# phirling/pyc2ray

Measured on AMD Instinct MI355X. Metric: cell-updates/sec (raytrace+chem), higher is better.
Workload: dtype f64

## Files before the change

include/asora_hip.h:

```cpp
#ifndef ASORA_HIP_H
#define ASORA_HIP_H

#include <stddef.h>
#include <stdint.h>

#ifdef __cplusplus
extern "C" {
#endif


int asora_device_init(int N, int num_src_par);
int asora_device_init_ex(int N, int num_src_par, int device_id);

int asora_device_close(void);

int asora_density_to_device(const double *ndens, int N);

int asora_photo_table_to_device(const double *thin_table, const double *thick_table, int NumTau);

int asora_heat_table_to_device(const double *heat_thin_table, const double *heat_thick_table, int NumTau);

int asora_source_data_to_device(const int32_t *pos, const double *flux, int NumSrc);

#define ASORA_MAX_SPECTRA 16
int asora_spectra_to_device(int NumSpec, int NumTau, const double *photo_thin, const double *photo_thick,
                            const double *heat_thin, const double *heat_thick);
int asora_source_spectra_to_device(const int32_t *spec, int NumSrc);
int asora_num_spectra(void);
int asora_debug_sort_sources(const int32_t *pos, const double *flux, const int32_t *spec, int NumSrc, int32_t *pos_out,
                             double *flux_out, int32_t *spec_out);

int asora_do_all_sources(double R, double *coldensh_out, double sig, double dr, const double *ndens,
                         const double *xh_av, double *phi_ion, int NumSrc, int m1,
                         double minlogtau, double dlogtau, int NumTau);

int c2ray_global_pass(double dt, const double *ndens, const double *temp, const double *xh,
                      double *xh_av, double *xh_intermed, const double *phi_ion,
                      double bh00, double albpow, double colh0, double temph0, double abu_c,
                      int m1, int m2, int m3, int *conv_flag);

int c2ray_do_all_sources(const double *normflux, const int32_t *srcpos, int max_subbox, int subboxsize,
                         double *coldensh_out, double sig, double dr, const double *ndens, const double *xh_av,
                         double *phi_ion, double *phi_heat, float loss_fraction,
                         const double *photo_thin_table, const double *photo_thick_table,
                         const double *heat_thin_table, const double *heat_thick_table,
                         double minlogtau, double dlogtau, double R_max_LLS,
                         int NumTau, int NumSrc, int m1, int m2, int m3,
                         int *sum_nbox, double *photon_loss);

const char *asora_last_error(void);


enum {
    ASORA_GRID_NDENS = 0,
    ASORA_GRID_XH_AV = 1,
    ASORA_GRID_PHI_ION = 2,
    ASORA_GRID_TEMP = 3,
    ASORA_GRID_XH = 4,
    ASORA_GRID_XH_INTERMED = 5,
    ASORA_GRID_PHI_HEAT = 6,
    ASORA_GRID_TEMP_END = 7,
    ASORA_GRID_CLUMP = 8,
    ASORA_GRID_COUNT = 9
};

int asora_grid_to_device(int which, const double *host, int N, char order);
int asora_grid_to_host(int which, double *host, int N, char order);
int asora_grid_copy(int dst, int src);
int asora_grid_scale(int which, double factor);
int asora_grid_sum(int which, double *sum);
int asora_host_alloc(size_t bytes, void **host);
int asora_host_free(void *host);
void *asora_device_ptr(int which);

int asora_raytrace_device(double R, double sig, double dr, int src_begin, int src_count,
                          double minlogtau, double dlogtau, int NumTau);

int asora_raytrace_begin(double R, double sig, double dr, double minlogtau, double dlogtau, int NumTau);
int asora_raytrace_range(int src_begin, int src_count);
int asora_raytrace_begin_planes(double R, double sig, double dr, double minlogtau, double dlogtau, int NumTau,
                                const int *runs, int nruns);
int asora_raytrace_fold(int i_begin, int i_count);
void *asora_stream(void);

int asora_subbox_raytrace_device(int max_subbox, int subboxsize, float loss_fraction, double R_max_LLS, double sig,
                                 double dr, double minlogtau, double dlogtau, int NumTau, int src_begin, int src_count,
                                 int *sum_nbox, double *photon_loss);
int asora_device_init_auto(int N);

int asora_chemistry_device(double dt, double bh00, double albpow, double colh0, double temph0,
                           double abu_c, int *conv_flag, double *sum_xh1, double *sum_xh0);

int asora_chemistry_range(double dt, double bh00, double albpow, double colh0, double temph0, double abu_c,
                          int i_begin, int i_count, int first);
int asora_chemistry_finish(int *conv_flag, double *sum_xh1, double *sum_xh0);
void *asora_reduction_ptr(void);

int asora_evolve_begin(double dt, double bh00, double albpow, double colh0, double temph0, double abu_c,
                       double R, double sig, double dr, double minlogtau, double dlogtau, int NumTau,
                       int src_begin, int src_count, double conv_criterion, double convergence_fraction);
int asora_evolve_enqueue(int iterations);
int asora_evolve_poll(int *niter, int *converged, double *history, int history_rows, int *rows_written);

int asora_evolve_begin_slab(double dt, double bh00, double albpow, double colh0, double temph0, double abu_c,
                            double R, double sig, double dr, double minlogtau, double dlogtau, int NumTau,
                            int src_begin, int src_count, double conv_criterion, double convergence_fraction,
                            int own_begin, int own_count);
int asora_evolve_begin_slab_thermal(double dt, double bh00, double albpow, double colh0, double temph0, double abu_c,
                                    double R, double sig, double dr, double minlogtau, double dlogtau, int NumTau,
                                    int src_begin, int src_count, double conv_criterion, double convergence_fraction,
                                    int own_begin, int own_count);
int asora_evolve_slab_trace(int src_begin, int src_count);
int asora_evolve_slab_fold_out(int i_begin, int i_count);
int asora_evolve_slab_fold_all(void);
void *asora_evolve_slab_outbox(void);
int asora_evolve_slab_outbox_to_host(int i_begin, int i_count, double *host);
int asora_evolve_slab_outbox_from_host(int i_begin, int i_count, const double *host);
int asora_evolve_slab_add(int i_begin, int i_count, const double *dev_planes);
int asora_evolve_slab_add_host(int i_begin, int i_count, const double *host_planes);
void *asora_evolve_slab_heat_outbox(void);
int asora_evolve_slab_heat_outbox_to_host(int i_begin, int i_count, double *host);
int asora_evolve_slab_heat_outbox_from_host(int i_begin, int i_count, const double *host);
int asora_evolve_slab_add_heat(int i_begin, int i_count, const double *dev_planes);
int asora_evolve_slab_add_heat_host(int i_begin, int i_count, const double *host_planes);
int asora_evolve_slab_pass(void);
int asora_evolve_slab_nhi(int i_begin, int i_count);
int asora_evolve_slab_close(const double *host_sums);

int asora_planes_to_host(int which, int i_begin, int i_count, double *host);
int asora_planes_to_device(int which, int i_begin, int i_count, const double *host);

int asora_thermal_params(int enable, double relative_denergy, double t_floor, int max_substeps, unsigned cooling_mask,
                         int compton, double t_cmb);
int asora_thermal_stats(long long *cells_max_substeps, long long *cells_floored, int *max_substeps_used);

int asora_clumping(int mode, double constant);

int asora_lls_opacity(double n_const, double per_density);
int asora_get_lls_opacity(double *n_const, double *per_density);


enum {
    ASORA_OPT_FORTRAN_CONSTANTS = 0,
    ASORA_OPT_GREY_NOTABLES = 1,
    ASORA_OPT_TIMING = 2,
    ASORA_OPT_Z_TRANSPOSED = 3,
    ASORA_OPT_BLOCK_THREADS = 4,
    ASORA_OPT_SECTORS = 5,
    ASORA_OPT_HEATING = 6,
    ASORA_OPT_C2RAY_OWN_FLUX = 7,
    ASORA_OPT_NO_UNIFORM_T = 8,
    ASORA_OPT_SUBBOX_GLOBAL_SHELLS = 9,
    ASORA_OPT_PIPELINED_COPIES = 10,
    ASORA_OPT_SKIP_ZERO_RATES = 11,
    ASORA_OPT_GLOBAL_ATOMICS = 12,
    ASORA_OPT_PAIR_SOURCES = 13,
    ASORA_OPT_SUBBOX_TABLES = 14,
    ASORA_OPT_ALIGNED_ROWS = 15,
    ASORA_OPT_GEOMETRY_ON_HOST = 16,
    ASORA_OPT_PLACEMENT_CANDIDATES = 17,
    ASORA_OPT_OPEN_BOUNDARIES = 18,
    ASORA_OPT_COUNT = 19
};
int asora_set_option(int option, int value);
int asora_get_option(int option);

enum { ASORA_KERNEL_RAYTRACE = 0, ASORA_KERNEL_CHEMISTRY = 1, ASORA_KERNEL_PREP = 2,
       ASORA_KERNEL_FINISH = 3, ASORA_KERNEL_COUNT = 4 };
int asora_kernel_time_ms(int kernel, double *total_ms, long *launches);
int asora_kernel_time_reset(void);
int asora_synchronize(void);

int asora_last_raytrace_counts(long long *gamma_cells, long long *evaluated_cells);
int asora_last_raytrace_counts_ex(long long *gamma_cells, long long *evaluated_cells, long long *zero_rates_left_out);

int asora_debug_coldens(double R, double sig, double dr, int source_index, double *coldens_out, int N);

enum {
    ASORA_VARIANT_PAIRED = 1,
    ASORA_VARIANT_ALIGNED = 2,
    ASORA_VARIANT_BUFFER_ATOMICS = 4,
    ASORA_VARIANT_SPLIT_DESCRIPTORS = 8,
    ASORA_VARIANT_SKIP_ZERO = 16,
    ASORA_VARIANT_GLOBAL_SHELLS = 32,
    ASORA_VARIANT_OPEN_BOUNDARIES = 64
};
int asora_last_raytrace_variant(void);

size_t asora_debug_geometry_bytes(void);
void asora_debug_placement(int *candidates, double *chosen_probe_ms, double *slowest_probe_ms);
void asora_debug_init_cost(double *device_init_ms, double *placement_probe_ms);
int asora_debug_geometry_table(int table, uint32_t *words, size_t capacity_entries, size_t *entries, int *nsteps, int *ntables,
                               int *shells, int *max_cells, int *threads);

const char *asora_build_id(void);
const char *asora_build_flags(void);

#ifdef __cplusplus
}
#endif
#endif
```

pyc2ray_amd/_capi.py:

```python
import ctypes as C
import os

_HERE = os.path.dirname(os.path.abspath(__file__))
LIB_PATH = os.environ.get("PYC2RAY_AMD_LIBASORA") or os.path.join(_HERE, "lib", "libasora_hip.so")

GRID_NDENS, GRID_XH_AV, GRID_PHI_ION, GRID_TEMP, GRID_XH, GRID_XH_INTERMED, GRID_PHI_HEAT = range(7)
GRID_TEMP_END = 7
GRID_CLUMP = 8
(OPT_FORTRAN_CONSTANTS, OPT_GREY_NOTABLES, OPT_TIMING, OPT_Z_TRANSPOSED, OPT_BLOCK_THREADS, OPT_SECTORS,
 OPT_HEATING, OPT_C2RAY_OWN_FLUX, OPT_NO_UNIFORM_T, OPT_SUBBOX_GLOBAL_SHELLS, OPT_PIPELINED_COPIES,
 OPT_SKIP_ZERO_RATES, OPT_GLOBAL_ATOMICS, OPT_PAIR_SOURCES, OPT_SUBBOX_TABLES, OPT_ALIGNED_ROWS, OPT_GEOMETRY_ON_HOST,
 OPT_PLACEMENT_CANDIDATES, OPT_OPEN_BOUNDARIES) = range(19)
MAX_SPECTRA = 16
KERNEL_RAYTRACE, KERNEL_CHEMISTRY, KERNEL_PREP, KERNEL_FINISH = range(4)
VARIANT_PAIRED, VARIANT_ALIGNED, VARIANT_BUFFER_ATOMICS, VARIANT_SPLIT_DESCRIPTORS, VARIANT_SKIP_ZERO, VARIANT_GLOBAL_SHELLS = 1, 2, 4, 8, 16, 32
VARIANT_OPEN_BOUNDARIES = 64

_dp = C.POINTER(C.c_double)
_ip = C.POINTER(C.c_int32)

SIGNATURES = {
    "asora_device_init": (C.c_int, [C.c_int, C.c_int]),
    "asora_device_init_ex": (C.c_int, [C.c_int, C.c_int, C.c_int]),
    "asora_device_close": (C.c_int, []),
    "asora_density_to_device": (C.c_int, [_dp, C.c_int]),
    "asora_photo_table_to_device": (C.c_int, [_dp, _dp, C.c_int]),
    "asora_heat_table_to_device": (C.c_int, [_dp, _dp, C.c_int]),
    "asora_source_data_to_device": (C.c_int, [_ip, _dp, C.c_int]),
    "asora_spectra_to_device": (C.c_int, [C.c_int, C.c_int, _dp, _dp, _dp, _dp]),
    "asora_source_spectra_to_device": (C.c_int, [_ip, C.c_int]),
    "asora_num_spectra": (C.c_int, []),
    "asora_debug_sort_sources": (C.c_int, [_ip, _dp, _ip, C.c_int, _ip, _dp, _ip]),
    "asora_do_all_sources": (C.c_int, [C.c_double, _dp, C.c_double, C.c_double, _dp, _dp, _dp, C.c_int, C.c_int,
                                       C.c_double, C.c_double, C.c_int]),
    "c2ray_global_pass": (C.c_int, [C.c_double, _dp, _dp, _dp, _dp, _dp, _dp, C.c_double, C.c_double, C.c_double,
                                    C.c_double, C.c_double, C.c_int, C.c_int, C.c_int, C.POINTER(C.c_int)]),
    "c2ray_do_all_sources": (C.c_int, [_dp, _ip, C.c_int, C.c_int, _dp, C.c_double, C.c_double, _dp, _dp, _dp, _dp,
                                       C.c_float, _dp, _dp, _dp, _dp, C.c_double, C.c_double, C.c_double,
                                       C.c_int, C.c_int, C.c_int, C.c_int, C.c_int, C.POINTER(C.c_int), _dp]),
    "asora_last_error": (C.c_char_p, []),
    "asora_grid_to_device": (C.c_int, [C.c_int, _dp, C.c_int, C.c_char]),
    "asora_grid_to_host": (C.c_int, [C.c_int, _dp, C.c_int, C.c_char]),
    "asora_grid_copy": (C.c_int, [C.c_int, C.c_int]),
    "asora_grid_scale": (C.c_int, [C.c_int, C.c_double]),
    "asora_device_ptr": (C.c_void_p, [C.c_int]),
    "asora_grid_sum": (C.c_int, [C.c_int, C.POINTER(C.c_double)]),
    "asora_host_alloc": (C.c_int, [C.c_size_t, C.POINTER(C.c_void_p)]),
    "asora_host_free": (C.c_int, [C.c_void_p]),
    "asora_raytrace_device": (C.c_int, [C.c_double, C.c_double, C.c_double, C.c_int, C.c_int, C.c_double,
                                        C.c_double, C.c_int]),
    "asora_raytrace_begin": (C.c_int, [C.c_double, C.c_double, C.c_double, C.c_double, C.c_double, C.c_int]),
    "asora_raytrace_range": (C.c_int, [C.c_int, C.c_int]),
    "asora_raytrace_begin_planes": (C.c_int, [C.c_double, C.c_double, C.c_double, C.c_double, C.c_double, C.c_int, _ip,
                                              C.c_int]),
    "asora_raytrace_fold": (C.c_int, [C.c_int, C.c_int]),
    "asora_stream": (C.c_void_p, []),
    "asora_subbox_raytrace_device": (C.c_int, [C.c_int, C.c_int, C.c_float, C.c_double, C.c_double, C.c_double, C.c_double,
                                               C.c_double, C.c_int, C.c_int, C.c_int, C.POINTER(C.c_int), _dp]),
    "asora_device_init_auto": (C.c_int, [C.c_int]),
    "asora_chemistry_device": (C.c_int, [C.c_double, C.c_double, C.c_double, C.c_double, C.c_double, C.c_double,
                                         C.POINTER(C.c_int), _dp, _dp]),
    "asora_chemistry_range": (C.c_int, [C.c_double, C.c_double, C.c_double, C.c_double, C.c_double, C.c_double,
                                        C.c_int, C.c_int, C.c_int]),
    "asora_chemistry_finish": (C.c_int, [C.POINTER(C.c_int), _dp, _dp]),
    "asora_reduction_ptr": (C.c_void_p, []),
    "asora_evolve_begin": (C.c_int, [C.c_double] * 11 + [C.c_int, C.c_int, C.c_int, C.c_double, C.c_double]),
    "asora_evolve_enqueue": (C.c_int, [C.c_int]),
    "asora_evolve_poll": (C.c_int, [C.POINTER(C.c_int), C.POINTER(C.c_int), _dp, C.c_int, C.POINTER(C.c_int)]),
    "asora_evolve_begin_slab": (C.c_int, [C.c_double] * 11 + [C.c_int, C.c_int, C.c_int, C.c_double, C.c_double, C.c_int, C.c_int]),
    "asora_evolve_begin_slab_thermal": (C.c_int, [C.c_double] * 11 + [C.c_int, C.c_int, C.c_int, C.c_double, C.c_double, C.c_int, C.c_int]),
    "asora_evolve_slab_trace": (C.c_int, [C.c_int, C.c_int]),
    "asora_evolve_slab_fold_out": (C.c_int, [C.c_int, C.c_int]),
    "asora_evolve_slab_outbox": (C.c_void_p, []),
    "asora_evolve_slab_outbox_to_host": (C.c_int, [C.c_int, C.c_int, _dp]),
    "asora_evolve_slab_outbox_from_host": (C.c_int, [C.c_int, C.c_int, _dp]),
    "asora_evolve_slab_fold_all": (C.c_int, []),
    "asora_debug_placement": (None, [C.POINTER(C.c_int), _dp, _dp]),
    "asora_debug_init_cost": (None, [_dp, _dp]),
    "asora_evolve_slab_add": (C.c_int, [C.c_int, C.c_int, C.c_void_p]),
    "asora_evolve_slab_add_host": (C.c_int, [C.c_int, C.c_int, _dp]),
    "asora_evolve_slab_heat_outbox": (C.c_void_p, []),
    "asora_evolve_slab_heat_outbox_to_host": (C.c_int, [C.c_int, C.c_int, _dp]),
    "asora_evolve_slab_heat_outbox_from_host": (C.c_int, [C.c_int, C.c_int, _dp]),
    "asora_evolve_slab_add_heat": (C.c_int, [C.c_int, C.c_int, C.c_void_p]),
    "asora_evolve_slab_add_heat_host": (C.c_int, [C.c_int, C.c_int, _dp]),
    "asora_evolve_slab_pass": (C.c_int, []),
    "asora_evolve_slab_nhi": (C.c_int, [C.c_int, C.c_int]),
    "asora_evolve_slab_close": (C.c_int, [_dp]),
    "asora_planes_to_host": (C.c_int, [C.c_int, C.c_int, C.c_int, _dp]),
    "asora_planes_to_device": (C.c_int, [C.c_int, C.c_int, C.c_int, _dp]),
    "asora_thermal_params": (C.c_int, [C.c_int, C.c_double, C.c_double, C.c_int, C.c_uint, C.c_int, C.c_double]),
    "asora_thermal_stats": (C.c_int, [C.POINTER(C.c_longlong), C.POINTER(C.c_longlong), C.POINTER(C.c_int)]),
    "asora_clumping": (C.c_int, [C.c_int, C.c_double]),
    "asora_lls_opacity": (C.c_int, [C.c_double, C.c_double]),
    "asora_get_lls_opacity": (C.c_int, [_dp, _dp]),
    "asora_set_option": (C.c_int, [C.c_int, C.c_int]),
    "asora_get_option": (C.c_int, [C.c_int]),
    "asora_kernel_time_ms": (C.c_int, [C.c_int, _dp, C.POINTER(C.c_long)]),
    "asora_kernel_time_reset": (C.c_int, []),
    "asora_synchronize": (C.c_int, []),
    "asora_last_raytrace_counts": (C.c_int, [C.POINTER(C.c_longlong), C.POINTER(C.c_longlong)]),
    "asora_last_raytrace_counts_ex": (C.c_int, [C.POINTER(C.c_longlong), C.POINTER(C.c_longlong), C.POINTER(C.c_longlong)]),
    "asora_debug_coldens": (C.c_int, [C.c_double, C.c_double, C.c_double, C.c_int, _dp, C.c_int]),
    "asora_last_raytrace_variant": (C.c_int, []),
    "asora_debug_geometry_bytes": (C.c_size_t, []),
    "asora_debug_geometry_table": (C.c_int, [C.c_int, C.POINTER(C.c_uint32), C.c_size_t, C.POINTER(C.c_size_t), C.POINTER(C.c_int),
                                             C.POINTER(C.c_int), C.POINTER(C.c_int), C.POINTER(C.c_int), C.POINTER(C.c_int)]),
    "asora_build_id": (C.c_char_p, []),
    "asora_build_flags": (C.c_char_p, []),
}

_lib = None


def load():
    global _lib
    if _lib is not None:
        return _lib
    if not os.path.exists(LIB_PATH):
        raise RuntimeError(
            f"pyc2ray_amd: HIP library not found at {LIB_PATH}. Build it with "
            "`make -C pyc2ray_amd/csrc` (or `python -c 'import __graft_entry__ as g; g.build()'`). "
            "There is no CPU fallback.")
    if os.environ.get("PYC2RAY_AMD_NO_TORCH", "0") != "1":
        try:
            import torch
        except ImportError:
            pass
    lib = C.CDLL(LIB_PATH)
    for name, (res, args) in SIGNATURES.items():
        fn = getattr(lib, name)
        fn.restype = res
        fn.argtypes = args
    _lib = lib
    return lib


def check(rc, what):
    if rc != 0:
        msg = load().asora_last_error()
        raise RuntimeError(f"{what} failed (code {rc}): {msg.decode() if msg else 'unknown error'}")


def dptr(a):
    return a.ctypes.data_as(_dp)


def iptr(a):
    return a.ctypes.data_as(_ip)
```

pyc2ray_amd/csrc/api.hip:

```cpp
#include "asora_internal.hpp"

#include <chrono>

namespace asora {

static State g_state;
static std::string g_error;

State &state() { return g_state; }
int fail(int code, const std::string &msg) { g_error = msg; return code; }
void clear_error() { g_error.clear(); }

static int flush_timers()
{
    State &st = g_state;
    if (st.pending_timers.empty()) return 0;
    ASORA_HIP_TRY(hipStreamSynchronize(st.stream));
    for (hipStream_t s : st.side) if (s) ASORA_HIP_TRY(hipStreamSynchronize(s));
    for (auto &pt : st.pending_timers) {
        float ms = 0.f;
        if (hipEventElapsedTime(&ms, pt.e0, pt.e1) == hipSuccess) {
            st.k_ms[pt.which] += (double)ms;
            st.k_n[pt.which] += 1;
        }
        st.free_events.push_back(pt.e0);
        st.free_events.push_back(pt.e1);
    }
    st.pending_timers.clear();
    return 0;
}

static hipEvent_t take_event()
{
    State &st = g_state;
    if (!st.free_events.empty()) { hipEvent_t e = st.free_events.back(); st.free_events.pop_back(); return e; }
    hipEvent_t e = nullptr;
    (void)hipEventCreate(&e);
    return e;
}

KernelTimer::KernelTimer(int w, hipStream_t s)
    : which(w), on(g_state.opt[ASORA_OPT_TIMING] != 0 && g_state.stream != nullptr), stream(s ? s : g_state.stream)
{
    if (!on) return;
    if (g_state.pending_timers.size() >= 4096) (void)flush_timers();
    e0 = take_event();
    e1 = take_event();
    (void)hipEventRecord(e0, stream);
}
KernelTimer::~KernelTimer()
{
    if (!on) return;
    (void)hipEventRecord(e1, stream);
    g_state.pending_timers.push_back({which, e0, e1});
}

int ensure_runtime()
{
    State &st = g_state;
    if (st.stream) return 0;
    ASORA_HIP_TRY(hipSetDevice(st.device));
    hipDeviceProp_t prop;
    ASORA_HIP_TRY(hipGetDeviceProperties(&prop, st.device));
    st.cu_count = prop.multiProcessorCount > 0 ? prop.multiProcessorCount : 256;
    ASORA_HIP_TRY(hipStreamCreateWithFlags(&st.stream, hipStreamNonBlocking));
    for (int q = 0; q < 2; ++q) {
        ASORA_HIP_TRY(hipStreamCreateWithFlags(&st.side[q], hipStreamNonBlocking));
        ASORA_HIP_TRY(hipEventCreateWithFlags(&st.side_done[q], hipEventDisableTiming));
    }
    ASORA_HIP_TRY(hipEventCreateWithFlags(&st.main_ready, hipEventDisableTiming));
    st.red_blocks = chemistry_reduction_blocks(st);
    st.red_cap = 3 * (size_t)st.red_blocks;
    ASORA_HIP_TRY(hipMalloc(&st.red_partial, sizeof(double) * st.red_cap));
    ASORA_HIP_TRY(hipMalloc(&st.red_final, sizeof(double) * 3));
    ASORA_HIP_TRY(hipHostMalloc(&st.red_host, sizeof(double) * 3, hipHostMallocDefault));
    ASORA_HIP_TRY(hipMalloc(&st.counters, sizeof(unsigned long long) * COUNTER_FIELDS * COUNTER_SLOTS));
    ASORA_HIP_TRY(hipMemset(st.counters, 0, sizeof(unsigned long long) * COUNTER_FIELDS * COUNTER_SLOTS));
    return 0;
}

static int release_all()
{
    State &st = g_state;
    auto drop = [](auto *&ptr) { if (ptr) { (void)hipFree(ptr); ptr = nullptr; } };
    drop(st.grid[ASORA_GRID_PHI_HEAT]);
    drop(st.grid[ASORA_GRID_TEMP_END]); drop(st.heat_acc); drop(st.heat_outbox); drop(st.th_stats_dev);
    st.heat_clean[0] = st.heat_clean[1] = false;
    st.th_on = false; st.th = ThermalConsts();
    drop(st.grid[ASORA_GRID_CLUMP]);
    st.clump_mode = 0; st.clump_c = 1.0;
    st.lls_a = st.lls_b = 0.0;
    for (int g = 0; g < ASORA_GRID_COUNT; ++g) { st.grid[g] = nullptr; st.grid_valid[g] = false; }
    st.nhi = st.staging = st.acc = nullptr;
    drop(st.arena); st.arena_bytes = 0;
    st.ev_clean[0] = st.ev_clean[1] = false; st.ev_sets_known = false;
    drop(st.reach.mask); drop(st.reach.count_dev); st.reach = State::ReachMask();
    st.ev_open = false;
    st.temp_probe_valid = false;
    st.nhi_t = st.phi_t = st.heat_t = nullptr;
    st.have_heat_tables = false;
    drop(st.tables); st.table_len = 0; st.num_spec = 1; st.spec_stride = 0;
    drop(st.src_spec); drop(st.src_spec_sorted); st.src_spec_max = 0;
    drop(st.src_pos); drop(st.src_flux); drop(st.src_pos_sorted); drop(st.src_flux_sorted); st.src_i0_sorted.clear(); st.num_src = 0;
    st.src_pos_host.clear(); st.src_pos_sorted_host.clear();
    release_pair_lists(st);
    drop(st.shell_scratch); st.shell_scratch_bytes = 0;
    drop(st.sb_trail); st.sb_trail_bytes = 0;
    if (st.geom_patch_dev) { (void)hipFree(st.geom_patch_dev); st.geom_patch_dev = nullptr; st.geom_patch_cap = 0; }
    drop(st.sb_active); drop(st.sb_nbox); drop(st.sb_loss); drop(st.sb_loss_final); st.subbox_cap = 0;
    release_geometry(st);
    st.init = false; st.N = 0; st.ncell = 0;
    st.rt_radius[0] = State::RadiusHistory(); st.rt_radius[1] = State::RadiusHistory();
    if (st.zero_probe_dev) { (void)hipFree(st.zero_probe_dev); st.zero_probe_dev = nullptr; }
    if (st.zero_probe_host) { (void)hipHostFree(st.zero_probe_host); st.zero_probe_host = nullptr; }
    if (st.zero_probe_done) { (void)hipEventDestroy(st.zero_probe_done); st.zero_probe_done = nullptr; }
    st.zero_probe_pending = false; st.zero_known = false; st.zero_dark = false; st.zero_since_probe = 0;
    st.rt_open = false;
    return 0;
}

int require_init(const char *who)
{
    if (!g_state.init) return fail(2, std::string(who) + ": device not initialised (call asora_device_init first)");
    return 0;
}

int check_N(const char *who, int N)
{
    if (N != g_state.N)
        return fail(3, std::string(who) + ": mesh size " + std::to_string(N) + " does not match device_init(" +
                           std::to_string(g_state.N) + ")");
    return 0;
}

int check_planes(const char *who, int code, const char *tail, int i_begin, int i_count)
{
    if (i_begin < 0 || i_count < 0 || i_begin + i_count > g_state.N) return fail(code, std::string(who) + ": " + tail);
    return 0;
}

int check_sources(const char *who, int code, const std::string &tail, int src_begin, int src_count)
{
    if (src_begin < 0 || src_count < 0 || src_begin + src_count > g_state.num_src) return fail(code, std::string(who) + ": " + tail);
    return 0;
}

int require_grids(const char *who, std::initializer_list<int> grids)
{
    for (int g : grids)
        if (!g_state.grid_valid[g]) return fail(4, std::string(who) + ": grid " + std::to_string(g) + " holds no data");
    return 0;
}

}

using namespace asora;

extern "C" {

constexpr int ARENA_CANDIDATES = 8;
constexpr int ARENA_SLOTS = 14;
__global__ void __launch_bounds__(256) placement_probe_kernel(char *arena, size_t slot, size_t n)
{
    const double *in[5]; double *out[7];
    for (int q = 0; q < 5; ++q) in[q] = reinterpret_cast<const double *>(arena + q * slot);
    for (int q = 0; q < 7; ++q) out[q] = reinterpret_cast<double *>(arena + (5 + q) * slot);
    for (size_t i = (size_t)blockIdx.x * 256 + threadIdx.x; i < n; i += (size_t)gridDim.x * 256) {
        double s = 0.0;
#pragma unroll
        for (int q = 0; q < 5; ++q) s += __builtin_nontemporal_load(in[q] + i);
#pragma unroll
        for (int q = 0; q < 7; ++q) out[q][i] = s;
    }
}

static int choose_arena(State &st, size_t slot, int slots)
{
    const auto wall0 = std::chrono::steady_clock::now();
    const size_t total = slot * (size_t)slots;
    int want = st.opt[ASORA_OPT_PLACEMENT_CANDIDATES] > 0 ? st.opt[ASORA_OPT_PLACEMENT_CANDIDATES] : ARENA_CANDIDATES;
    if (const char *e = getenv("ASORA_PLACEMENT_CANDIDATES")) want = std::max(1, atoi(e));
    want = std::min(want, 32);
    if (st.N < 128) want = 1;
    size_t free_b = 0, all_b = 0;
    if (want > 1 && hipMemGetInfo(&free_b, &all_b) == hipSuccess && total > 0)
        want = (int)std::max<size_t>(1, std::min<size_t>((size_t)want, (size_t)(0.125 * (double)free_b) / total));
    st.arena_candidates = 0; st.arena_probe_ms = st.arena_probe_worst_ms = st.arena_probe_wall_ms = 0.0;
    if (want == 1) {
        ASORA_HIP_TRY(hipMalloc(&st.arena, total));
        st.arena_bytes = total; st.arena_candidates = 1;
        return 0;
    }
    hipEvent_t t0, t1;
    ASORA_HIP_TRY(hipEventCreate(&t0)); ASORA_HIP_TRY(hipEventCreate(&t1));
    std::vector<char *> cand;
    std::vector<float> ms;
    int best = -1;
    float worst = 0.0f;
    const size_t n = st.ncell;
    for (int c = 0; c < want; ++c) {
        char *a = nullptr;
        if (hipMalloc(&a, total) != hipSuccess) { (void)hipGetLastError(); break; }
        cand.push_back(a);
        float t = 1e30f;
        for (int rep = 0; rep < 3; ++rep) {
            (void)hipEventRecord(t0, st.stream);
            hipLaunchKernelGGL(placement_probe_kernel, dim3(1024), dim3(256), 0, st.stream, a, slot, n);
            (void)hipEventRecord(t1, st.stream);
            if (hipEventSynchronize(t1) != hipSuccess) { t = 1e30f; break; }
            float e = 0.0f;
            (void)hipEventElapsedTime(&e, t0, t1);
            if (rep >= 1) t = std::min(t, e);
        }
        ms.push_back(t);
        if (best < 0 || t < ms[(size_t)best]) best = c;
        worst = std::max(worst, t);
        if (c >= 1 && ms[(size_t)best] <= 0.93f * worst) break;
    }
    (void)hipEventDestroy(t0); (void)hipEventDestroy(t1);
    if (best < 0) return fail(2, "device_init: out of device memory for the grids");
    for (size_t c = 0; c < cand.size(); ++c) if ((int)c != best) (void)hipFree(cand[c]);
    st.arena = cand[(size_t)best];
    st.arena_bytes = total;
    st.arena_candidates = (int)cand.size();
    st.arena_probe_ms = ms[(size_t)best]; st.arena_probe_worst_ms = worst;
    st.arena_probe_wall_ms = std::chrono::duration<double, std::milli>(std::chrono::steady_clock::now() - wall0).count();
    return 0;
}

void asora_debug_placement(int *candidates, double *chosen_probe_ms, double *slowest_probe_ms)
{
    if (candidates) *candidates = g_state.arena_candidates;
    if (chosen_probe_ms) *chosen_probe_ms = g_state.arena_probe_ms;
    if (slowest_probe_ms) *slowest_probe_ms = g_state.arena_probe_worst_ms;
}

void asora_debug_init_cost(double *device_init_ms, double *placement_probe_ms)
{
    if (device_init_ms) *device_init_ms = g_state.device_init_wall_ms;
    if (placement_probe_ms) *placement_probe_ms = g_state.arena_probe_wall_ms;
}

const char *asora_last_error(void) { return g_error.c_str(); }

int asora_device_init_ex(int N, int num_src_par, int device_id)
{
    clear_error();
    State &st = g_state;
    const auto init_wall0 = std::chrono::steady_clock::now();
    if (N < 2 || N > 1280) return fail(1, "device_init: N must be in [2, 1280] (32-bit cell indices over 2 N^3)");
    if (st.stream && device_id != st.device) return fail(1, "device_init: the device cannot change within a process");
    if (st.init) release_all();
    st.device = device_id;
    if (int rc = ensure_runtime()) return rc;
    st.N = N;
    st.ncell = (size_t)N * N * N;
    st.num_src_par = num_src_par;
    st.auto_init = false;
    const size_t bytes = st.ncell * sizeof(double);
    const size_t slot = (bytes + 4095) / 4096 * 4096;
    if (int rc = choose_arena(st, slot, ARENA_SLOTS)) return rc;
    {
        size_t at = 0;
        auto take = [&](size_t grids) { double *q = reinterpret_cast<double *>(st.arena + at); at += grids * slot; return q; };
        st.grid[ASORA_GRID_NDENS] = take(1); st.grid[ASORA_GRID_XH] = take(1); st.grid[ASORA_GRID_XH_AV] = take(1);
        st.grid[ASORA_GRID_TEMP] = take(1); st.grid[ASORA_GRID_XH_INTERMED] = take(1);
        st.acc = take(4);
        st.nhi = take(2);
        st.grid[ASORA_GRID_PHI_ION] = take(2);
        st.staging = take(1);
    }
    for (int g = 0; g < ASORA_GRID_COUNT; ++g)
        if (g != ASORA_GRID_PHI_HEAT && g != ASORA_GRID_TEMP_END && g != ASORA_GRID_CLUMP && !st.grid[g]) return fail(11, "device_init: a grid without a place in the arena (internal error)");
    st.nhi_t = st.nhi + st.ncell;
    st.phi_t = st.grid[ASORA_GRID_PHI_ION] + st.ncell;
    st.heat_t = nullptr;
    st.ev_sets_known = false;
    {
        size_t worst = 0;
        for (int planes = 1; planes <= N; ++planes) worst = std::max(worst, chemistry_tile_blocks(st, N, planes));
        if (int rc = ensure_red_capacity(3 * worst)) return rc;
    }
    st.init = true;
    st.device_init_wall_ms = std::chrono::duration<double, std::milli>(std::chrono::steady_clock::now() - init_wall0).count();
    return 0;
}

int asora_device_init(int N, int num_src_par)
{
    int dev = g_state.stream ? g_state.device : 0;
    if (!g_state.stream) {
        if (hipGetDevice(&dev) != hipSuccess) dev = 0;
    }
    return asora_device_init_ex(N, num_src_par, dev);
}

int asora_device_close(void)
{
    clear_error();
    if (int rc = require_init("device_close")) return rc;
    ASORA_HIP_TRY(hipStreamSynchronize(g_state.stream));
    return release_all();
}

void *asora_stream(void) { return (void *)g_state.stream; }

int asora_set_option(int option, int value)
{
    clear_error();
    if (option < 0 || option >= ASORA_OPT_COUNT) return fail(3, "set_option: unknown option");
    g_state.opt[option] = value;
    return 0;
}

int asora_get_option(int option)
{
    if (option < 0 || option >= ASORA_OPT_COUNT) return -1;
    return g_state.opt[option];
}

int asora_kernel_time_ms(int kernel, double *total_ms, long *launches)
{
    clear_error();
    if (kernel < 0 || kernel >= ASORA_KERNEL_COUNT) return fail(3, "kernel_time_ms: unknown kernel");
    if (int rc = flush_timers()) return rc;
    if (total_ms) *total_ms = g_state.k_ms[kernel];
    if (launches) *launches = g_state.k_n[kernel];
    return 0;
}

int asora_kernel_time_reset(void)
{
    (void)flush_timers();
    for (int k = 0; k < ASORA_KERNEL_COUNT; ++k) { g_state.k_ms[k] = 0.0; g_state.k_n[k] = 0; }
    return 0;
}

int asora_synchronize(void)
{
    clear_error();
    if (!g_state.stream) return 0;
    ASORA_HIP_TRY(hipStreamSynchronize(g_state.stream));
    ASORA_HIP_TRY(hipDeviceSynchronize());
    return 0;
}

}
```

pyc2ray_amd/csrc/asora_internal.hpp:

```cpp
#pragma once
#include <hip/hip_runtime.h>
#include <algorithm>
#include <cmath>
#include <cstdint>
#include <cstdio>
#include <cstdlib>
#include <cstring>
#include <initializer_list>
#include <string>
#include <vector>

#include "../../include/asora_hip.h"

namespace asora {

struct OctGeomDev {
    const uint4 *cellA;
    const uint4 *cellB;
    int nsteps;
    int info;
    int inner;
    int reserved_;
};

constexpr int MAX_UNITS = 96;

constexpr int COUNTER_SLOTS = 4096;
constexpr int ZERO_PROBE_SLOTS = 256;
constexpr int COUNTER_FIELDS = 3;

inline double lut_index_limit(int NumTau, int table_len)
{
    const double by_reference = (double)(float)NumTau, by_table = (double)(table_len > 0 ? table_len - 1 : 0);
    return by_reference < by_table ? by_reference : by_table;
}

struct RtParams {
    int N;
    int S;
    int max_cells;
    double R;
    double sig, dr;
    double minlogtau, dlogtau, numtau_f;
    double lut_k1, lut_k0;
    double tau_zero;
    int NumTau, table_len;
    int fortran_consts, grey, z_transposed;
    int src_begin, src_count;
    int shape_src_count;
    int split_desc;
    int radius_stays;
    OctGeomDev geom[MAX_UNITS];
    int units;
    int spread;
    const double2 *logtab;
    unsigned ncell;
    const double *nhi;
    double *phi;
    const double2 *tables;
    double *heat;
    const int32_t *src_pos;
    const double *src_flux;
    double *dump;
    double *shell_scratch;
    unsigned long long *counters;
    const int *done_flag;
    unsigned long long *zero_probe;
    int aligned;
    const int2 *pairs[2];
    int npairs[2];
    int sb_k0[12], sb_k1[12];
    int sb_first;
    int sb_edge_r, sb_edge_l;
    int flux_src;
    const int *sb_active;
    double *sb_loss;
    double *sb_trail;
    const int32_t *src_spec;
    unsigned spec_stride;
    int open_bc;
};

struct ThermalConsts {
    double relative_denergy = 0.1;
    double t_floor = 1.0;
    double t_cmb = 0.0;
    int max_substeps = 10000;
    unsigned cooling_mask = 31u;
    int compton = 0;
};
constexpr unsigned THERMAL_COOL_RECOMB = 1u, THERMAL_COOL_COLION = 2u, THERMAL_COOL_COLEXC = 4u, THERMAL_COOL_BREMS = 8u,
                   THERMAL_COOL_COMPTON = 16u;

constexpr int EVOLVE_HIST = 64;
struct EvolveStatus {
    int niter;
    int done;
    double prev1, prev0;
    double conv_criterion, conv_fraction;
    double hist[EVOLVE_HIST][5];
};

struct State {
    bool init = false;
    bool auto_init = false;
    int device = 0;
    int N = 0;
    size_t ncell = 0;
    int num_src_par = 0;
    int cu_count = 256;

    double *grid[ASORA_GRID_COUNT] = {nullptr, nullptr, nullptr, nullptr, nullptr, nullptr, nullptr, nullptr, nullptr};
    bool grid_valid[ASORA_GRID_COUNT] = {false, false, false, false, false, false, false, false, false};

    double *nhi = nullptr;
    double *nhi_t = nullptr;
    double *phi_t = nullptr;
    double *heat_t = nullptr;
    bool have_heat_tables = false;
    double *staging = nullptr;

    double2 *tables = nullptr;
    int table_len = 0;
    int num_spec = 1;
    size_t spec_stride = 0;

    int32_t *src_pos = nullptr;
    double *src_flux = nullptr;
    int num_src = 0;
    int32_t *src_pos_sorted = nullptr;
    double *src_flux_sorted = nullptr;
    std::vector<int> src_i0_sorted;
    int32_t *src_spec = nullptr, *src_spec_sorted = nullptr;
    int src_spec_max = 0;
    std::vector<hipEvent_t> pipe_events;

    std::vector<void *> geom_owned;
    size_t geom_bytes = 0;
    OctGeomDev geom_host[MAX_UNITS];
    bool geom_aligned = false;
    unsigned long long *zero_probe_dev = nullptr;
    unsigned long long *zero_probe_host = nullptr;
    hipEvent_t zero_probe_done = nullptr;
    bool zero_probe_pending = false, zero_known = false, zero_dark = false;
    int zero_since_probe = 0;
    int last_variant = 0;
    struct RadiusHistory { double last_R = -1.0; long same_R_calls = 0; bool has_changed = false; };
    RadiusHistory rt_radius[2];
    std::vector<int32_t> src_pos_host, src_pos_sorted_host;
    struct PairList { const void *list; int begin, count; int2 *dev[2]; int n[2]; };
    std::vector<PairList> pair_lists;
    int geom_units = 0;
    double2 *logtab_dev = nullptr;
    bool geom_valid = false;
    bool geom_on_host = false;
    struct SphereCell { uint32_t *dev_word; uint32_t word_without_rate; int a, b, c; };
    std::vector<SphereCell> geom_sphere;
    void *geom_patch_dev = nullptr;
    size_t geom_patch_cap = 0;
    int geom_N = 0, geom_S = 0, geom_max_cells = 0, geom_threads = 0;
    int geom_subbox = 0, geom_ext_r = 0, geom_ext_l = 0, geom_boxsize = 0;
    std::vector<int> geom_step_after_shell[12];
    double geom_R = 0.0, geom_dr = 0.0;

    RtParams rt_params;
    bool rt_open = false, rt_heat = false;
    bool rt_pipelined = false;
    bool rt_by_planes = false;
    hipStream_t side[2] = {nullptr, nullptr};
    hipEvent_t side_done[2] = {nullptr, nullptr}, main_ready = nullptr;
    bool side_pending[2] = {false, false};
    int side_next = 0;

    int *sb_active = nullptr, *sb_nbox = nullptr, *sb_nactive = nullptr;
    double *sb_loss = nullptr, *sb_loss_final = nullptr;
    size_t subbox_cap = 0;

    double *sb_trail = nullptr;
    size_t sb_trail_bytes = 0;

    double *shell_scratch = nullptr;
    size_t shell_scratch_bytes = 0;

    double *red_partial = nullptr;
    size_t red_cap = 0;
    double *red_final = nullptr;
    double *red_host = nullptr;
    int red_blocks = 0;

    unsigned long long *counters = nullptr;
    long long last_gamma_cells = 0, last_eval_cells = 0;

    double *acc = nullptr;
    char *arena = nullptr;
    size_t arena_bytes = 0;
    int arena_candidates = 0;
    double arena_probe_ms = 0.0, arena_probe_worst_ms = 0.0;
    double arena_probe_wall_ms = 0.0, device_init_wall_ms = 0.0;
    int ev_base = 0;
    bool ev_clean[2] = {false, false};
    bool ev_sets_known = false;
    int ev_folded_iter = -1;
    EvolveStatus *ev_status = nullptr;
    EvolveStatus *ev_host = nullptr;
    bool ev_open = false, ev_first = true;
    double *temp_probe_dev = nullptr;
    double temp_probe[5] = {0, 0, 0, 0, 0};
    bool temp_probe_valid = false;
    double temp_consts[4] = {0, 0, 0, 0};
    int ev_reported = 0;
    int ev_enqueued = 0;
    double ev_chem[6] = {0, 0, 0, 0, 0, 0};
    int ev_src_begin = 0, ev_src_count = 0;
    RtParams ev_rt;
    bool ev_slab = false;
    int ev_own_begin = 0, ev_own_count = 0;
    bool ev_slab_passed = false;
    bool ev_folded_all = false;
    bool ev_rates_in_outbox = false;
    bool ev_slab_thermal = false;
    struct ReachMask {
        unsigned char *mask = nullptr;
        size_t bytes = 0;
        unsigned long long *count_dev = nullptr;
        bool in_use = false;
        bool pays = false;
        struct Key {
            bool valid = false;
            long src_generation = -1;
            int src_begin = 0, src_count = 0;
            double R = -1.0;
            bool operator==(const Key &o) const { return valid == o.valid && src_generation == o.src_generation && src_begin == o.src_begin && src_count == o.src_count && R == o.R; }
        } key;
    } reach;
    long src_generation = 0;

    bool th_on = false;
    ThermalConsts th;
    double *heat_acc = nullptr;
    bool heat_clean[2] = {false, false};
    double *heat_outbox = nullptr;
    unsigned long long *th_stats_dev = nullptr;

    int clump_mode = 0;
    double clump_c = 1.0;
    double temp_probe_clump = 1.0;

    double lls_a = 0.0, lls_b = 0.0;
    bool coldens_only = false;

    hipStream_t stream = nullptr;
    struct PendingTimer { int which; hipEvent_t e0, e1; };
    std::vector<PendingTimer> pending_timers;
    std::vector<hipEvent_t> free_events;
    int opt[ASORA_OPT_COUNT] = {0, 0, 0, 1, 0, 0, 0, 0, 0, 0, 1, 0, 0, 0, 0, 0, 0, 0, 0};
    double k_ms[ASORA_KERNEL_COUNT] = {0, 0, 0, 0};
    long k_n[ASORA_KERNEL_COUNT] = {0, 0, 0, 0};
};

State &state();
int fail(int code, const std::string &msg);
void clear_error();

#define ASORA_HIP_TRY(expr)                                                                     \
    do {                                                                                        \
        hipError_t e__ = (expr);                                                                \
        if (e__ != hipSuccess)                                                                  \
            return ::asora::fail(10, std::string(#expr) + ": " + hipGetErrorName(e__) + " - " + \
                                         hipGetErrorString(e__));                               \
    } while (0)

struct KernelTimer {
    int which;
    bool on;
    hipStream_t stream;
    hipEvent_t e0 = nullptr, e1 = nullptr;
    explicit KernelTimer(int w, hipStream_t s = nullptr);
    ~KernelTimer();
};


constexpr unsigned CELL_VALID = 1u << 30, CELL_LAST = 1u << 31, CELL_RATE = 1u << 29,
                   CELL_SPHERE = 1u << 28,
                   CELL_ZERO_SHIFT = 25,
                   CELL_NEG_SHIFT = 22,
                   CELL_SLOT_MASK = (1u << 22) - 1;

struct GeomTableSpec {
    int face = -1;
    int merge_mask = 0;
    int ext[3] = {0, 0, 0};
    int ext_neg = 0;
    int wedge = -1;
    int align_class = -1;
};
int build_geometry_on_device(State &st, const std::vector<GeomTableSpec> &specs, double R, double dr, int q_max, int threads,
                             int boxsize, std::vector<OctGeomDev> &out, std::vector<std::vector<int>> &step_after, int &S_all,
                             uint32_t &max_cells_all);
struct SubboxGeometry { int ext_r, ext_l, boxsize; };
int ensure_geometry(State &st, RtParams &p, int threads, int units, const SubboxGeometry *sbg = nullptr, bool aligned = false);
void release_geometry(State &st);
bool note_call_radius(State &st, double R, int path);
void release_pair_lists(State &st);
int launch_fold_range(State &st, const double *src_t, double *dst, int i_begin, int i_count);
int ensure_logtab(State &st);
int launch_prepare_nhi(State &st, bool need_transposed);
int launch_finish_phi(State &st);
int check_open_boundaries(const State &st, const char *who, bool open, bool dump);
int launch_raytrace(State &st, RtParams &p, bool dump, bool heat, hipStream_t side = nullptr);
struct SubboxTables { int units = 0, threads = 0, S = 0, max_batch = 0, nsrc = 1; bool ok = false, aligned = false; const int32_t *host_pos = nullptr; };
int subbox_tables_prepare(State &st, RtParams &p, int ext_r, int ext_l, int subboxsize, int src_count, bool heat, SubboxTables &out,
                          const int32_t *host_pos);
int subbox_tables_sweep(State &st, const RtParams &p, const SubboxTables &tab, int s_begin, int s_end, bool heat);
int launch_fold_transposed(State &st, const double *src_t, double *dst);
int launch_fold_sum(State &st, const double *a, const double *b_t, double *dst);
int launch_transpose(State &st, const double *src, double *dst, int N);

struct SubboxParams {
    int N, W;
    int ext_r, ext_l;
    int s_begin, s_end;
    int edge_r, edge_l;
    double sig, dr, R;
    double numtau_f, lut_k1, lut_k0;
    int table_len;
    int grey, heat, add_zero;
    int src_begin, src_count;
    int flux_src;
    int dump_src;
    unsigned ncell;
    const double *nhi;
    double *phi, *heat_grid;
    double *dump;
    const double2 *tables, *logtab;
    const int32_t *src_pos;
    const double *src_flux;
    double *scratch;
    size_t unit_stride;
    const int *active;
    double *loss;
};
int launch_subbox_sweep(State &st, const SubboxParams &p, hipStream_t side = nullptr);
int launch_subbox_decide(State &st, int mode, int count, const double *src_flux, int src_begin, double loss_fraction,
                         int more_range, int *active, double *loss, double *loss_final, int *nbox, int *n_active);

struct ChemParams {
    size_t ncell;
    double dt, bh00, albpow, colh0, temph0, abu_c;
    const double *ndens, *temp, *xh, *phi;
    double *xh_av, *xh_intermed;
    double *red_partial, *red_final;
    int red_blocks;
    int accumulate = 0;
    bool thermal = false;
    const double *phi_heat = nullptr;
    double *temp_end = nullptr;
    unsigned long long *th_stats = nullptr;
    ThermalConsts th;
    const double *clump = nullptr;
    double clump_c = 1.0;
};
int launch_chemistry(State &st, ChemParams &p, hipStream_t stream, bool clumped = true);
int chemistry_reduction_blocks(const State &st);

struct ChemTileParams {
    int N = 0, i_begin = 0, i_end = 0;
    double dt = 0, bh00 = 0, albpow = 0, colh0 = 0, temph0 = 0, abu_c = 0;
    const double *ndens = nullptr, *temp = nullptr, *xh = nullptr, *xh_av_in = nullptr;
    double *gamma = nullptr, *gamma_t = nullptr;
    double *phi_out = nullptr;
    double *zero_a = nullptr, *zero_t = nullptr;
    double *xh_av = nullptr, *xh_intermed = nullptr;
    double *nhi = nullptr, *nhi_t = nullptr;
    double *red_partial = nullptr, *red_final = nullptr;
    int red_stride = 0;
    int accumulate = 0;
    EvolveStatus *status = nullptr;
    bool local_sums = false;
    const unsigned char *reach_a = nullptr, *reach_t = nullptr;
    bool fold = false, emit = false;
    int uniform = 0, uniform_t_ok = 0;
    double uniform_T = 0, uniform_brech0 = 0, uniform_acolh0 = 0;
    bool thermal = false;
    double *heat = nullptr, *heat_t = nullptr;
    double *zero_ha = nullptr, *zero_ht = nullptr;
    double *temp_end = nullptr;
    unsigned long long *th_stats = nullptr;
    ThermalConsts th;
    const double *clump = nullptr;
    double clump_c = 1.0;
    double *heat_out = nullptr;
    double lls_a = 0.0, lls_b = 0.0;
};
int launch_grid_sum(State &st, const double *a, size_t n, double *out_dev);
int launch_scale(State &st, double *a, size_t n, double factor);
int launch_temp_probe(State &st, const double *temp, size_t n, double bh00, double albpow, double colh0, double temph0,
                      double *out_dev);
int launch_chemistry_tiles(State &st, ChemTileParams &p, hipStream_t stream);
size_t chemistry_tile_blocks(const State &st, int N, int planes);
int launch_prepare_nhi_from(State &st, const double *xh_av, bool need_transposed);
int launch_prepare_range(State &st, int i_begin, int i_count, bool zero_acc, double *acc, const int *done = nullptr);
int launch_fold_out(State &st, const double *a, const double *a_t, double *out, double *z_a, double *z_t, int i_begin, int i_count,
                    const int *done);
int launch_fold_out_pair(State &st, const double *a, const double *a_t, double *out, double *z_a, double *z_t, const double *h,
                         const double *h_t, double *hout, double *zh_a, double *zh_t, int i_begin, int i_count, const int *done);
int launch_add_planes(State &st, double *dst, const double *src, size_t n, const int *done);
int launch_convergence_test(State &st, const double *sums, EvolveStatus *status);
int launch_reach_mask(State &st, const int32_t *src_pos, int src_begin, int src_count, double R, unsigned char *mask, size_t bytes_one_layout);
int launch_reach_count(State &st, const unsigned char *mask, size_t bytes_both_layouts, unsigned long long *out_dev);

int ensure_runtime();
int require_init(const char *who);
int check_N(const char *who, int N);
int check_planes(const char *who, int code, const char *tail, int i_begin, int i_count);
int check_sources(const char *who, int code, const std::string &tail, int src_begin, int src_count);
int require_grids(const char *who, std::initializer_list<int> grids);
int ensure_optional_grid(int which);
int reset_counters();
int require_raytrace_inputs(const char *who, double R, int NumTau, bool density, bool xh_av);
void fill_rt_params(RtParams &p, double R, double sig, double dr, double minlogtau, double dlogtau, int NumTau, int radius_path = 0);
inline void use_source_list(RtParams &p, const State &st, bool sorted)
{
    p.src_pos = sorted ? st.src_pos_sorted : st.src_pos;
    p.src_flux = sorted ? st.src_flux_sorted : st.src_flux;
    p.src_spec = sorted ? st.src_spec_sorted : st.src_spec;
}
int check_source_spectra(const char *who);
void sort_sources_by_position(const int32_t *pos, int NumSrc, std::vector<int> &order);
int ensure_red_capacity(size_t entries);
int ensure_temp_probe(double bh00, double albpow, double colh0, double temph0);
ChemTileParams chem_tile_common(int i_begin, int i_count, const double chem[6]);

}
```

pyc2ray_amd/csrc/chemistry.hip:

```cpp
#include "rates_device.hpp"

#include <algorithm>

namespace asora {

constexpr int CH_THREADS = 256;

struct TempFactors {
    double T = -1.0;
    double brech0 = 0.0, acolh0 = 0.0;
    bool t_ok = false;
};
__device__ __forceinline__ void temperature_factors(const ChemParams &p, double T, TempFactors &f)
{
    if (T == f.T) return;
    f.T = T;
    f.brech0 = 1.0 * p.bh00 * pow(T / 1e4, p.albpow);
    f.acolh0 = p.colh0 * sqrt(T) * exp(-p.temph0 / T);
    f.t_ok = fabs((T - T) / T) < (double)1.0e-3f;
}

template <bool CLUMP = false>
__device__ __forceinline__ void chemistry_cell(const ChemParams &p, double n, double x0, double gamma,
                                               double &xav, double &xint, unsigned int &nconv, const TempFactors &tf,
                                               double clump = 1.0)
{
    const double min_frac_change = (double)1.0e-3f;
    const double min_frac_atoms = (double)1.0e-8f;
    const double eps = 1e-14;

    const double xav_start = xav;
    const double yh_av = 1.0 - xav;

    const double brech0 = CLUMP ? clump * tf.brech0 : tf.brech0, acolh0 = tf.acolh0;
    const bool t_ok = tf.t_ok;

    int nit = 0;
    for (;;) {
        nit += 1;
        const double xav_old = xav;
        const double de = n * (xav + p.abu_c);
        const double aih0 = gamma + de * acolh0;
        const double delth = aih0 + de * brech0;
        const double eqxh = aih0 / delth;
        const double deltht = delth * p.dt;
        const double ee = exp(-deltht);
        xint = (x0 - eqxh) * ee + eqxh;
        if (xint < eps) xint = eps;
        const double avg = (deltht < (double)1.0e-8f) ? 1.0 : (1.0 - ee) / deltht;
        xav = eqxh + (x0 - eqxh) * avg;
        if (xav < eps) xav = eps;
        if ((fabs((xav - xav_old) / (1.0 - xav)) < min_frac_change || (1.0 - xav < min_frac_atoms)) && t_ok)
            break;
        if (nit > 400) break;
    }
    if (fabs(xav - xav_start) > min_frac_change && fabs((xav - xav_start) / yh_av) > min_frac_change &&
        yh_av > min_frac_atoms)
        nconv += 1;
}

constexpr double THERMAL_KB = 1.381e-16;
constexpr double CODATA_SIGMA_T = 6.6524587321e-25, CODATA_SIGMA_SB = 5.670374419e-5, CODATA_C = 2.99792458e10,
                 CODATA_KB = 1.380649e-16, CODATA_ME = 9.1093837015e-28;
constexpr double COMPTON_A_RAD = 4.0 * CODATA_SIGMA_SB / CODATA_C;
constexpr double COMPTON_C = 4.0 * CODATA_SIGMA_T * COMPTON_A_RAD * CODATA_KB / (CODATA_ME * CODATA_C);

template <bool CLUMP = false>
__device__ __forceinline__ double thermal_cooling(const ThermalConsts &c, double T, double n_e, double n_HII, double n_HI,
                                                  double colh0, double temph0, double clump = 1.0)
{
#pragma clang fp contract(off)
    double L = 0.0;
    if (c.cooling_mask & THERMAL_COOL_RECOMB) {
        const double lam = 2.0 * 157807.0 / T;
        double rec = 3.435e-30 * T * pow(lam, 1.970) / pow(1.0 + pow(lam / 2.25, 0.376), 3.720) * n_e * n_HII;
        if (CLUMP) rec = rec * clump;
        L += rec;
    }
    if (c.cooling_mask & THERMAL_COOL_COLION)
        L += THERMAL_KB * temph0 * colh0 * sqrt(T) * exp(-temph0 / T) * n_e * n_HI;
    if (c.cooling_mask & THERMAL_COOL_COLEXC)
        L += 7.5e-19 * exp(-118348.0 / T) / (1.0 + sqrt(T / 1e5)) * n_e * n_HI;
    if (c.cooling_mask & THERMAL_COOL_BREMS) {
        const double u = 5.5 - log10(T);
        const double gff = 1.1 + 0.34 * exp(-(u * u) / 3.0);
        L += 1.42e-27 * gff * sqrt(T) * n_e * n_HII;
    }
    if ((c.cooling_mask & THERMAL_COOL_COMPTON) && c.compton) {
        const double tg = c.t_cmb;
        L += COMPTON_C * ((tg * tg) * (tg * tg)) * (T - tg) * n_e;
    }
    return L;
}

struct ThermalTally {
    unsigned capped = 0, floored = 0;
    int max_sub = 0;
};

template <bool CLUMP = false>
__device__ __forceinline__ void thermal_integrate(const ThermalConsts &c, double dt, double abu_c, double colh0, double temph0,
                                                  double n, double x, double phi_heat, double T_start, double &T_end,
                                                  double &T_av, bool &capped, bool &floored, int &max_sub, double clump = 1.0)
{
#pragma clang fp contract(off)
    const double n_e = n * (x + abu_c), n_HII = n * x, n_HI = n * (1.0 - x);
    const double n_p = n * (1.0 + x + abu_c);
    const double cv = 1.5 * THERMAL_KB * n_p;
    const double H = n_HI * phi_heat;
    double T = T_start, e = cv * T_start, t = 0.0, intT = 0.0;
    int k = 0;
    for (;;) {
        k += 1;
        const double r = H - thermal_cooling<CLUMP>(c, T, n_e, n_HII, n_HI, colh0, temph0, clump);
        double h = dt - t;
        bool last = true;
        if (k < c.max_substeps && r != 0.0) {
            const double hl = c.relative_denergy * e / fabs(r);
            if (hl < h) { h = hl; last = false; }
        }
        double Tn = (e + h * r) / cv;
        if (Tn < c.t_floor) { Tn = c.t_floor; floored = true; }
        e = cv * Tn;
        intT += h * (T + Tn) * 0.5;
        T = Tn;
        if (last) break;
        t += h;
    }
    if (k >= c.max_substeps) capped = true;
    if (k > max_sub) max_sub = k;
    T_end = T;
    T_av = intT / dt;
}

template <bool CLUMP = false>
__device__ __forceinline__ void chemistry_cell_thermal(const ChemParams &p, double n, double x0, double gamma, double phi_heat,
                                                       double T_start, double &xav_io, double &xint_out, double &T_end_out,
                                                       unsigned int &nconv, ThermalTally &tally, double clump = 1.0)
{
#pragma clang fp contract(off)
    const double min_frac_change = (double)1.0e-3f;
    const double min_frac_atoms = (double)1.0e-8f;
    const double eps = 1e-14;

    double xav = xav_io, xint = 0.0;
    const double xav_start = xav;
    const double yh_av = 1.0 - xav;
    double T_av = T_start, T_end = T_start;
    bool capped = false, floored = false;
    int max_sub = tally.max_sub;

    int nit = 0;
    for (;;) {
        nit += 1;
        const double xav_old = xav, T_prev = T_end;
        const double de = n * (xav + p.abu_c);
        double brech0 = 1.0 * p.bh00 * pow(T_av / 1e4, p.albpow);
        if (CLUMP) brech0 = clump * brech0;
        const double acolh0 = p.colh0 * sqrt(T_av) * exp(-p.temph0 / T_av);
        const double aih0 = gamma + de * acolh0;
        const double delth = aih0 + de * brech0;
        const double eqxh = aih0 / delth;
        const double deltht = delth * p.dt;
        const double ee = exp(-deltht);
        xint = (x0 - eqxh) * ee + eqxh;
        if (xint < eps) xint = eps;
        const double avg = (deltht < (double)1.0e-8f) ? 1.0 : (1.0 - ee) / deltht;
        xav = eqxh + (x0 - eqxh) * avg;
        if (xav < eps) xav = eps;
        thermal_integrate<CLUMP>(p.th, p.dt, p.abu_c, p.colh0, p.temph0, n, xav, phi_heat, T_start, T_end, T_av, capped, floored,
                                 max_sub, clump);
        const bool t_ok = fabs((T_end - T_prev) / T_end) < min_frac_change;
        if ((fabs((xav - xav_old) / (1.0 - xav)) < min_frac_change || (1.0 - xav < min_frac_atoms)) && t_ok)
            break;
        if (nit > 400) break;
    }
    if (fabs(xav - xav_start) > min_frac_change && fabs((xav - xav_start) / yh_av) > min_frac_change &&
        yh_av > min_frac_atoms)
        nconv += 1;
    tally.capped += capped ? 1u : 0u;
    tally.floored += floored ? 1u : 0u;
    tally.max_sub = max_sub;
    xav_io = xav; xint_out = xint; T_end_out = T_end;
}

__device__ __forceinline__ void thermal_tally_flush(unsigned long long *stats, ThermalTally t)
{
    unsigned c = t.capped, f = t.floored;
    int m = t.max_sub;
    for (int o = 32; o > 0; o >>= 1) {
        c += __shfl_xor(c, o);
        f += __shfl_xor(f, o);
        m = max(m, __shfl_xor(m, o));
    }
    if ((threadIdx.x & 63) == 0) {
        if (c) atomicAdd(&stats[0], (unsigned long long)c);
        if (f) atomicAdd(&stats[1], (unsigned long long)f);
        atomicMax(&stats[2], (unsigned long long)m);
    }
}

template <bool THERMAL, bool CLUMP = false>
__global__ void __launch_bounds__(CH_THREADS) chemistry_kernel(const ChemParams p)
{
    double sum1 = 0.0, sum0 = 0.0;
    unsigned int nconv = 0;
    TempFactors tf;

    const size_t npair = p.ncell / 2;
    const size_t stride = (size_t)gridDim.x * CH_THREADS;
    const double2 *nd2 = reinterpret_cast<const double2 *>(p.ndens);
    const double2 *tp2 = reinterpret_cast<const double2 *>(p.temp);
    const double2 *x02 = reinterpret_cast<const double2 *>(p.xh);
    const double2 *ph2 = reinterpret_cast<const double2 *>(p.phi);
    double2 *xa2 = reinterpret_cast<double2 *>(p.xh_av);
    double2 *xi2 = reinterpret_cast<double2 *>(p.xh_intermed);
    const double2 *cl2 = reinterpret_cast<const double2 *>(p.clump);
    ThermalTally tally;
    if (THERMAL) {
#pragma unroll 1
        for (size_t i = (size_t)blockIdx.x * CH_THREADS + threadIdx.x; i < p.ncell; i += stride) {
            double xav = p.xh_av[i], xint, te;
            const double c = !CLUMP ? 1.0 : p.clump ? p.clump[i] : p.clump_c;
            chemistry_cell_thermal<CLUMP>(p, p.ndens[i], p.xh[i], p.phi[i], p.phi_heat[i], p.temp[i], xav, xint, te, nconv, tally, c);
            p.xh_intermed[i] = xint;
            p.xh_av[i] = xav;
            p.temp_end[i] = te;
            sum1 += xint; sum0 += 1.0 - xint;
        }
    }
    for (size_t q = (size_t)blockIdx.x * CH_THREADS + threadIdx.x; !THERMAL && q < npair; q += stride) {
        const double2 n = nd2[q], T = tp2[q], x0 = x02[q], g = ph2[q];
        double2 xav = xa2[q], xint;
        const double2 c = CLUMP ? cl2[q] : make_double2(1.0, 1.0);
        temperature_factors(p, T.x, tf);
        chemistry_cell<CLUMP>(p, n.x, x0.x, g.x, xav.x, xint.x, nconv, tf, c.x);
        temperature_factors(p, T.y, tf);
        chemistry_cell<CLUMP>(p, n.y, x0.y, g.y, xav.y, xint.y, nconv, tf, c.y);
        xi2[q] = xint;
        xa2[q] = xav;
        sum1 += xint.x; sum0 += 1.0 - xint.x;
        sum1 += xint.y; sum0 += 1.0 - xint.y;
    }
    if (!THERMAL && (p.ncell & 1) && blockIdx.x == 0 && threadIdx.x == 0) {
        const size_t idx = p.ncell - 1;
        double xav = p.xh_av[idx], xint;
        temperature_factors(p, p.temp[idx], tf);
        chemistry_cell<CLUMP>(p, p.ndens[idx], p.xh[idx], p.phi[idx], xav, xint, nconv, tf, CLUMP ? p.clump[idx] : 1.0);
        p.xh_intermed[idx] = xint;
        p.xh_av[idx] = xav;
        sum1 += xint; sum0 += 1.0 - xint;
    }
    if (THERMAL) thermal_tally_flush(p.th_stats, tally);

    __shared__ double r1[CH_THREADS], r0[CH_THREADS];
    __shared__ unsigned int rc[CH_THREADS];
    r1[threadIdx.x] = sum1; r0[threadIdx.x] = sum0; rc[threadIdx.x] = nconv;
    __syncthreads();
    for (int off = CH_THREADS / 2; off > 0; off >>= 1) {
        if ((int)threadIdx.x < off) {
            r1[threadIdx.x] += r1[threadIdx.x + off];
            r0[threadIdx.x] += r0[threadIdx.x + off];
            rc[threadIdx.x] += rc[threadIdx.x + off];
        }
        __syncthreads();
    }
    if (threadIdx.x == 0) {
        p.red_partial[blockIdx.x] = r1[0];
        p.red_partial[p.red_blocks + blockIdx.x] = r0[0];
        p.red_partial[2 * p.red_blocks + blockIdx.x] = (double)rc[0];
    }
}

constexpr int RED_THREADS = 1024;
__global__ void __launch_bounds__(RED_THREADS) chemistry_reduce_kernel(const double *partial, int nblocks, double *out,
                                                                       int accumulate, EvolveStatus *status,
                                                                       const EvolveStatus *gate = nullptr)
{
    if (status && status->done) return;
    if (gate && gate->done) return;
    double v[3];
    for (int q = 0; q < 3; ++q) {
        double s = 0.0;
        for (int b = threadIdx.x; b < nblocks; b += RED_THREADS) s += partial[(size_t)q * nblocks + b];
        for (int o = 32; o > 0; o >>= 1) s += __shfl_down(s, o);
        v[q] = s;
    }
    __shared__ double r[3][RED_THREADS / 64];
    if ((threadIdx.x & 63) == 0)
        for (int q = 0; q < 3; ++q) r[q][threadIdx.x >> 6] = v[q];
    __syncthreads();
    if (threadIdx.x == 0) {
        double tot[3];
        for (int q = 0; q < 3; ++q) {
            double s = 0.0;
            for (int w = 0; w < RED_THREADS / 64; ++w) s += r[q][w];
            tot[q] = s;
            out[q] = (accumulate ? out[q] : 0.0) + s;
        }
        if (status) {
            const double sum1 = tot[0], sum0 = tot[1], nconv = tot[2];
            const double rel1 = sum1 > 0.0 ? fabs((sum1 - status->prev1) / sum1) : 1.0;
            const double rel0 = sum0 > 0.0 ? fabs((sum0 - status->prev0) / sum0) : 1.0;
            const bool converged = (nconv < status->conv_criterion) ||
                                   (rel1 < status->conv_fraction && rel0 < status->conv_fraction);
            double *h = status->hist[status->niter % EVOLVE_HIST];
            h[0] = nconv; h[1] = sum1; h[2] = sum0; h[3] = rel1; h[4] = rel0;
            status->prev1 = sum1; status->prev0 = sum0;
            status->niter += 1;
            if (converged) status->done = 1;
        }
    }
}

__device__ __forceinline__ double stream_load(const double *q) { return __builtin_nontemporal_load(q); }

template <bool FOLD, bool EMIT, bool UNIFORM_T, bool THERMAL = false, bool CLUMP = false>
__global__ void __launch_bounds__(CH_THREADS, 1) chemistry_tile_kernel(const ChemTileParams p)
{
    static_assert(!THERMAL || (EMIT && !UNIFORM_T), "thermal pass: the device loop's emit forms only (with or without fold), never UNIFORM_T");
    if (p.status && p.status->done) return;
    __shared__ double tile_g[32][33], tile_n[32][33];
    __shared__ double tile_h[(THERMAL && FOLD) ? 32 : 1][33];
    __shared__ double r1[CH_THREADS], r0[CH_THREADS];
    __shared__ unsigned int rc[CH_THREADS];

    const int N = p.N;
    const int NL = (N + 7) >> 3;
    const int tx = threadIdx.x & 31, ty = threadIdx.x >> 5;
    const int kb = blockIdx.x * 32, ib = p.i_begin + blockIdx.z * 32;
    ChemParams cp;
    cp.dt = p.dt; cp.bh00 = p.bh00; cp.albpow = p.albpow; cp.colh0 = p.colh0; cp.temph0 = p.temph0; cp.abu_c = p.abu_c;
    if (THERMAL) cp.th = p.th;

    double sum1 = 0.0, sum0 = 0.0;
    unsigned int nconv = 0;
    ThermalTally tally;
    TempFactors tf;
    if (UNIFORM_T) { tf.T = p.uniform_T; tf.brech0 = p.uniform_brech0; tf.acolh0 = p.uniform_acolh0; tf.t_ok = p.uniform_t_ok != 0; }
    for (int j = blockIdx.y; j < N; j += gridDim.y) {
        if ((FOLD || EMIT) && j != (int)blockIdx.y) __syncthreads();
        if (FOLD) {
            for (int r = ty; r < 32; r += 8) {
                const int k = kb + r, i = ib + tx;
                if (k < N && i < p.i_end) {
                    const size_t o = ((size_t)k * N + j) * N + i;
                    const bool reached = !p.reach_t || p.reach_t[((size_t)k * N + j) * NL + (i >> 3)] != 0;
                    tile_g[r][tx] = reached ? stream_load(p.gamma_t + o) : 0.0;
                    if (EMIT && reached) p.zero_t[o] = 0.0;
                    if (THERMAL) {
                        tile_h[r][tx] = reached ? stream_load(p.heat_t + o) : 0.0;
                        if (reached) p.zero_ht[o] = 0.0;
                    }
                }
            }
            __syncthreads();
        }
        for (int r = ty; r < 32; r += 8) {
            const int i = ib + r, k = kb + tx;
            if (i < p.i_end && k < N) {
                const size_t idx = ((size_t)i * N + j) * N + k;
                const bool reached = !FOLD || !p.reach_a || p.reach_a[((size_t)i * N + j) * NL + (k >> 3)] != 0;
                double g = reached ? stream_load(p.gamma + idx) : 0.0;
                if (FOLD) g += tile_g[tx][r];
                if (p.phi_out) p.phi_out[idx] = g;
                if (EMIT && reached) p.zero_a[idx] = 0.0;
                const double n = stream_load(p.ndens + idx);
                double xav = stream_load(p.xh_av_in + idx), xint;
                double c = 1.0;
                if (CLUMP) c = (THERMAL && !p.clump) ? p.clump_c : stream_load(p.clump + idx);
                if (THERMAL) {
                    double hr = reached ? stream_load(p.heat + idx) : 0.0;
                    if (FOLD) hr += tile_h[tx][r];
                    else p.heat_out[idx] = hr;
                    if (reached) p.zero_ha[idx] = 0.0;
                    double te;
                    chemistry_cell_thermal<CLUMP>(cp, n, stream_load(p.xh + idx), g, hr, stream_load(p.temp + idx), xav, xint, te, nconv,
                                                  tally, c);
                    p.temp_end[idx] = te;
                } else {
                    if (!UNIFORM_T) temperature_factors(cp, stream_load(p.temp + idx), tf);
                    chemistry_cell<CLUMP>(cp, n, stream_load(p.xh + idx), g, xav, xint, nconv, tf, c);
                }
                p.xh_intermed[idx] = xint;
                p.xh_av[idx] = xav;
                sum1 += xint; sum0 += 1.0 - xint;
                if (EMIT) {
                    const double v = absorber_density(n, xav, p.lls_a, p.lls_b);
                    p.nhi[idx] = v;
                    tile_n[r][tx] = v;
                }
            }
        }
        if (EMIT) {
            __syncthreads();
            for (int r = ty; r < 32; r += 8) {
                const int k = kb + r, i = ib + tx;
                if (k < N && i < p.i_end) p.nhi_t[((size_t)k * N + j) * N + i] = tile_n[tx][r];
            }
        }
    }

    if (THERMAL) thermal_tally_flush(p.th_stats, tally);
    r1[threadIdx.x] = sum1; r0[threadIdx.x] = sum0; rc[threadIdx.x] = nconv;
    __syncthreads();
    for (int off = CH_THREADS / 2; off > 0; off >>= 1) {
        if ((int)threadIdx.x < off) {
            r1[threadIdx.x] += r1[threadIdx.x + off];
            r0[threadIdx.x] += r0[threadIdx.x + off];
            rc[threadIdx.x] += rc[threadIdx.x + off];
        }
        __syncthreads();
    }
    if (threadIdx.x == 0) {
        const size_t b = ((size_t)blockIdx.z * gridDim.y + blockIdx.y) * gridDim.x + blockIdx.x;
        p.red_partial[b] = r1[0];
        p.red_partial[(size_t)p.red_stride + b] = r0[0];
        p.red_partial[2 * (size_t)p.red_stride + b] = (double)rc[0];
    }
}

__global__ void __launch_bounds__(CH_THREADS) temp_minmax_kernel(const double *__restrict__ temp, size_t n, double *partial)
{
    double lo = INFINITY, hi = -INFINITY;
    bool nan = false;
    for (size_t q = (size_t)blockIdx.x * CH_THREADS + threadIdx.x; q < n; q += (size_t)gridDim.x * CH_THREADS) {
        const double t = temp[q];
        nan = nan || (t != t);
        lo = fmin(lo, t); hi = fmax(hi, t);
    }
    __shared__ double slo[CH_THREADS], shi[CH_THREADS];
    __shared__ int snan[CH_THREADS];
    slo[threadIdx.x] = lo; shi[threadIdx.x] = hi; snan[threadIdx.x] = nan ? 1 : 0;
    __syncthreads();
    for (int off = CH_THREADS / 2; off > 0; off >>= 1) {
        if ((int)threadIdx.x < off) {
            slo[threadIdx.x] = fmin(slo[threadIdx.x], slo[threadIdx.x + off]);
            shi[threadIdx.x] = fmax(shi[threadIdx.x], shi[threadIdx.x + off]);
            snan[threadIdx.x] |= snan[threadIdx.x + off];
        }
        __syncthreads();
    }
    if (threadIdx.x == 0) {
        partial[blockIdx.x] = slo[0];
        partial[gridDim.x + blockIdx.x] = shi[0];
        partial[2 * gridDim.x + blockIdx.x] = (double)snan[0];
    }
}

__global__ void __launch_bounds__(CH_THREADS) temp_probe_final_kernel(const double *partial, int nblocks, double bh00, double albpow,
                                                                      double colh0, double temph0, double *out)
{
    double lo = INFINITY, hi = -INFINITY, nan = 0.0;
    for (int b = threadIdx.x; b < nblocks; b += CH_THREADS) {
        lo = fmin(lo, partial[b]); hi = fmax(hi, partial[nblocks + b]); nan += partial[2 * nblocks + b];
    }
    __shared__ double slo[CH_THREADS], shi[CH_THREADS], snan[CH_THREADS];
    slo[threadIdx.x] = lo; shi[threadIdx.x] = hi; snan[threadIdx.x] = nan;
    __syncthreads();
    for (int off = CH_THREADS / 2; off > 0; off >>= 1) {
        if ((int)threadIdx.x < off) {
            slo[threadIdx.x] = fmin(slo[threadIdx.x], slo[threadIdx.x + off]);
            shi[threadIdx.x] = fmax(shi[threadIdx.x], shi[threadIdx.x + off]);
            snan[threadIdx.x] += snan[threadIdx.x + off];
        }
        __syncthreads();
    }
    if (threadIdx.x != 0) return;
    lo = slo[0]; hi = shi[0]; nan = snan[0];
    ChemParams p;
    p.bh00 = bh00; p.albpow = albpow; p.colh0 = colh0; p.temph0 = temph0;
    TempFactors tf;
    temperature_factors(p, lo, tf);
    out[0] = (lo == hi && nan == 0.0) ? 1.0 : 0.0;
    out[1] = lo; out[2] = tf.brech0; out[3] = tf.acolh0; out[4] = tf.t_ok ? 1.0 : 0.0;
}

int launch_temp_probe(State &st, const double *temp, size_t n, double bh00, double albpow, double colh0, double temph0,
                      double *out_dev)
{
    const int blocks = (int)std::min<size_t>(std::max<size_t>(1, (n + CH_THREADS - 1) / CH_THREADS), (size_t)st.red_blocks);
    hipLaunchKernelGGL(temp_minmax_kernel, dim3(blocks), dim3(CH_THREADS), 0, st.stream, temp, n, st.red_partial);
    ASORA_HIP_TRY(hipGetLastError());
    hipLaunchKernelGGL(temp_probe_final_kernel, dim3(1), dim3(CH_THREADS), 0, st.stream, (const double *)st.red_partial, blocks, bh00,
                       albpow, colh0, temph0, out_dev);
    ASORA_HIP_TRY(hipGetLastError());
    return 0;
}

__global__ void __launch_bounds__(CH_THREADS) grid_sum_kernel(const double *__restrict__ a, size_t n, double *partial)
{
    double s = 0.0;
    for (size_t q = (size_t)blockIdx.x * CH_THREADS + threadIdx.x; q < n; q += (size_t)gridDim.x * CH_THREADS) s += a[q];
    __shared__ double sh[CH_THREADS];
    sh[threadIdx.x] = s;
    __syncthreads();
    for (int off = CH_THREADS / 2; off > 0; off >>= 1) {
        if ((int)threadIdx.x < off) sh[threadIdx.x] += sh[threadIdx.x + off];
        __syncthreads();
    }
    if (threadIdx.x == 0) partial[blockIdx.x] = sh[0];
}

__global__ void __launch_bounds__(CH_THREADS) grid_sum_final_kernel(const double *partial, int nblocks, double *out)
{
    double s = 0.0;
    for (int b = threadIdx.x; b < nblocks; b += CH_THREADS) s += partial[b];
    __shared__ double sh[CH_THREADS];
    sh[threadIdx.x] = s;
    __syncthreads();
    for (int off = CH_THREADS / 2; off > 0; off >>= 1) {
        if ((int)threadIdx.x < off) sh[threadIdx.x] += sh[threadIdx.x + off];
        __syncthreads();
    }
    if (threadIdx.x == 0) out[0] = sh[0];
}

int launch_grid_sum(State &st, const double *a, size_t n, double *out_dev)
{
    const int blocks = (int)std::min<size_t>(std::max<size_t>(1, (n + CH_THREADS - 1) / CH_THREADS), (size_t)st.red_blocks);
    hipLaunchKernelGGL(grid_sum_kernel, dim3(blocks), dim3(CH_THREADS), 0, st.stream, a, n, st.red_partial);
    ASORA_HIP_TRY(hipGetLastError());
    hipLaunchKernelGGL(grid_sum_final_kernel, dim3(1), dim3(CH_THREADS), 0, st.stream, (const double *)st.red_partial, blocks, out_dev);
    ASORA_HIP_TRY(hipGetLastError());
    return 0;
}

int chemistry_reduction_blocks(const State &st) { return st.cu_count * 8; }

static int clumping_of(const State &st, bool thermal, size_t ncell, const double *&clump, double &clump_c, double &bh00_factor)
{
    clump = nullptr; clump_c = 1.0; bh00_factor = 1.0;
    if (st.clump_mode == 0) return 0;
    if (st.clump_mode == 2) {
        if (!st.grid[ASORA_GRID_CLUMP] || !st.grid_valid[ASORA_GRID_CLUMP] || ncell != st.ncell)
            return fail(4, "chemistry: clumping mode 2 needs ASORA_GRID_CLUMP on the device");
        clump = st.grid[ASORA_GRID_CLUMP];
        return 1;
    }
    if (!thermal) { bh00_factor = st.clump_c; return 0; }
    clump_c = st.clump_c;
    return 1;
}

int launch_chemistry(State &st, ChemParams &p, hipStream_t stream, bool clumped)
{
    const size_t want = std::max<size_t>(1, (p.ncell / 2 + CH_THREADS - 1) / CH_THREADS);
    const int blocks = (int)std::min<size_t>(want, (size_t)p.red_blocks);
    ChemParams q = p;
    q.red_blocks = blocks;
    int ck = 0;
    if (clumped) {
        double f;
        ck = clumping_of(st, p.thermal, p.ncell, q.clump, q.clump_c, f);
        if (ck > 1) return ck;
        q.bh00 = f * p.bh00;
    }
    {
        KernelTimer kt(ASORA_KERNEL_CHEMISTRY);
        if (p.thermal && ck) hipLaunchKernelGGL((chemistry_kernel<true, true>), dim3(blocks), dim3(CH_THREADS), 0, stream, q);
        else if (p.thermal)  hipLaunchKernelGGL(chemistry_kernel<true>, dim3(blocks), dim3(CH_THREADS), 0, stream, q);
        else if (ck)         hipLaunchKernelGGL((chemistry_kernel<false, true>), dim3(blocks), dim3(CH_THREADS), 0, stream, q);
        else                 hipLaunchKernelGGL(chemistry_kernel<false>, dim3(blocks), dim3(CH_THREADS), 0, stream, q);
        ASORA_HIP_TRY(hipGetLastError());
    }
    hipLaunchKernelGGL(chemistry_reduce_kernel, dim3(1), dim3(RED_THREADS), 0, stream,
                       (const double *)p.red_partial, blocks, p.red_final, p.accumulate, (EvolveStatus *)nullptr,
                       (const EvolveStatus *)nullptr);
    ASORA_HIP_TRY(hipGetLastError());
    return 0;
}

static dim3 tile_pass_grid(const State &st, int N, int planes)
{
    const unsigned kt = (N + 31) / 32, it = (planes + 31) / 32;
    const unsigned want = (unsigned)st.cu_count * 16u;
    unsigned jc = std::max(1u, std::min((unsigned)N, (want + kt * it - 1) / (kt * it)));
    return dim3(kt, jc, it);
}

size_t chemistry_tile_blocks(const State &st, int N, int planes)
{
    const dim3 g = tile_pass_grid(st, N, planes);
    return (size_t)g.x * g.y * g.z;
}

template <bool CLUMP>
static int launch_tile_form(const ChemTileParams &q, dim3 grid, hipStream_t stream)
{
    const bool u = q.uniform != 0;
    if (q.thermal) {
        if (!q.emit) return fail(11, "chemistry: the thermal pass exists in the emit forms only (internal error)");
        if (!q.fold && !q.heat_out) return fail(11, "chemistry: the thermal pass without fold keeps the summed heating (internal error)");
        if (q.fold) hipLaunchKernelGGL((chemistry_tile_kernel<true, true, false, true, CLUMP>), grid, dim3(CH_THREADS), 0, stream, q);
        else        hipLaunchKernelGGL((chemistry_tile_kernel<false, true, false, true, CLUMP>), grid, dim3(CH_THREADS), 0, stream, q);
    } else if (q.fold && q.emit) {
        if (u) hipLaunchKernelGGL((chemistry_tile_kernel<true, true, true, false, CLUMP>), grid, dim3(CH_THREADS), 0, stream, q);
        else   hipLaunchKernelGGL((chemistry_tile_kernel<true, true, false, false, CLUMP>), grid, dim3(CH_THREADS), 0, stream, q);
    } else if (!q.fold && !q.emit) {
        if (u) hipLaunchKernelGGL((chemistry_tile_kernel<false, false, true, false, CLUMP>), grid, dim3(CH_THREADS), 0, stream, q);
        else   hipLaunchKernelGGL((chemistry_tile_kernel<false, false, false, false, CLUMP>), grid, dim3(CH_THREADS), 0, stream, q);
    } else if (!q.fold && q.emit) {
        if (u) hipLaunchKernelGGL((chemistry_tile_kernel<false, true, true, false, CLUMP>), grid, dim3(CH_THREADS), 0, stream, q);
        else   hipLaunchKernelGGL((chemistry_tile_kernel<false, true, false, false, CLUMP>), grid, dim3(CH_THREADS), 0, stream, q);
    } else return fail(11, "chemistry: unsupported fold/emit combination (internal error)");
    return 0;
}

int launch_chemistry_tiles(State &st, ChemTileParams &p, hipStream_t stream)
{
    const int planes = p.i_end - p.i_begin;
    if (planes <= 0) return 0;
    const dim3 grid = tile_pass_grid(st, p.N, planes);
    const size_t blocks = (size_t)grid.x * grid.y * grid.z;
    if (3 * blocks > st.red_cap) return fail(11, "chemistry: reduction buffer too small (internal error)");
    ChemTileParams q = p;
    q.red_stride = (int)blocks;
    double f;
    const int ck = clumping_of(st, p.thermal, st.ncell, q.clump, q.clump_c, f);
    if (ck > 1) return ck;
    q.bh00 = f * p.bh00;
    if (p.uniform && !p.thermal && st.temp_probe_clump != f)
        return fail(4, "chemistry: the temperature probe was made for another clumping mode (set asora_clumping before asora_evolve_begin)");
    {
        KernelTimer kt(ASORA_KERNEL_CHEMISTRY, stream);
        if (int rc = ck ? launch_tile_form<true>(q, grid, stream) : launch_tile_form<false>(q, grid, stream)) return rc;
        ASORA_HIP_TRY(hipGetLastError());
    }
    hipLaunchKernelGGL(chemistry_reduce_kernel, dim3(1), dim3(RED_THREADS), 0, stream,
                       (const double *)p.red_partial, (int)blocks, p.red_final, p.accumulate,
                       p.local_sums ? (EvolveStatus *)nullptr : p.status, (const EvolveStatus *)(p.local_sums ? p.status : nullptr));
    ASORA_HIP_TRY(hipGetLastError());
    return 0;
}

__global__ void convergence_test_kernel(const double *sums, EvolveStatus *status)
{
    if (status->done) return;
    const double sum1 = sums[0], sum0 = sums[1], nconv = sums[2];
    const double rel1 = sum1 > 0.0 ? fabs((sum1 - status->prev1) / sum1) : 1.0;
    const double rel0 = sum0 > 0.0 ? fabs((sum0 - status->prev0) / sum0) : 1.0;
    const bool converged = (nconv < status->conv_criterion) ||
                           (rel1 < status->conv_fraction && rel0 < status->conv_fraction);
    double *h = status->hist[status->niter % EVOLVE_HIST];
    h[0] = nconv; h[1] = sum1; h[2] = sum0; h[3] = rel1; h[4] = rel0;
    status->prev1 = sum1; status->prev0 = sum0;
    status->niter += 1;
    if (converged) status->done = 1;
}

int launch_convergence_test(State &st, const double *sums, EvolveStatus *status)
{
    hipLaunchKernelGGL(convergence_test_kernel, dim3(1), dim3(1), 0, st.stream, sums, status);
    ASORA_HIP_TRY(hipGetLastError());
    return 0;
}

}
```

pyc2ray_amd/csrc/chemistry_api.hip:

```cpp
#include "asora_internal.hpp"

namespace asora {

int ensure_temp_probe(double bh00, double albpow, double colh0, double temph0)
{
    State &st = state();
    const double clump = st.clump_mode == 1 ? st.clump_c : 1.0;
    const double b = clump * bh00;
    const double c[4] = {b, albpow, colh0, temph0};
    if (st.temp_probe_valid && std::memcmp(c, st.temp_consts, sizeof c) == 0 && st.temp_probe_clump == clump) return 0;
    if (!st.temp_probe_dev) ASORA_HIP_TRY(hipMalloc(&st.temp_probe_dev, sizeof(double) * 8));
    if (int rc = launch_temp_probe(st, st.grid[ASORA_GRID_TEMP], st.ncell, b, albpow, colh0, temph0, st.temp_probe_dev)) return rc;
    ASORA_HIP_TRY(hipMemcpyAsync(st.temp_probe, st.temp_probe_dev, sizeof(double) * 5, hipMemcpyDeviceToHost, st.stream));
    ASORA_HIP_TRY(hipStreamSynchronize(st.stream));
    std::memcpy(st.temp_consts, c, sizeof c);
    st.temp_probe_clump = clump;
    st.temp_probe_valid = true;
    return 0;
}

ChemTileParams chem_tile_common(int i_begin, int i_count, const double chem[6])
{
    State &st = state();
    ChemTileParams p;
    p.N = st.N; p.i_begin = i_begin; p.i_end = i_begin + i_count;
    p.dt = chem[0]; p.bh00 = chem[1]; p.albpow = chem[2]; p.colh0 = chem[3]; p.temph0 = chem[4]; p.abu_c = chem[5];
    p.ndens = st.grid[ASORA_GRID_NDENS]; p.temp = st.grid[ASORA_GRID_TEMP]; p.xh = st.grid[ASORA_GRID_XH];
    p.xh_av = st.grid[ASORA_GRID_XH_AV]; p.xh_intermed = st.grid[ASORA_GRID_XH_INTERMED];
    p.red_partial = st.red_partial; p.red_final = st.red_final;
    p.uniform = (st.temp_probe_valid && st.temp_probe[0] != 0.0 && !st.opt[ASORA_OPT_NO_UNIFORM_T]) ? 1 : 0;
    p.uniform_T = st.temp_probe[1]; p.uniform_brech0 = st.temp_probe[2]; p.uniform_acolh0 = st.temp_probe[3];
    p.uniform_t_ok = st.temp_probe[4] != 0.0 ? 1 : 0;
    p.lls_a = st.lls_a; p.lls_b = st.lls_b;
    return p;
}

static int read_reductions(int *conv_flag, double *sum_xh1, double *sum_xh0)
{
    State &st = state();
    ASORA_HIP_TRY(hipMemcpyAsync(st.red_host, st.red_final, sizeof(double) * 3, hipMemcpyDeviceToHost, st.stream));
    ASORA_HIP_TRY(hipStreamSynchronize(st.stream));
    if (sum_xh1) *sum_xh1 = st.red_host[0];
    if (sum_xh0) *sum_xh0 = st.red_host[1];
    if (conv_flag) *conv_flag = (int)st.red_host[2];
    return 0;
}

int ensure_red_capacity(size_t entries)
{
    State &st = state();
    if (entries <= st.red_cap) return 0;
    if (st.stream) ASORA_HIP_TRY(hipStreamSynchronize(st.stream));
    if (st.red_partial) { (void)hipFree(st.red_partial); st.red_partial = nullptr; st.red_cap = 0; }
    ASORA_HIP_TRY(hipMalloc(&st.red_partial, sizeof(double) * entries));
    st.red_cap = entries;
    return 0;
}

}

using namespace asora;

extern "C" {

int asora_chemistry_device(double dt, double bh00, double albpow, double colh0, double temph0, double abu_c,
                           int *conv_flag, double *sum_xh1, double *sum_xh0)
{
    clear_error();
    if (int rc = require_init("chemistry_device")) return rc;
    State &st = state();
    if (int rc = require_grids("chemistry_device", {ASORA_GRID_NDENS, ASORA_GRID_TEMP, ASORA_GRID_XH, ASORA_GRID_XH_AV, ASORA_GRID_PHI_ION})) return rc;
    if (st.th_on) {
        if (!st.grid[ASORA_GRID_PHI_HEAT] || !st.grid_valid[ASORA_GRID_PHI_HEAT])
            return fail(4, "chemistry_device: thermal mode needs the heating rates (ASORA_GRID_PHI_HEAT) on the device");
        if (int rc = ensure_optional_grid(ASORA_GRID_TEMP_END)) return rc;
    }
    st.grid_valid[ASORA_GRID_XH_INTERMED] = true;
    ChemParams p;
    p.ncell = st.ncell;
    p.dt = dt; p.bh00 = bh00; p.albpow = albpow; p.colh0 = colh0; p.temph0 = temph0; p.abu_c = abu_c;
    p.ndens = st.grid[ASORA_GRID_NDENS]; p.temp = st.grid[ASORA_GRID_TEMP]; p.xh = st.grid[ASORA_GRID_XH];
    p.phi = st.grid[ASORA_GRID_PHI_ION];
    p.xh_av = st.grid[ASORA_GRID_XH_AV]; p.xh_intermed = st.grid[ASORA_GRID_XH_INTERMED];
    p.red_partial = st.red_partial; p.red_final = st.red_final; p.red_blocks = st.red_blocks;
    if (st.th_on) {
        p.thermal = true; p.th = st.th;
        p.phi_heat = st.grid[ASORA_GRID_PHI_HEAT]; p.temp_end = st.grid[ASORA_GRID_TEMP_END]; p.th_stats = st.th_stats_dev;
        ASORA_HIP_TRY(hipMemsetAsync(st.th_stats_dev, 0, 3 * sizeof(unsigned long long), st.stream));
        st.grid_valid[ASORA_GRID_TEMP_END] = true;
    }
    if (int rc = launch_chemistry(st, p, st.stream)) return rc;
    return read_reductions(conv_flag, sum_xh1, sum_xh0);
}

int asora_chemistry_range(double dt, double bh00, double albpow, double colh0, double temph0, double abu_c,
                          int i_begin, int i_count, int first)
{
    clear_error();
    if (int rc = require_init("chemistry_range")) return rc;
    State &st = state();
    if (st.th_on) return fail(4, "chemistry_range: not available in thermal mode (single GPU: asora_chemistry_device or asora_evolve_*)");
    if (int rc = require_grids("chemistry_range", {ASORA_GRID_NDENS, ASORA_GRID_TEMP, ASORA_GRID_XH, ASORA_GRID_XH_AV, ASORA_GRID_PHI_ION})) return rc;
    st.grid_valid[ASORA_GRID_XH_INTERMED] = true;
    if (int rc = check_planes("chemistry_range", 4, "bad plane range", i_begin, i_count)) return rc;
    if (i_count == 0 && !first) return 0;
    if (i_count == 0) {
        ASORA_HIP_TRY(hipMemsetAsync(st.red_final, 0, sizeof(double) * 3, st.stream));
        return 0;
    }
    if (int rc = ensure_red_capacity(3 * chemistry_tile_blocks(st, st.N, i_count))) return rc;
    if (int rc = ensure_temp_probe(bh00, albpow, colh0, temph0)) return rc;
    const double chem[6] = {dt, bh00, albpow, colh0, temph0, abu_c};
    ChemTileParams p = chem_tile_common(i_begin, i_count, chem);
    p.xh_av_in = st.grid[ASORA_GRID_XH_AV];
    p.gamma = st.grid[ASORA_GRID_PHI_ION];
    p.accumulate = first ? 0 : 1;
    return launch_chemistry_tiles(st, p, st.stream);
}

int asora_chemistry_finish(int *conv_flag, double *sum_xh1, double *sum_xh0)
{
    clear_error();
    if (int rc = require_init("chemistry_finish")) return rc;
    return read_reductions(conv_flag, sum_xh1, sum_xh0);
}

void *asora_reduction_ptr(void) { return state().init ? (void *)state().red_final : nullptr; }

int c2ray_global_pass(double dt, const double *ndens, const double *temp, const double *xh, double *xh_av,
                      double *xh_intermed, const double *phi_ion, double bh00, double albpow, double colh0,
                      double temph0, double abu_c, int m1, int m2, int m3, int *conv_flag)
{
    clear_error();
    if (m1 < 1 || m2 < 1 || m3 < 1) return fail(3, "global_pass: bad mesh size");
    if (!ndens || !temp || !xh || !xh_av || !xh_intermed || !phi_ion) return fail(3, "global_pass: null grid");
    if (int rc = ensure_runtime()) return rc;
    State &st = state();
    const size_t ncell = (size_t)m1 * m2 * m3, bytes = ncell * sizeof(double);
    double *d[6] = {nullptr, nullptr, nullptr, nullptr, nullptr, nullptr};
    const double *h[6] = {ndens, temp, xh, xh_av, xh_intermed, phi_ion};
    int rc = 0;
    auto cleanup = [&]() { for (auto *q : d) if (q) (void)hipFree(q); };
    for (int g = 0; g < 6 && !rc; ++g) {
        hipError_t e = hipMalloc(&d[g], bytes);
        if (e == hipSuccess) e = hipMemcpyAsync(d[g], h[g], bytes, hipMemcpyHostToDevice, st.stream);
        if (e != hipSuccess) rc = fail(10, std::string("global_pass: ") + hipGetErrorString(e));
    }
    if (rc) { cleanup(); return rc; }
    ChemParams p;
    p.ncell = ncell;
    p.dt = dt; p.bh00 = bh00; p.albpow = albpow; p.colh0 = colh0; p.temph0 = temph0; p.abu_c = abu_c;
    p.ndens = d[0]; p.temp = d[1]; p.xh = d[2]; p.xh_av = d[3]; p.xh_intermed = d[4]; p.phi = d[5];
    p.red_partial = st.red_partial; p.red_final = st.red_final; p.red_blocks = st.red_blocks;
    rc = launch_chemistry(st, p, st.stream, false);
    if (!rc) {
        hipError_t e = hipMemcpyAsync(xh_av, d[3], bytes, hipMemcpyDeviceToHost, st.stream);
        if (e == hipSuccess) e = hipMemcpyAsync(xh_intermed, d[4], bytes, hipMemcpyDeviceToHost, st.stream);
        if (e == hipSuccess) e = hipMemcpyAsync(st.red_host, st.red_final, sizeof(double) * 3, hipMemcpyDeviceToHost, st.stream);
        if (e == hipSuccess) e = hipStreamSynchronize(st.stream);
        if (e != hipSuccess) rc = fail(10, std::string("global_pass: ") + hipGetErrorString(e));
    }
    if (!rc && conv_flag) *conv_flag = (int)st.red_host[2];
    cleanup();
    return rc;
}

int asora_thermal_params(int enable, double relative_denergy, double t_floor, int max_substeps, unsigned cooling_mask,
                         int compton, double t_cmb)
{
    clear_error();
    if (int rc = require_init("thermal_params")) return rc;
    State &st = state();
    if (!enable) { st.th_on = false; return 0; }
    if (!st.have_heat_tables || st.opt[ASORA_OPT_GREY_NOTABLES])
        return fail(4, "thermal_params: thermal mode needs heating tables on the device (heat_table_to_device) and table rates");
    if (!(relative_denergy > 0.0) || !(t_floor >= 0.0) || max_substeps < 1 || !(t_cmb >= 0.0) || cooling_mask > 31u)
        return fail(3, "thermal_params: need relative_denergy > 0, t_floor >= 0, max_substeps >= 1, t_cmb >= 0, cooling_mask < 32");
    if (!st.th_stats_dev) {
        ASORA_HIP_TRY(hipMalloc(&st.th_stats_dev, 3 * sizeof(unsigned long long)));
        ASORA_HIP_TRY(hipMemsetAsync(st.th_stats_dev, 0, 3 * sizeof(unsigned long long), st.stream));
    }
    st.th.relative_denergy = relative_denergy; st.th.t_floor = t_floor; st.th.max_substeps = max_substeps;
    st.th.cooling_mask = cooling_mask; st.th.compton = compton ? 1 : 0; st.th.t_cmb = t_cmb;
    st.th_on = true;
    return 0;
}

int asora_clumping(int mode, double constant)
{
    clear_error();
    State &st = state();
    if (mode == 0) { st.clump_mode = 0; st.clump_c = 1.0; return 0; }
    if (int rc = require_init("clumping")) return rc;
    if (mode == 1) {
        if (!(std::isfinite(constant) && constant > 0.0)) return fail(3, "clumping: the constant must be finite and > 0");
        st.clump_mode = 1; st.clump_c = constant;
        return 0;
    }
    if (mode == 2) {
        if (!st.grid[ASORA_GRID_CLUMP] || !st.grid_valid[ASORA_GRID_CLUMP])
            return fail(4, "clumping: mode 2 needs the factors on the device (asora_grid_to_device(ASORA_GRID_CLUMP, ...))");
        st.clump_mode = 2; st.clump_c = 1.0;
        return 0;
    }
    return fail(3, "clumping: mode must be 0 (off), 1 (constant) or 2 (per cell)");
}

int asora_lls_opacity(double n_const, double per_density)
{
    clear_error();
    State &st = state();
    if (!(std::isfinite(n_const) && n_const >= 0.0 && std::isfinite(per_density) && per_density >= 0.0))
        return fail(3, "lls_opacity: n_const and per_density must be finite and >= 0");
    if (n_const == 0.0 && per_density == 0.0) { st.lls_a = st.lls_b = 0.0; return 0; }
    if (int rc = require_init("lls_opacity")) return rc;
    if (st.opt[ASORA_OPT_GREY_NOTABLES])
        return fail(4, "lls_opacity: needs table rates (grey opacity, ASORA_OPT_GREY_NOTABLES, is on)");
    st.lls_a = n_const; st.lls_b = per_density;
    return 0;
}

int asora_get_lls_opacity(double *n_const, double *per_density)
{
    clear_error();
    if (n_const) *n_const = state().lls_a;
    if (per_density) *per_density = state().lls_b;
    return 0;
}

int asora_thermal_stats(long long *cells_max_substeps, long long *cells_floored, int *max_substeps_used)
{
    clear_error();
    if (int rc = require_init("thermal_stats")) return rc;
    State &st = state();
    unsigned long long h[3] = {0, 0, 0};
    if (st.th_stats_dev) {
        ASORA_HIP_TRY(hipMemcpyAsync(h, st.th_stats_dev, sizeof h, hipMemcpyDeviceToHost, st.stream));
        ASORA_HIP_TRY(hipStreamSynchronize(st.stream));
    }
    if (cells_max_substeps) *cells_max_substeps = (long long)h[0];
    if (cells_floored) *cells_floored = (long long)h[1];
    if (max_substeps_used) *max_substeps_used = (int)h[2];
    return 0;
}

}
```

pyc2ray_amd/csrc/evolve_api.hip:

```cpp
#include "asora_internal.hpp"

namespace asora {

static double *acc_pair(int set) { return state().acc + (size_t)set * 2 * state().ncell; }
static double *heat_pair(int set) { return state().heat_acc + (size_t)set * 2 * state().ncell; }

static int ensure_heat_acc()
{
    State &st = state();
    if (st.heat_acc) return 0;
    ASORA_HIP_TRY(hipMalloc(&st.heat_acc, 4 * st.ncell * sizeof(double)));
    ASORA_HIP_TRY(hipMemsetAsync(st.heat_acc, 0, 4 * st.ncell * sizeof(double), st.stream));
    st.heat_clean[0] = st.heat_clean[1] = true;
    return 0;
}

static int ensure_heat_outbox()
{
    State &st = state();
    if (st.heat_outbox) return 0;
    ASORA_HIP_TRY(hipMalloc(&st.heat_outbox, st.ncell * sizeof(double)));
    return 0;
}

static int zero_pairs_unless_clean(bool heating = false)
{
    State &st = state();
    const size_t pair_bytes = 2 * st.ncell * sizeof(double);
    if (heating) {
        for (int q = 0; q < 2; ++q)
            if (!st.heat_clean[q]) {
                ASORA_HIP_TRY(hipMemsetAsync(heat_pair(q), 0, pair_bytes, st.stream));
                st.heat_clean[q] = true;
            }
        return 0;
    }
    if (!st.ev_sets_known) { st.ev_clean[0] = st.ev_clean[1] = false; st.ev_sets_known = true; }
    if (st.ev_clean[0] && st.ev_clean[1]) return 0;
    ASORA_HIP_TRY(hipMemsetAsync(acc_pair(0), 0, 2 * pair_bytes, st.stream));
    st.ev_clean[0] = st.ev_clean[1] = true;
    return 0;
}

static int decide_reach_mask(int src_begin, int src_count, double R)
{
    State &st = state();
    State::ReachMask &rm = st.reach;
    static const int mode = []() { const char *v = getenv("ASORA_REACH_MASK"); return v ? atoi(v) : 1; }();
    const bool possible = mode != 0 && std::isfinite(R) && 2.0 * R + 2.0 < (double)st.N && st.opt[ASORA_OPT_Z_TRANSPOSED] != 0;
    const State::ReachMask::Key now{true, st.src_generation, src_begin, src_count, R};
    const bool same = rm.key == now;
    const bool covers = possible && mode != 2 && (double)src_count * (4.0 / 3.0) * 3.14159265358979 * R * R * R >= (double)st.ncell;
    if (possible && !same) {
        if (covers) rm.pays = false;
        else {
            const size_t one = (size_t)st.N * st.N * ((st.N + 7) / 8);
            if (!rm.mask) { ASORA_HIP_TRY(hipMalloc(&rm.mask, 2 * one)); rm.bytes = one; }
            if (!rm.count_dev) ASORA_HIP_TRY(hipMalloc(&rm.count_dev, sizeof(unsigned long long)));
            if (int rc = launch_reach_mask(st, st.src_pos, src_begin, src_count, R, rm.mask, one)) return rc;
            if (int rc = launch_reach_count(st, rm.mask, 2 * one, rm.count_dev)) return rc;
            unsigned long long marked = 0;
            ASORA_HIP_TRY(hipMemcpyAsync(&marked, rm.count_dev, sizeof marked, hipMemcpyDeviceToHost, st.stream));
            ASORA_HIP_TRY(hipStreamSynchronize(st.stream));
            rm.pays = (double)marked <= 0.55 * (double)(2 * one);
        }
        rm.key = now;
    }
    const bool wanted = possible && (rm.pays || mode == 2);
    if ((wanted && !same) || (wanted != rm.in_use))
        if (int rc = zero_pairs_unless_clean()) return rc;
    rm.in_use = wanted;
    return 0;
}

static ChemTileParams evolve_pass_params(int i_begin, int i_count, int set)
{
    State &st = state();
    ChemTileParams c = chem_tile_common(i_begin, i_count, st.ev_chem);
    c.xh_av_in = st.ev_first ? st.grid[ASORA_GRID_XH] : st.grid[ASORA_GRID_XH_AV];
    c.gamma = acc_pair(set); c.gamma_t = c.gamma + st.ncell;
    c.zero_a = acc_pair(set ^ 1); c.zero_t = c.zero_a + st.ncell;
    c.nhi = st.nhi; c.nhi_t = st.nhi_t;
    c.status = st.ev_status;
    c.fold = true; c.emit = true;
    return c;
}

static void evolve_pass_thermal(ChemTileParams &c, int set)
{
    State &st = state();
    c.thermal = true; c.uniform = 0; c.th = st.th;
    c.heat = heat_pair(set); c.heat_t = c.heat + st.ncell;
    c.zero_ha = heat_pair(set ^ 1); c.zero_ht = c.zero_ha + st.ncell;
    c.temp_end = st.grid[ASORA_GRID_TEMP_END]; c.th_stats = st.th_stats_dev;
}

}

using namespace asora;

extern "C" {

static int evolve_begin_impl(double dt, double bh00, double albpow, double colh0, double temph0, double abu_c,
                             double R, double sig, double dr, double minlogtau, double dlogtau, int NumTau,
                             int src_begin, int src_count, double conv_criterion, double convergence_fraction,
                             bool slab, int own_begin, int own_count, bool slab_thermal = false)
{
    clear_error();
    if (int rc = require_init("evolve_begin")) return rc;
    State &st = state();
    st.ev_open = false;
    if (slab && st.th_on && !slab_thermal)
        return fail(4, "evolve_begin_slab: thermal mode is on, and this entry begins an isothermal step (single-GPU thermal loop: "
                       "asora_evolve_begin; across ranks, with the heating rates exchanged as well: asora_evolve_begin_slab_thermal)");
    if (slab_thermal && (!st.have_heat_tables || st.opt[ASORA_OPT_GREY_NOTABLES]))
        return fail(4, "evolve_begin_slab_thermal: needs heating tables on the device (heat_table_to_device)");
    if (slab_thermal && !st.th_on)
        return fail(4, "evolve_begin_slab_thermal: needs the thermal mode (asora_thermal_params(1, ...) first)");
    if (slab) {
        if (int rc = check_planes("evolve_begin_slab", 4, "bad range of own planes", own_begin, own_count)) return rc;
        if (!st.opt[ASORA_OPT_Z_TRANSPOSED]) return fail(4, "evolve_begin_slab: needs the [k][j][i] twins (ASORA_OPT_Z_TRANSPOSED = 1)");
    }
    if (int rc = require_grids("evolve_begin", {ASORA_GRID_NDENS, ASORA_GRID_TEMP, ASORA_GRID_XH})) return rc;
    if (int rc = require_raytrace_inputs("evolve_begin", R, NumTau, false, false)) return rc;
    if (int rc = check_sources("evolve_begin", 4, "source range outside the " + std::to_string(st.num_src) + " uploaded sources", src_begin, src_count)) return rc;
    if (st.opt[ASORA_OPT_HEATING]) return fail(4, "evolve_begin: the fused loop carries no heating rates (use raytrace_device)");
    if (st.th_on) {
        if (!st.have_heat_tables || st.opt[ASORA_OPT_GREY_NOTABLES])
            return fail(4, "evolve_begin: thermal mode needs heating tables on the device (heat_table_to_device)");
        if (!st.opt[ASORA_OPT_Z_TRANSPOSED]) return fail(4, "evolve_begin: thermal mode needs the [k][j][i] twins (ASORA_OPT_Z_TRANSPOSED = 1)");
        if (int rc = ensure_optional_grid(ASORA_GRID_PHI_HEAT)) return rc;
        if (int rc = ensure_optional_grid(ASORA_GRID_TEMP_END)) return rc;
        if (int rc = ensure_heat_acc()) return rc;
        if (slab) { if (int rc = ensure_heat_outbox()) return rc; }
    }
    if (int rc = ensure_temp_probe(bh00, albpow, colh0, temph0)) return rc;

    if (!st.ev_sets_known || slab)
        if (int rc = zero_pairs_unless_clean()) return rc;
    if (slab) st.reach.in_use = false;
    else if (int rc = decide_reach_mask(src_begin, src_count, R)) return rc;

    if (!st.ev_clean[0] && !st.ev_clean[1]) return fail(11, "evolve_begin: no clean accumulator pair (internal error)");
    st.ev_base = st.ev_clean[0] ? 0 : 1;
    if (st.th_on) {
        if (int rc = zero_pairs_unless_clean(true)) return rc;
        ASORA_HIP_TRY(hipMemsetAsync(st.th_stats_dev, 0, 3 * sizeof(unsigned long long), st.stream));
    }
    st.ev_folded_iter = 0;
    if (!st.ev_status) {
        ASORA_HIP_TRY(hipMalloc(&st.ev_status, sizeof(EvolveStatus)));
        ASORA_HIP_TRY(hipHostMalloc(&st.ev_host, sizeof(EvolveStatus), hipHostMallocDefault));
    }
    ASORA_HIP_TRY(hipStreamSynchronize(st.stream));
    std::memset(st.ev_host, 0, sizeof(EvolveStatus));
    st.ev_host->prev1 = 2.0 * (double)st.ncell;
    st.ev_host->prev0 = 2.0 * (double)st.ncell;
    st.ev_host->conv_criterion = conv_criterion;
    st.ev_host->conv_fraction = convergence_fraction;
    ASORA_HIP_TRY(hipMemcpyAsync(st.ev_status, st.ev_host, sizeof(EvolveStatus), hipMemcpyHostToDevice, st.stream));
    if (int rc = reset_counters()) return rc;
    if (int rc = launch_prepare_nhi_from(st, st.grid[ASORA_GRID_XH], st.opt[ASORA_OPT_Z_TRANSPOSED] != 0)) return rc;

    fill_rt_params(st.ev_rt, R, sig, dr, minlogtau, dlogtau, NumTau);
    st.ev_rt.phi = acc_pair(st.ev_base);
    st.ev_rt.done_flag = &st.ev_status->done;
    st.ev_rt.src_begin = src_begin; st.ev_rt.src_count = src_count; st.ev_rt.shape_src_count = src_count;
    if (src_begin == 0 && src_count == st.num_src && st.src_pos_sorted) use_source_list(st.ev_rt, st, true);
    st.ev_src_begin = src_begin; st.ev_src_count = src_count;
    st.ev_chem[0] = dt; st.ev_chem[1] = bh00; st.ev_chem[2] = albpow; st.ev_chem[3] = colh0; st.ev_chem[4] = temph0;
    st.ev_chem[5] = abu_c;
    st.ev_first = true;
    st.ev_reported = 0;
    st.ev_enqueued = 0;
    st.ev_slab = slab; st.ev_own_begin = own_begin; st.ev_own_count = own_count; st.ev_slab_passed = false;
    st.ev_slab_thermal = slab && st.th_on;
    st.ev_rates_in_outbox = false; st.ev_folded_all = false;
    st.ev_open = true;
    return 0;
}

int asora_evolve_begin(double dt, double bh00, double albpow, double colh0, double temph0, double abu_c,
                       double R, double sig, double dr, double minlogtau, double dlogtau, int NumTau,
                       int src_begin, int src_count, double conv_criterion, double convergence_fraction)
{
    return evolve_begin_impl(dt, bh00, albpow, colh0, temph0, abu_c, R, sig, dr, minlogtau, dlogtau, NumTau, src_begin, src_count,
                             conv_criterion, convergence_fraction, false, 0, 0);
}

int asora_evolve_begin_slab(double dt, double bh00, double albpow, double colh0, double temph0, double abu_c,
                            double R, double sig, double dr, double minlogtau, double dlogtau, int NumTau,
                            int src_begin, int src_count, double conv_criterion, double convergence_fraction,
                            int own_begin, int own_count)
{
    return evolve_begin_impl(dt, bh00, albpow, colh0, temph0, abu_c, R, sig, dr, minlogtau, dlogtau, NumTau, src_begin, src_count,
                             conv_criterion, convergence_fraction, true, own_begin, own_count);
}

int asora_evolve_begin_slab_thermal(double dt, double bh00, double albpow, double colh0, double temph0, double abu_c,
                                    double R, double sig, double dr, double minlogtau, double dlogtau, int NumTau,
                                    int src_begin, int src_count, double conv_criterion, double convergence_fraction,
                                    int own_begin, int own_count)
{
    return evolve_begin_impl(dt, bh00, albpow, colh0, temph0, abu_c, R, sig, dr, minlogtau, dlogtau, NumTau, src_begin, src_count,
                             conv_criterion, convergence_fraction, true, own_begin, own_count, true);
}

static int require_slab(const char *who)
{
    if (int rc = require_init(who)) return rc;
    if (!state().ev_open || !state().ev_slab)
        return fail(4, std::string(who) + ": no multi-GPU evolve step in progress (call asora_evolve_begin_slab)");
    if (state().ev_enqueued - state().ev_reported + 1 > EVOLVE_HIST)
        return fail(4, std::string(who) + ": " + std::to_string(EVOLVE_HIST) + " iterations enqueued since the last asora_evolve_poll (poll first)");
    return 0;
}
static int slab_set() { return (state().ev_base + state().ev_enqueued) & 1; }
static double *slab_pair(int which) { return acc_pair(slab_set() ^ which); }
static double *slab_heat_pair(int which) { return heat_pair(slab_set() ^ which); }
static int require_slab_thermal(const char *who)
{
    if (int rc = require_slab(who)) return rc;
    if (!state().ev_slab_thermal)
        return fail(4, std::string(who) + ": the step carries no heating rates (begin it with asora_evolve_begin_slab_thermal)");
    return 0;
}

int asora_evolve_slab_trace(int src_begin, int src_count)
{
    clear_error();
    if (int rc = require_slab("evolve_slab_trace")) return rc;
    State &st = state();
    if (st.ev_slab_passed) return fail(4, "evolve_slab_trace: the iteration's pass has been enqueued already (close it first)");
    if (src_begin < st.ev_src_begin || src_count < 0 || src_begin + src_count > st.ev_src_begin + st.ev_src_count)
        return fail(4, "evolve_slab_trace: source range outside the step's sources");
    if (src_count == 0) return 0;
    st.ev_sets_known = false;
    RtParams p = st.ev_rt;
    p.phi = slab_pair(0);
    p.src_begin = src_begin; p.src_count = src_count;
    if (!(src_begin == 0 && src_count == st.num_src)) use_source_list(p, st, false);
    if (st.ev_slab_thermal) {
        p.heat = slab_heat_pair(0);
        st.heat_clean[0] = st.heat_clean[1] = false;
    }
    return launch_raytrace(st, p, false, st.ev_slab_thermal);
}

int asora_evolve_slab_fold_out(int i_begin, int i_count)
{
    clear_error();
    if (int rc = require_slab("evolve_slab_fold_out")) return rc;
    State &st = state();
    if (int rc = check_planes("evolve_slab_fold_out", 4, "bad plane range", i_begin, i_count)) return rc;
    if (i_count > 0 && i_begin < st.ev_own_begin + st.ev_own_count && st.ev_own_begin < i_begin + i_count)
        return fail(4, "evolve_slab_fold_out: the range holds planes this rank owns (their rates stay: the pass folds them)");
    st.ev_sets_known = false;
    double *cur = slab_pair(0), *nxt = slab_pair(1);
    if (st.ev_slab_thermal) {
        double *hcur = slab_heat_pair(0), *hnxt = slab_heat_pair(1);
        return launch_fold_out_pair(st, cur, cur + st.ncell, st.staging, nxt, nxt + st.ncell, hcur, hcur + st.ncell, st.heat_outbox,
                                    hnxt, hnxt + st.ncell, i_begin, i_count, &st.ev_status->done);
    }
    return launch_fold_out(st, cur, cur + st.ncell, st.staging, nxt, nxt + st.ncell, i_begin, i_count, &st.ev_status->done);
}

int asora_evolve_slab_fold_all(void)
{
    clear_error();
    if (int rc = require_slab("evolve_slab_fold_all")) return rc;
    State &st = state();
    if (st.ev_slab_passed) return fail(4, "evolve_slab_fold_all: the iteration's pass has been enqueued already");
    if (st.ev_own_begin != 0 || st.ev_own_count != st.N)
        return fail(4, "evolve_slab_fold_all: the step must own every plane (asora_evolve_begin_slab(..., 0, N)): the chemistry is replicated");
    st.ev_sets_known = false;
    st.ev_rates_in_outbox = true; st.ev_folded_all = true;
    double *cur = slab_pair(0), *nxt = slab_pair(1);
    if (st.ev_slab_thermal) {
        double *hcur = slab_heat_pair(0), *hnxt = slab_heat_pair(1);
        return launch_fold_out_pair(st, cur, cur + st.ncell, st.staging, nullptr, nxt + st.ncell, hcur, hcur + st.ncell, st.heat_outbox,
                                    nullptr, hnxt + st.ncell, 0, st.N, &st.ev_status->done);
    }
    return launch_fold_out(st, cur, cur + st.ncell, st.staging, nullptr, nxt + st.ncell, 0, st.N, &st.ev_status->done);
}

void *asora_evolve_slab_outbox(void) { return state().init ? (void *)state().staging : nullptr; }
void *asora_evolve_slab_heat_outbox(void) { return state().init ? (void *)state().heat_outbox : nullptr; }

static int outbox_copy(const char *who, double *box, int i_begin, int i_count, double *host, bool to_host)
{
    clear_error();
    if (int rc = require_init(who)) return rc;
    State &st = state();
    if (i_begin < 0 || i_count < 0 || i_begin + i_count > st.N || (i_count > 0 && !host)) return fail(3, std::string(who) + ": bad arguments");
    if (i_count == 0) return 0;
    if (!box) return fail(4, std::string(who) + ": no heating out-box (begin a step with asora_evolve_begin_slab_thermal)");
    const size_t plane = (size_t)st.N * st.N;
    double *dev = box + (size_t)i_begin * plane;
    if (to_host) ASORA_HIP_TRY(hipMemcpyAsync(host, dev, (size_t)i_count * plane * sizeof(double), hipMemcpyDeviceToHost, st.stream));
    else         ASORA_HIP_TRY(hipMemcpyAsync(dev, host, (size_t)i_count * plane * sizeof(double), hipMemcpyHostToDevice, st.stream));
    ASORA_HIP_TRY(hipStreamSynchronize(st.stream));
    return 0;
}

int asora_evolve_slab_outbox_from_host(int i_begin, int i_count, const double *host)
{
    return outbox_copy("evolve_slab_outbox_from_host", state().staging, i_begin, i_count, const_cast<double *>(host), false);
}

int asora_evolve_slab_outbox_to_host(int i_begin, int i_count, double *host)
{
    return outbox_copy("evolve_slab_outbox_to_host", state().staging, i_begin, i_count, host, true);
}

int asora_evolve_slab_heat_outbox_from_host(int i_begin, int i_count, const double *host)
{
    return outbox_copy("evolve_slab_heat_outbox_from_host", state().heat_outbox, i_begin, i_count, const_cast<double *>(host), false);
}

int asora_evolve_slab_heat_outbox_to_host(int i_begin, int i_count, double *host)
{
    return outbox_copy("evolve_slab_heat_outbox_to_host", state().heat_outbox, i_begin, i_count, host, true);
}

static int slab_add(const char *who, bool heating, int i_begin, int i_count, const double *dev_planes)
{
    clear_error();
    if (int rc = heating ? require_slab_thermal(who) : require_slab(who)) return rc;
    State &st = state();
    if (i_begin < 0 || i_count < 0 || i_begin + i_count > st.N || (i_count > 0 && !dev_planes)) return fail(4, std::string(who) + ": bad arguments");
    if (st.ev_slab_passed) return fail(4, std::string(who) + ": the iteration's pass has been enqueued already");
    if (i_count > 0 && (i_begin < st.ev_own_begin || i_begin + i_count > st.ev_own_begin + st.ev_own_count))
        return fail(4, std::string(who) + ": rates received for planes this rank does not own");
    st.ev_sets_known = false;
    const size_t plane = (size_t)st.N * st.N;
    double *pair = heating ? slab_heat_pair(0) : slab_pair(0);
    return launch_add_planes(st, pair + (size_t)i_begin * plane, dev_planes, (size_t)i_count * plane, &st.ev_status->done);
}

static int slab_add_host(const char *who, bool heating, int i_begin, int i_count, const double *host_planes)
{
    clear_error();
    if (int rc = heating ? require_slab_thermal(who) : require_slab(who)) return rc;
    State &st = state();
    if (i_begin < 0 || i_count < 0 || i_begin + i_count > st.N || (i_count > 0 && !host_planes)) return fail(4, std::string(who) + ": bad arguments");
    if (i_count == 0) return 0;
    const size_t plane = (size_t)st.N * st.N;
    double *tmp = (heating ? st.heat_outbox : st.staging) + (size_t)i_begin * plane;
    ASORA_HIP_TRY(hipMemcpyAsync(tmp, host_planes, (size_t)i_count * plane * sizeof(double), hipMemcpyHostToDevice, st.stream));
    ASORA_HIP_TRY(hipStreamSynchronize(st.stream));
    return slab_add(who, heating, i_begin, i_count, tmp);
}

int asora_evolve_slab_add(int i_begin, int i_count, const double *dev_planes)
{
    return slab_add("evolve_slab_add", false, i_begin, i_count, dev_planes);
}

int asora_evolve_slab_add_host(int i_begin, int i_count, const double *host_planes)
{
    return slab_add_host("evolve_slab_add_host", false, i_begin, i_count, host_planes);
}

int asora_evolve_slab_add_heat(int i_begin, int i_count, const double *dev_planes)
{
    return slab_add("evolve_slab_add_heat", true, i_begin, i_count, dev_planes);
}

int asora_evolve_slab_add_heat_host(int i_begin, int i_count, const double *host_planes)
{
    return slab_add_host("evolve_slab_add_heat_host", true, i_begin, i_count, host_planes);
}

int asora_evolve_slab_pass(void)
{
    clear_error();
    if (int rc = require_slab("evolve_slab_pass")) return rc;
    State &st = state();
    if (st.ev_slab_passed) return fail(4, "evolve_slab_pass: already enqueued for this iteration");
    if (st.ev_rates_in_outbox && !st.ev_folded_all)
        return fail(4, "evolve_slab_pass: this step exchanges whole grids (asora_evolve_slab_fold_all), and this iteration's fold has not been enqueued");
    st.ev_sets_known = false;
    st.ev_slab_passed = true;
    st.grid_valid[ASORA_GRID_XH_AV] = st.grid_valid[ASORA_GRID_XH_INTERMED] = true;
    st.grid_valid[ASORA_GRID_PHI_ION] = false;
    if (st.ev_slab_thermal) {
        st.heat_clean[0] = st.heat_clean[1] = false;
        st.grid_valid[ASORA_GRID_TEMP_END] = true;
        st.grid_valid[ASORA_GRID_PHI_HEAT] = false;
    }
    if (st.ev_own_count == 0) {
        ASORA_HIP_TRY(hipMemsetAsync(st.red_final, 0, sizeof(double) * 3, st.stream));
        return 0;
    }
    if (int rc = ensure_red_capacity(3 * chemistry_tile_blocks(st, st.N, st.ev_own_count))) return rc;
    ChemTileParams c = evolve_pass_params(st.ev_own_begin, st.ev_own_count, slab_set());
    c.local_sums = true;
    if (st.ev_slab_thermal) evolve_pass_thermal(c, slab_set());
    if (st.ev_rates_in_outbox) {
        c.gamma = st.staging; c.gamma_t = nullptr; c.phi_out = st.grid[ASORA_GRID_PHI_ION]; c.fold = false;
        if (st.ev_slab_thermal) { c.heat = st.heat_outbox; c.heat_t = nullptr; c.heat_out = st.grid[ASORA_GRID_PHI_HEAT]; }
    }
    return launch_chemistry_tiles(st, c, st.stream);
}

int asora_evolve_slab_nhi(int i_begin, int i_count)
{
    clear_error();
    if (int rc = require_slab("evolve_slab_nhi")) return rc;
    State &st = state();
    if (int rc = check_planes("evolve_slab_nhi", 4, "bad plane range", i_begin, i_count)) return rc;
    return launch_prepare_range(st, i_begin, i_count, false, nullptr, &st.ev_status->done);
}

int asora_evolve_slab_close(const double *host_sums)
{
    clear_error();
    if (int rc = require_slab("evolve_slab_close")) return rc;
    State &st = state();
    if (!st.ev_slab_passed) return fail(4, "evolve_slab_close: the iteration's pass has not been enqueued");
    if (host_sums) {
        ASORA_HIP_TRY(hipStreamSynchronize(st.stream));
        std::memcpy(st.red_host, host_sums, sizeof(double) * 3);
        ASORA_HIP_TRY(hipMemcpyAsync(st.red_final, st.red_host, sizeof(double) * 3, hipMemcpyHostToDevice, st.stream));
    }
    if (int rc = launch_convergence_test(st, st.red_final, st.ev_status)) return rc;
    st.ev_first = false;
    st.ev_slab_passed = false; st.ev_folded_all = false;
    st.ev_enqueued += 1;
    return 0;
}

int asora_evolve_enqueue(int iterations)
{
    clear_error();
    if (int rc = require_init("evolve_enqueue")) return rc;
    State &st = state();
    if (!st.ev_open) return fail(4, "evolve_enqueue: no evolve step in progress (call asora_evolve_begin)");
    if (st.ev_slab) return fail(4, "evolve_enqueue: the step was begun with asora_evolve_begin_slab (use the asora_evolve_slab_* calls)");
    if (iterations < 1 || iterations > EVOLVE_HIST / 2) return fail(3, "evolve_enqueue: between 1 and 32 iterations per call");
    if (st.ev_enqueued - st.ev_reported + iterations > EVOLVE_HIST)
        return fail(4, "evolve_enqueue: " + std::to_string(st.ev_enqueued - st.ev_reported) + " iterations enqueued since the last "
                           "asora_evolve_poll; the history ring holds " + std::to_string(EVOLVE_HIST) + " (poll first)");
    st.ev_sets_known = false;
    for (int it = 0; it < iterations; ++it) {
        const int set = (st.ev_base + st.ev_enqueued + it) & 1;
        if (st.ev_src_count > 0) {
            RtParams p = st.ev_rt;
            p.phi = acc_pair(set);
            if (st.th_on) p.heat = heat_pair(set);
            if (int rc = launch_raytrace(st, p, false, st.th_on)) return rc;
        }
        ChemTileParams c = evolve_pass_params(0, st.N, set);
        if (st.reach.in_use) { c.reach_a = st.reach.mask; c.reach_t = st.reach.mask + st.reach.bytes; }
        if (st.th_on) evolve_pass_thermal(c, set);
        if (int rc = launch_chemistry_tiles(st, c, st.stream)) return rc;
        st.ev_first = false;
    }
    if (st.th_on) {
        st.heat_clean[0] = st.heat_clean[1] = false;
        st.grid_valid[ASORA_GRID_TEMP_END] = true;
        st.grid_valid[ASORA_GRID_PHI_HEAT] = false;
    }
    st.ev_enqueued += iterations;
    st.grid_valid[ASORA_GRID_XH_AV] = st.grid_valid[ASORA_GRID_XH_INTERMED] = true;
    st.grid_valid[ASORA_GRID_PHI_ION] = false;
    return 0;
}

int asora_evolve_poll(int *niter, int *converged, double *history, int history_rows, int *rows_written)
{
    clear_error();
    if (int rc = require_init("evolve_poll")) return rc;
    State &st = state();
    if (!st.ev_open) return fail(4, "evolve_poll: no evolve step in progress (call asora_evolve_begin)");
    ASORA_HIP_TRY(hipMemcpyAsync(st.ev_host, st.ev_status, sizeof(EvolveStatus), hipMemcpyDeviceToHost, st.stream));
    ASORA_HIP_TRY(hipStreamSynchronize(st.stream));
    const EvolveStatus &h = *st.ev_host;
    const bool thermal = st.ev_slab ? st.ev_slab_thermal : st.th_on;
    if (h.niter > 0) {
        const int set = (st.ev_base + h.niter - 1) & 1;
        if (st.ev_slab && st.ev_rates_in_outbox) st.ev_folded_iter = h.niter;
        if (st.ev_folded_iter != h.niter) {
            const double *a = acc_pair(set);
            if (int rc = launch_fold_sum(st, a, a + st.ncell, st.grid[ASORA_GRID_PHI_ION])) return rc;
            if (thermal) {
                const double *hsum = heat_pair(set);
                if (int rc = launch_fold_sum(st, hsum, hsum + st.ncell, st.grid[ASORA_GRID_PHI_HEAT])) return rc;
            }
            st.ev_folded_iter = h.niter;
        }
        st.grid_valid[ASORA_GRID_PHI_ION] = true;
        st.ev_clean[set] = false; st.ev_clean[set ^ 1] = true;
        if (thermal) {
            st.grid_valid[ASORA_GRID_PHI_HEAT] = true;
            st.heat_clean[set] = false; st.heat_clean[set ^ 1] = true;
        }
    }
    st.ev_sets_known = true;
    int rows = 0;
    for (int it = st.ev_reported; it < h.niter && history && rows < history_rows; ++it, ++rows)
        for (int q = 0; q < 5; ++q) history[5 * rows + q] = h.hist[it % EVOLVE_HIST][q];
    st.ev_enqueued = h.niter;
    if (history) st.ev_reported += rows;
    else st.ev_reported = h.niter;
    if (rows_written) *rows_written = rows;
    if (niter) *niter = h.niter;
    if (converged) *converged = h.done;
    return 0;
}

}
```

pyc2ray_amd/csrc/grids_api.hip:

```cpp
#include "asora_internal.hpp"
#include "rates_device.hpp"


namespace asora {

int ensure_optional_grid(int which)
{
    State &st = state();
    if ((which != ASORA_GRID_PHI_HEAT && which != ASORA_GRID_TEMP_END && which != ASORA_GRID_CLUMP) || st.grid[which]) return 0;
    const bool twin = which == ASORA_GRID_PHI_HEAT;
    ASORA_HIP_TRY(hipMalloc(&st.grid[which], (twin ? 2 : 1) * st.ncell * sizeof(double)));
    if (twin) st.heat_t = st.grid[which] + st.ncell;
    st.grid_valid[which] = false;
    return 0;
}

}

using namespace asora;

extern "C" {

int asora_grid_to_device(int which, const double *host, int N, char order)
{
    clear_error();
    if (int rc = require_init("grid_to_device")) return rc;
    if (int rc = check_N("grid_to_device", N)) return rc;
    if (which < 0 || which >= ASORA_GRID_COUNT) return fail(3, "grid_to_device: bad grid selector");
    if (!host) return fail(3, "grid_to_device: null host pointer");
    State &st = state();
    if (int rc = ensure_optional_grid(which)) return rc;
    st.zero_since_probe = std::max(st.zero_since_probe, 48);
    const size_t bytes = st.ncell * sizeof(double);
    if (order == 'C' || order == 'c') {
        ASORA_HIP_TRY(hipMemcpyAsync(st.grid[which], host, bytes, hipMemcpyHostToDevice, st.stream));
    } else if (order == 'F' || order == 'f') {
        ASORA_HIP_TRY(hipMemcpyAsync(st.staging, host, bytes, hipMemcpyHostToDevice, st.stream));
        if (int rc = launch_transpose(st, st.staging, st.grid[which], N)) return rc;
    } else
        return fail(3, "grid_to_device: order must be 'C' or 'F'");
    ASORA_HIP_TRY(hipStreamSynchronize(st.stream));
    st.grid_valid[which] = true;
    if (which == ASORA_GRID_TEMP) st.temp_probe_valid = false;
    return 0;
}

int asora_grid_to_host(int which, double *host, int N, char order)
{
    clear_error();
    if (int rc = require_init("grid_to_host")) return rc;
    if (int rc = check_N("grid_to_host", N)) return rc;
    if (which < 0 || which >= ASORA_GRID_COUNT) return fail(3, "grid_to_host: bad grid selector");
    if (!host) return fail(3, "grid_to_host: null host pointer");
    State &st = state();
    if (!st.grid[which] || !st.grid_valid[which]) return fail(3, "grid_to_host: grid " + std::to_string(which) + " holds no data");
    const size_t bytes = st.ncell * sizeof(double);
    if (order == 'C' || order == 'c') {
        ASORA_HIP_TRY(hipMemcpyAsync(host, st.grid[which], bytes, hipMemcpyDeviceToHost, st.stream));
    } else if (order == 'F' || order == 'f') {
        if (int rc = launch_transpose(st, st.grid[which], st.staging, N)) return rc;
        ASORA_HIP_TRY(hipMemcpyAsync(host, st.staging, bytes, hipMemcpyDeviceToHost, st.stream));
    } else
        return fail(3, "grid_to_host: order must be 'C' or 'F'");
    ASORA_HIP_TRY(hipStreamSynchronize(st.stream));
    return 0;
}

int asora_grid_copy(int dst, int src)
{
    clear_error();
    if (int rc = require_init("grid_copy")) return rc;
    if (dst < 0 || dst >= ASORA_GRID_COUNT || src < 0 || src >= ASORA_GRID_COUNT || dst == src)
        return fail(3, "grid_copy: bad grid selectors");
    State &st = state();
    if (!st.grid_valid[src]) return fail(3, "grid_copy: source grid holds no data");
    if (int rc = ensure_optional_grid(dst)) return rc;
    ASORA_HIP_TRY(hipMemcpyAsync(st.grid[dst], st.grid[src], st.ncell * sizeof(double), hipMemcpyDeviceToDevice,
                                 st.stream));
    st.grid_valid[dst] = true;
    if (dst == ASORA_GRID_TEMP) st.temp_probe_valid = false;
    return 0;
}

int asora_grid_scale(int which, double factor)
{
    clear_error();
    if (int rc = require_init("grid_scale")) return rc;
    if (which < 0 || which >= ASORA_GRID_COUNT) return fail(3, "grid_scale: bad grid selector");
    State &st = state();
    if (!st.grid_valid[which]) return fail(3, "grid_scale: grid " + std::to_string(which) + " holds no data");
    if (int rc = launch_scale(st, st.grid[which], st.ncell, factor)) return rc;
    if (which == ASORA_GRID_TEMP) st.temp_probe_valid = false;
    return 0;
}

int asora_grid_sum(int which, double *sum)
{
    clear_error();
    if (int rc = require_init("grid_sum")) return rc;
    if (which < 0 || which >= ASORA_GRID_COUNT) return fail(3, "grid_sum: bad grid selector");
    if (!sum) return fail(3, "grid_sum: null output pointer");
    State &st = state();
    if (!st.grid_valid[which]) return fail(3, "grid_sum: grid " + std::to_string(which) + " holds no data");
    if (!st.temp_probe_dev) ASORA_HIP_TRY(hipMalloc(&st.temp_probe_dev, sizeof(double) * 8));
    if (int rc = launch_grid_sum(st, st.grid[which], st.ncell, st.temp_probe_dev + 5)) return rc;
    ASORA_HIP_TRY(hipMemcpyAsync(sum, st.temp_probe_dev + 5, sizeof(double), hipMemcpyDeviceToHost, st.stream));
    ASORA_HIP_TRY(hipStreamSynchronize(st.stream));
    return 0;
}

int asora_host_alloc(size_t bytes, void **host)
{
    clear_error();
    if (!host || bytes == 0) return fail(3, "host_alloc: null pointer or zero size");
    *host = nullptr;
    ASORA_HIP_TRY(hipHostMalloc(host, bytes, hipHostMallocDefault));
    return 0;
}

int asora_host_free(void *host)
{
    clear_error();
    if (!host) return 0;
    ASORA_HIP_TRY(hipHostFree(host));
    return 0;
}

void *asora_device_ptr(int which)
{
    if (!state().init || which < 0 || which >= ASORA_GRID_COUNT) return nullptr;
    return state().grid[which];
}

int asora_density_to_device(const double *ndens, int N)
{
    return asora_grid_to_device(ASORA_GRID_NDENS, ndens, N, 'C');
}

static size_t rate_block_entries(int NumTau) { return std::max<size_t>(4 * (size_t)NumTau, 16); }

static int upload_rate_tables(const char *who, int NumSpec, int NumTau, const double *thin, const double *thick, const double *heat_thin,
                              const double *heat_thick)
{
    State &st = state();
    const bool heat = heat_thin && heat_thick;
    if (heat) { if (int rc = ensure_optional_grid(ASORA_GRID_PHI_HEAT)) return rc; }
    st.zero_since_probe = std::max(st.zero_since_probe, 48);
    if (st.tables) { (void)hipFree(st.tables); st.tables = nullptr; }
    st.table_len = 0; st.num_spec = 1; st.spec_stride = 0; st.have_heat_tables = false;
    const size_t block = rate_block_entries(NumTau);
    std::vector<double2> pairs(block * (size_t)NumSpec, double2{0.0, 0.0});
    for (int k = 0; k < NumSpec; ++k) {
        double2 *b = pairs.data() + block * (size_t)k;
        pack_rate_table(b, 0, thick + (size_t)k * NumTau, NumTau);
        pack_rate_table(b, 1, thin + (size_t)k * NumTau, NumTau);
        if (heat) {
            pack_rate_table(b, 2, heat_thick + (size_t)k * NumTau, NumTau);
            pack_rate_table(b, 3, heat_thin + (size_t)k * NumTau, NumTau);
        }
    }
    (void)who;
    ASORA_HIP_TRY(hipMalloc(&st.tables, pairs.size() * sizeof(double2)));
    ASORA_HIP_TRY(hipMemcpy(st.tables, pairs.data(), pairs.size() * sizeof(double2), hipMemcpyHostToDevice));
    st.table_len = NumTau;
    st.num_spec = NumSpec;
    st.spec_stride = block;
    st.have_heat_tables = heat;
    return 0;
}

int asora_photo_table_to_device(const double *thin_table, const double *thick_table, int NumTau)
{
    clear_error();
    if (int rc = require_init("photo_table_to_device")) return rc;
    if (NumTau < 1 || !thin_table || !thick_table) return fail(3, "photo_table_to_device: empty table");
    return upload_rate_tables("photo_table_to_device", 1, NumTau, thin_table, thick_table, nullptr, nullptr);
}

int asora_heat_table_to_device(const double *heat_thin_table, const double *heat_thick_table, int NumTau)
{
    clear_error();
    if (int rc = require_init("heat_table_to_device")) return rc;
    State &st = state();
    if (!st.tables) return fail(4, "heat_table_to_device: upload the photo tables first (photo_table_to_device)");
    if (st.num_spec != 1)
        return fail(4, "heat_table_to_device: " + std::to_string(st.num_spec) + " table sets are on the device; their heating tables go "
                       "up with them (spectra_to_device)");
    if (NumTau != st.table_len || !heat_thin_table || !heat_thick_table)
        return fail(3, "heat_table_to_device: the heating tables must have the length of the photo tables (" +
                           std::to_string(st.table_len) + ")");
    if (int rc = ensure_optional_grid(ASORA_GRID_PHI_HEAT)) return rc;
    std::vector<double2> pairs(4 * (size_t)NumTau, double2{0.0, 0.0});
    pack_rate_table(pairs.data(), 2, heat_thick_table, NumTau);
    pack_rate_table(pairs.data(), 3, heat_thin_table, NumTau);
    const size_t lo = rate_table_byte_offset(2, NumTau), hi = rate_table_byte_offset(4, NumTau);
    ASORA_HIP_TRY(hipMemcpy(reinterpret_cast<char *>(st.tables) + lo, reinterpret_cast<const char *>(pairs.data()) + lo, hi - lo,
                            hipMemcpyHostToDevice));
    st.have_heat_tables = true;
    return 0;
}

int asora_spectra_to_device(int NumSpec, int NumTau, const double *photo_thin, const double *photo_thick, const double *heat_thin,
                            const double *heat_thick)
{
    clear_error();
    if (int rc = require_init("spectra_to_device")) return rc;
    if (NumSpec < 1 || NumSpec > ASORA_MAX_SPECTRA)
        return fail(3, "spectra_to_device: NumSpec=" + std::to_string(NumSpec) + " outside [1, " + std::to_string(ASORA_MAX_SPECTRA) + "]");
    if (NumTau < 1 || !photo_thin || !photo_thick) return fail(3, "spectra_to_device: empty table");
    if ((heat_thin == nullptr) != (heat_thick == nullptr)) return fail(3, "spectra_to_device: one heating table without the other");
    return upload_rate_tables("spectra_to_device", NumSpec, NumTau, photo_thin, photo_thick, heat_thin, heat_thick);
}

int asora_num_spectra(void) { return state().tables ? state().num_spec : 0; }

}

namespace asora {

void sort_sources_by_position(const int32_t *pos, int NumSrc, std::vector<int> &order)
{
    order.resize((size_t)std::max(NumSrc, 0));
    for (int s = 0; s < NumSrc; ++s) order[s] = s;
    std::stable_sort(order.begin(), order.end(), [pos](int a, int b) {
        if (pos[3 * a] != pos[3 * b]) return pos[3 * a] < pos[3 * b];
        if (pos[3 * a + 1] != pos[3 * b + 1]) return pos[3 * a + 1] < pos[3 * b + 1];
        return pos[3 * a + 2] < pos[3 * b + 2];
    });
}

static void drop_source_spectra(State &st)
{
    if (st.src_spec) { (void)hipFree(st.src_spec); st.src_spec = nullptr; }
    if (st.src_spec_sorted) { (void)hipFree(st.src_spec_sorted); st.src_spec_sorted = nullptr; }
    st.src_spec_max = 0;
}

int check_source_spectra(const char *who)
{
    State &st = state();
    if (!st.src_spec) return 0;
    if (st.opt[ASORA_OPT_GREY_NOTABLES])
        return fail(4, std::string(who) + ": grey opacity uses no tables, so sources cannot have table sets of their own "
                                          "(source_spectra_to_device with zeros, or ASORA_OPT_GREY_NOTABLES = 0)");
    if (st.src_spec_max >= st.num_spec)
        return fail(4, std::string(who) + ": a source has table set " + std::to_string(st.src_spec_max) + " but the device holds " +
                           std::to_string(st.num_spec) + " (spectra_to_device)");
    return 0;
}

}

extern "C" {

int asora_source_data_to_device(const int32_t *pos, const double *flux, int NumSrc)
{
    clear_error();
    if (int rc = require_init("source_data_to_device")) return rc;
    if (NumSrc < 0 || (NumSrc > 0 && (!pos || !flux))) return fail(3, "source_data_to_device: bad arguments");
    State &st = state();
    st.zero_since_probe = std::max(st.zero_since_probe, 48);
    for (int s = 0; s < NumSrc; ++s)
        for (int ax = 0; ax < 3; ++ax)
            if (pos[3 * s + ax] < 0 || pos[3 * s + ax] >= st.N)
                return fail(3, "source_data_to_device: source " + std::to_string(s) + " lies outside the mesh (0-based " +
                                   std::to_string(pos[3 * s + ax]) + " on axis " + std::to_string(ax) + ")");
    if (st.src_pos) { (void)hipFree(st.src_pos); st.src_pos = nullptr; }
    if (st.src_flux) { (void)hipFree(st.src_flux); st.src_flux = nullptr; }
    if (st.src_pos_sorted) { (void)hipFree(st.src_pos_sorted); st.src_pos_sorted = nullptr; }
    if (st.src_flux_sorted) { (void)hipFree(st.src_flux_sorted); st.src_flux_sorted = nullptr; }
    drop_source_spectra(st);
    st.src_i0_sorted.clear();
    st.src_pos_host.clear(); st.src_pos_sorted_host.clear();
    release_pair_lists(st);
    st.num_src = 0;
    if (NumSrc == 0) return 0;
    ASORA_HIP_TRY(hipMalloc(&st.src_pos, sizeof(int32_t) * 3 * (size_t)NumSrc));
    ASORA_HIP_TRY(hipMalloc(&st.src_flux, sizeof(double) * (size_t)NumSrc));
    ASORA_HIP_TRY(hipMemcpy(st.src_pos, pos, sizeof(int32_t) * 3 * (size_t)NumSrc, hipMemcpyHostToDevice));
    ASORA_HIP_TRY(hipMemcpy(st.src_flux, flux, sizeof(double) * (size_t)NumSrc, hipMemcpyHostToDevice));
    {
        std::vector<int> order;
        sort_sources_by_position(pos, NumSrc, order);
        std::vector<int32_t> ps(3 * (size_t)NumSrc);
        std::vector<double> fs((size_t)NumSrc);
        st.src_i0_sorted.resize((size_t)NumSrc);
        for (int s = 0; s < NumSrc; ++s) {
            const int o = order[s];
            ps[3 * s] = pos[3 * o]; ps[3 * s + 1] = pos[3 * o + 1]; ps[3 * s + 2] = pos[3 * o + 2];
            fs[s] = flux[o];
            st.src_i0_sorted[s] = pos[3 * o];
        }
        ASORA_HIP_TRY(hipMalloc(&st.src_pos_sorted, sizeof(int32_t) * 3 * (size_t)NumSrc));
        ASORA_HIP_TRY(hipMalloc(&st.src_flux_sorted, sizeof(double) * (size_t)NumSrc));
        ASORA_HIP_TRY(hipMemcpy(st.src_pos_sorted, ps.data(), sizeof(int32_t) * 3 * (size_t)NumSrc, hipMemcpyHostToDevice));
        ASORA_HIP_TRY(hipMemcpy(st.src_flux_sorted, fs.data(), sizeof(double) * (size_t)NumSrc, hipMemcpyHostToDevice));
        st.src_pos_sorted_host.swap(ps);
    }
    st.src_pos_host.assign(pos, pos + 3 * (size_t)NumSrc);
    st.num_src = NumSrc;
    st.src_generation += 1;
    return 0;
}

int asora_source_spectra_to_device(const int32_t *spec, int NumSrc)
{
    clear_error();
    if (int rc = require_init("source_spectra_to_device")) return rc;
    State &st = state();
    if (NumSrc != st.num_src)
        return fail(3, "source_spectra_to_device: " + std::to_string(NumSrc) + " table sets for the " + std::to_string(st.num_src) +
                           " sources on the device (source_data_to_device first)");
    drop_source_spectra(st);
    if (!spec || NumSrc == 0) return 0;
    const int limit = st.tables ? st.num_spec : ASORA_MAX_SPECTRA;
    int top = 0;
    for (int s = 0; s < NumSrc; ++s) {
        if (spec[s] < 0 || spec[s] >= limit)
            return fail(3, "source_spectra_to_device: source " + std::to_string(s) + " has table set " + std::to_string(spec[s]) +
                               ", outside [0, " + std::to_string(limit) + ")");
        top = std::max(top, (int)spec[s]);
    }
    if (top == 0) return 0;
    std::vector<int> order;
    sort_sources_by_position(st.src_pos_host.data(), NumSrc, order);
    std::vector<int32_t> sorted((size_t)NumSrc);
    for (int s = 0; s < NumSrc; ++s) sorted[s] = spec[order[s]];
    ASORA_HIP_TRY(hipMalloc(&st.src_spec, sizeof(int32_t) * (size_t)NumSrc));
    ASORA_HIP_TRY(hipMalloc(&st.src_spec_sorted, sizeof(int32_t) * (size_t)NumSrc));
    ASORA_HIP_TRY(hipMemcpy(st.src_spec, spec, sizeof(int32_t) * (size_t)NumSrc, hipMemcpyHostToDevice));
    ASORA_HIP_TRY(hipMemcpy(st.src_spec_sorted, sorted.data(), sizeof(int32_t) * (size_t)NumSrc, hipMemcpyHostToDevice));
    st.src_spec_max = top;
    return 0;
}

int asora_debug_sort_sources(const int32_t *pos, const double *flux, const int32_t *spec, int NumSrc, int32_t *pos_out,
                             double *flux_out, int32_t *spec_out)
{
    clear_error();
    if (NumSrc < 0 || (NumSrc > 0 && (!pos || !flux || !pos_out || !flux_out))) return fail(3, "debug_sort_sources: bad arguments");
    std::vector<int> order;
    sort_sources_by_position(pos, NumSrc, order);
    for (int s = 0; s < NumSrc; ++s) {
        const int o = order[s];
        for (int ax = 0; ax < 3; ++ax) pos_out[3 * s + ax] = pos[3 * o + ax];
        flux_out[s] = flux[o];
        if (spec && spec_out) spec_out[s] = spec[o];
    }
    return 0;
}

int asora_planes_to_host(int which, int i_begin, int i_count, double *host)
{
    clear_error();
    if (int rc = require_init("planes_to_host")) return rc;
    State &st = state();
    if (which < 0 || which >= ASORA_GRID_COUNT) return fail(3, "planes_to_host: bad grid selector");
    if (int rc = check_planes("planes_to_host", 3, "bad plane range", i_begin, i_count)) return rc;
    if (i_count == 0) return 0;
    if (!host) return fail(3, "planes_to_host: null host pointer");
    if (!st.grid_valid[which]) return fail(3, "planes_to_host: grid " + std::to_string(which) + " holds no data");
    const size_t plane = (size_t)st.N * st.N;
    ASORA_HIP_TRY(hipMemcpyAsync(host, st.grid[which] + (size_t)i_begin * plane, (size_t)i_count * plane * sizeof(double),
                                 hipMemcpyDeviceToHost, st.stream));
    ASORA_HIP_TRY(hipStreamSynchronize(st.stream));
    return 0;
}

int asora_planes_to_device(int which, int i_begin, int i_count, const double *host)
{
    clear_error();
    if (int rc = require_init("planes_to_device")) return rc;
    State &st = state();
    if (which < 0 || which >= ASORA_GRID_COUNT) return fail(3, "planes_to_device: bad grid selector");
    if (int rc = check_planes("planes_to_device", 3, "bad plane range", i_begin, i_count)) return rc;
    if (i_count == 0) return 0;
    if (!host) return fail(3, "planes_to_device: null host pointer");
    if (int rc = ensure_optional_grid(which)) return rc;
    const size_t plane = (size_t)st.N * st.N;
    ASORA_HIP_TRY(hipMemcpyAsync(st.grid[which] + (size_t)i_begin * plane, host, (size_t)i_count * plane * sizeof(double),
                                 hipMemcpyHostToDevice, st.stream));
    ASORA_HIP_TRY(hipStreamSynchronize(st.stream));
    st.grid_valid[which] = true;
    if (which == ASORA_GRID_TEMP) st.temp_probe_valid = false;
    return 0;
}

}
```

pyc2ray_amd/csrc/raytrace_api.hip:

```cpp
#include "asora_internal.hpp"

namespace asora {

int reset_counters()
{
    State &st = state();
    ASORA_HIP_TRY(hipMemsetAsync(st.counters, 0, sizeof(unsigned long long) * COUNTER_FIELDS * COUNTER_SLOTS, st.stream));
    return 0;
}

int require_raytrace_inputs(const char *who, double R, int NumTau, bool density, bool xh_av)
{
    State &st = state();
    const std::string w = std::string(who) + ": ";
    if (int rc = check_open_boundaries(st, who, st.opt[ASORA_OPT_OPEN_BOUNDARIES] != 0, false)) return rc;
    if (density && !st.grid_valid[ASORA_GRID_NDENS]) return fail(4, w + "density not on device (density_to_device)");
    if (xh_av && !st.grid_valid[ASORA_GRID_XH_AV]) return fail(4, w + "xh_av not on device");
    if (!st.opt[ASORA_OPT_GREY_NOTABLES] && !st.tables) return fail(4, w + "radiation tables not on device (photo_table_to_device)");
    if (!(R >= 0.0)) return fail(4, w + "R must be >= 0");
    if (NumTau < 1 && !st.opt[ASORA_OPT_GREY_NOTABLES]) return fail(4, w + "NumTau must be >= 1");
    return check_source_spectra(who);
}

static int check_rt_sources(int src_begin, int src_count)
{
    return check_sources("raytrace", 4, "source range [" + std::to_string(src_begin) + "," + std::to_string(src_begin + src_count) +
                         ") outside the " + std::to_string(state().num_src) + " uploaded sources (source_data_to_device)", src_begin, src_count);
}

void fill_rt_params(RtParams &p, double R, double sig, double dr, double minlogtau, double dlogtau, int NumTau, int radius_path)
{
    State &st = state();
    std::memset(&p, 0, sizeof p);
    p.N = st.N;
    p.R = R; p.sig = sig; p.dr = dr;
    p.minlogtau = minlogtau; p.dlogtau = dlogtau;
    p.table_len = st.table_len > 0 ? st.table_len : 1;
    p.NumTau = NumTau; p.numtau_f = lut_index_limit(NumTau, p.table_len);
    p.fortran_consts = st.opt[ASORA_OPT_FORTRAN_CONSTANTS];
    p.grey = st.opt[ASORA_OPT_GREY_NOTABLES];
    p.z_transposed = st.opt[ASORA_OPT_Z_TRANSPOSED] != 0 ? 1 : 0;
    p.ncell = (unsigned)st.ncell;
    p.nhi = st.nhi;
    p.phi = st.grid[ASORA_GRID_PHI_ION];
    p.tables = st.tables;
    p.heat = st.grid[ASORA_GRID_PHI_HEAT];
    p.spec_stride = (unsigned)st.spec_stride;
    use_source_list(p, st, false);
    p.counters = st.counters;
    p.radius_stays = note_call_radius(st, R, radius_path) ? 1 : 0;
    p.open_bc = st.opt[ASORA_OPT_OPEN_BOUNDARIES] != 0 ? 1 : 0;
}

static int rt_begin(double R, double sig, double dr, double minlogtau, double dlogtau, int NumTau, double *dump,
                    bool pipelined = false)
{
    State &st = state();
    st.rt_open = false;
    if (int rc = require_raytrace_inputs("raytrace", R, NumTau, true, true)) return rc;

    const bool zt = st.opt[ASORA_OPT_Z_TRANSPOSED] != 0;
    const bool heat = st.opt[ASORA_OPT_HEATING] != 0 && dump == nullptr;
    if (heat && (!st.have_heat_tables || st.opt[ASORA_OPT_GREY_NOTABLES]))
        return fail(4, "raytrace: heating requested but no heating tables on device (heat_table_to_device)");
    const size_t bytes = st.ncell * sizeof(double);
    ASORA_HIP_TRY(hipMemsetAsync(st.grid[ASORA_GRID_PHI_ION], 0, bytes, st.stream));
    if (zt) ASORA_HIP_TRY(hipMemsetAsync(st.phi_t, 0, bytes, st.stream));
    if (heat) {
        ASORA_HIP_TRY(hipMemsetAsync(st.grid[ASORA_GRID_PHI_HEAT], 0, bytes, st.stream));
        if (zt) ASORA_HIP_TRY(hipMemsetAsync(st.heat_t, 0, bytes, st.stream));
    }
    if (int rc = reset_counters()) return rc;
    if (int rc = launch_prepare_nhi(st, zt)) return rc;

    RtParams &p = st.rt_params;
    fill_rt_params(p, R, sig, dr, minlogtau, dlogtau, NumTau);
    p.dump = dump;
    st.rt_heat = heat;
    st.rt_pipelined = pipelined;
    st.rt_by_planes = false;
    if (pipelined) {
        ASORA_HIP_TRY(hipEventRecord(st.main_ready, st.stream));
        for (int q = 0; q < 2; ++q) {
            ASORA_HIP_TRY(hipStreamWaitEvent(st.side[q], st.main_ready, 0));
            st.side_pending[q] = false;
        }
        st.side_next = 0;
    }
    st.rt_open = true;
    return 0;
}

static int rt_range(int src_begin, int src_count)
{
    State &st = state();
    if (!st.rt_open) return fail(4, "raytrace_range: no raytrace in progress (call asora_raytrace_begin)");
    if (int rc = check_rt_sources(src_begin, src_count)) return rc;
    if (src_count == 0) return 0;
    RtParams p = st.rt_params;
    use_source_list(p, st, src_begin == 0 && src_count == st.num_src && st.src_pos_sorted && !p.dump);
    p.src_begin = src_begin; p.src_count = src_count;
    p.shape_src_count = (st.rt_pipelined || st.rt_by_planes) ? st.num_src : src_count;
    if (!st.rt_pipelined) return launch_raytrace(st, p, p.dump != nullptr, st.rt_heat);
    const int q = st.side_next;
    st.side_next ^= 1;
    if (int rc = launch_raytrace(st, p, p.dump != nullptr, st.rt_heat, st.side[q])) return rc;
    ASORA_HIP_TRY(hipEventRecord(st.side_done[q], st.side[q]));
    st.side_pending[q] = true;
    return 0;
}

static int rt_fold(int i_begin, int i_count)
{
    State &st = state();
    if (!st.rt_open) return fail(4, "raytrace_fold: no raytrace in progress (call asora_raytrace_begin)");
    if (int rc = check_planes("raytrace_fold", 4, "bad plane range", i_begin, i_count)) return rc;
    for (int q = 0; q < 2; ++q)
        if (st.side_pending[q]) {
            ASORA_HIP_TRY(hipStreamWaitEvent(st.stream, st.side_done[q], 0));
            st.side_pending[q] = false;
        }
    if (st.rt_params.z_transposed && i_count > 0) {
        if (int rc = launch_fold_range(st, st.phi_t, st.grid[ASORA_GRID_PHI_ION], i_begin, i_count)) return rc;
        if (st.rt_heat)
            if (int rc = launch_fold_range(st, st.heat_t, st.grid[ASORA_GRID_PHI_HEAT], i_begin, i_count)) return rc;
    }
    st.grid_valid[ASORA_GRID_PHI_ION] = true;
    if (st.rt_heat) st.grid_valid[ASORA_GRID_PHI_HEAT] = true;
    return 0;
}

static int do_raytrace(double R, double sig, double dr, int src_begin, int src_count, double minlogtau,
                       double dlogtau, int NumTau, double *dump)
{
    State &st = state();
    if (int rc = check_rt_sources(src_begin, src_count)) return rc;
    if (int rc = rt_begin(R, sig, dr, minlogtau, dlogtau, NumTau, dump)) return rc;
    if (int rc = rt_range(src_begin, src_count)) return rc;
    if (int rc = rt_fold(0, st.N)) return rc;
    st.rt_open = false;
    return 0;
}

static int do_all_sources_pipelined(double R, double sig, double dr, const double *xh_av, double *phi_ion, int NumSrc,
                                    double minlogtau, double dlogtau, int NumTau, bool &done)
{
    State &st = state();
    done = false;
    const int N = st.N;
    constexpr int KMAX = 16;
    const char *kenv = getenv("ASORA_PIPELINE_SLABS");
    const int K = kenv ? std::max(2, std::min(KMAX, atoi(kenv))) : 8;
    if (!st.opt[ASORA_OPT_PIPELINED_COPIES] || !st.opt[ASORA_OPT_Z_TRANSPOSED] || st.opt[ASORA_OPT_HEATING]) return 0;
    if (NumSrc != st.num_src || NumSrc < 1 || !st.src_pos_sorted || N < 8 * K) return 0;
    if (!std::isfinite(R) || !(R >= 0.0)) return 0;
    const int m = (int)std::floor(R);
    if (2 * m + N / K >= N) return 0;
    if (int rc = require_raytrace_inputs("raytrace", R, NumTau, true, false)) return rc;

    const size_t bytes = st.ncell * sizeof(double);
    if (hipHostRegister((void *)xh_av, bytes, hipHostRegisterDefault) != hipSuccess) { (void)hipGetLastError(); return 0; }
    if (hipHostRegister((void *)phi_ion, bytes, hipHostRegisterDefault) != hipSuccess) {
        (void)hipGetLastError(); (void)hipHostUnregister((void *)xh_av); return 0;
    }
    struct Unpin {
        const void *a, *b;
        ~Unpin()
        {
            State &s = state();
            for (hipStream_t q : {s.side[0], s.side[1], s.stream}) if (q) (void)hipStreamSynchronize(q);
            (void)hipHostUnregister((void *)a); (void)hipHostUnregister((void *)b);
        }
    } unpin{xh_av, phi_ion};

    while ((int)st.pipe_events.size() < 2 * K) {
        hipEvent_t e = nullptr;
        ASORA_HIP_TRY(hipEventCreateWithFlags(&e, hipEventDisableTiming));
        st.pipe_events.push_back(e);
    }
    hipStream_t up = st.side[0], down = st.side[1];
    const size_t plane = (size_t)N * N;
    int lo[KMAX + 1];
    for (int c = 0; c <= K; ++c) lo[c] = c * N / K;
    int sb[KMAX + 1];
    for (int c = 0; c <= K; ++c)
        sb[c] = (int)(std::lower_bound(st.src_i0_sorted.begin(), st.src_i0_sorted.end(), lo[c]) - st.src_i0_sorted.begin());
    bool reach[KMAX][KMAX];
    for (int c = 0; c < K; ++c)
        for (int d = 0; d < K; ++d) {
            bool hit = false;
            if (sb[c + 1] > sb[c])
                for (int q = lo[d]; q < lo[d + 1] && !hit; ++q) {
                    int dist = 0;
                    if (q < lo[c]) dist = std::min(lo[c] - q, q + N - (lo[c + 1] - 1));
                    else if (q >= lo[c + 1]) dist = std::min(q - (lo[c + 1] - 1), lo[c] + N - q);
                    hit = dist <= m;
                }
            reach[c][d] = hit;
        }

    ASORA_HIP_TRY(hipMemsetAsync(st.grid[ASORA_GRID_PHI_ION], 0, 2 * bytes, st.stream));
    if (int rc = reset_counters()) return rc;
    RtParams base;
    fill_rt_params(base, R, sig, dr, minlogtau, dlogtau, NumTau);
    use_source_list(base, st, true);
    base.shape_src_count = NumSrc;
    st.rt_open = false;
    ASORA_HIP_TRY(hipEventRecord(st.main_ready, st.stream));
    ASORA_HIP_TRY(hipStreamWaitEvent(up, st.main_ready, 0));
    ASORA_HIP_TRY(hipStreamWaitEvent(down, st.main_ready, 0));

    bool prepped[KMAX] = {}, traced[KMAX] = {}, sent[KMAX] = {};
    auto try_traces = [&]() -> int {
        for (int c = 0; c < K; ++c) {
            if (traced[c]) continue;
            bool ready = true;
            for (int d = 0; d < K; ++d) if (reach[c][d] && !prepped[d]) ready = false;
            if (!ready) continue;
            if (sb[c + 1] > sb[c]) {
                RtParams p = base;
                p.src_begin = sb[c]; p.src_count = sb[c + 1] - sb[c];
                if (int rc = launch_raytrace(st, p, false, false)) return rc;
            }
            traced[c] = true;
        }
        return 0;
    };
    bool folded[KMAX] = {};
    std::vector<int> to_send;
    auto try_folds = [&]() -> int {
        for (int d = 0; d < K; ++d) {
            if (folded[d]) continue;
            bool final_ = true;
            for (int c = 0; c < K; ++c) if (reach[c][d] && !traced[c]) final_ = false;
            if (!final_) continue;
            if (int rc = launch_fold_range(st, st.phi_t, st.grid[ASORA_GRID_PHI_ION], lo[d], lo[d + 1] - lo[d])) return rc;
            ASORA_HIP_TRY(hipEventRecord(st.pipe_events[K + d], st.stream));
            folded[d] = true;
            to_send.push_back(d);
        }
        return 0;
    };
    auto send = [&](int d) -> int {
        ASORA_HIP_TRY(hipStreamWaitEvent(down, st.pipe_events[K + d], 0));
        ASORA_HIP_TRY(hipMemcpyAsync(phi_ion + (size_t)lo[d] * plane, st.grid[ASORA_GRID_PHI_ION] + (size_t)lo[d] * plane,
                                     (size_t)(lo[d + 1] - lo[d]) * plane * sizeof(double), hipMemcpyDeviceToHost, down));
        sent[d] = true;
        return 0;
    };
    int w = 0;
    for (int c = 0; c < K; ++c)
        for (int d = 0; d < K; ++d) {
            const int back = (c - d + K) % K;
            if (reach[c][d] && back <= K / 2) w = std::max(w, back);
        }
    for (int q = 0; q < K; ++q) {
        const int c = (q + K - w) % K;
        ASORA_HIP_TRY(hipMemcpyAsync(st.grid[ASORA_GRID_XH_AV] + (size_t)lo[c] * plane, xh_av + (size_t)lo[c] * plane,
                                     (size_t)(lo[c + 1] - lo[c]) * plane * sizeof(double), hipMemcpyHostToDevice, up));
        ASORA_HIP_TRY(hipEventRecord(st.pipe_events[c], up));
    }
    for (int q = 0; q < K; ++q) {
        const int c = (q + K - w) % K;
        ASORA_HIP_TRY(hipStreamWaitEvent(st.stream, st.pipe_events[c], 0));
        if (int rc = launch_prepare_range(st, lo[c], lo[c + 1] - lo[c], false, nullptr)) return rc;
        prepped[c] = true;
        const std::vector<int> ready = to_send;
        to_send.clear();
        if (int rc = try_traces()) return rc;
        if (int rc = try_folds()) return rc;
        for (int d : ready) if (int rc = send(d)) return rc;
    }
    for (int d : to_send) if (int rc = send(d)) return rc;
    for (int c = 0; c < K; ++c) if (!traced[c] || !sent[c]) return fail(11, "do_all_sources: pipeline schedule incomplete (internal error)");
    ASORA_HIP_TRY(hipStreamSynchronize(down));
    ASORA_HIP_TRY(hipStreamSynchronize(up));
    ASORA_HIP_TRY(hipStreamSynchronize(st.stream));
    st.grid_valid[ASORA_GRID_XH_AV] = true;
    st.grid_valid[ASORA_GRID_PHI_ION] = true;
    done = true;
    return 0;
}

}

using namespace asora;

extern "C" {

int asora_raytrace_device(double R, double sig, double dr, int src_begin, int src_count, double minlogtau,
                          double dlogtau, int NumTau)
{
    clear_error();
    if (int rc = require_init("raytrace_device")) return rc;
    return do_raytrace(R, sig, dr, src_begin, src_count, minlogtau, dlogtau, NumTau, nullptr);
}

int asora_raytrace_begin(double R, double sig, double dr, double minlogtau, double dlogtau, int NumTau)
{
    clear_error();
    if (int rc = require_init("raytrace_begin")) return rc;
    return rt_begin(R, sig, dr, minlogtau, dlogtau, NumTau, nullptr, true);
}

int asora_raytrace_begin_planes(double R, double sig, double dr, double minlogtau, double dlogtau, int NumTau,
                                const int *runs, int nruns)
{
    clear_error();
    if (int rc = require_init("raytrace_begin_planes")) return rc;
    State &st = state();
    st.rt_open = false;
    if (int rc = require_raytrace_inputs("raytrace_begin_planes", R, NumTau, true, true)) return rc;
    if (!st.opt[ASORA_OPT_Z_TRANSPOSED]) return fail(4, "raytrace_begin_planes: needs the [k][j][i] twins (ASORA_OPT_Z_TRANSPOSED = 1)");
    if (st.opt[ASORA_OPT_HEATING]) return fail(4, "raytrace_begin_planes: no heating rates on this path");
    if (nruns < 0 || (nruns > 0 && !runs)) return fail(3, "raytrace_begin_planes: bad plane runs");
    for (int q = 0; q < nruns; ++q)
        if (int rc = check_planes("raytrace_begin_planes", 3, "plane run outside the mesh", runs[2 * q], runs[2 * q + 1])) return rc;
    if (int rc = reset_counters()) return rc;
    for (int q = 0; q < nruns; ++q)
        if (int rc = launch_prepare_range(st, runs[2 * q], runs[2 * q + 1], true, st.grid[ASORA_GRID_PHI_ION])) return rc;
    fill_rt_params(st.rt_params, R, sig, dr, minlogtau, dlogtau, NumTau);
    st.rt_heat = false;
    st.rt_pipelined = false;
    st.rt_by_planes = true;
    st.rt_open = true;
    return 0;
}

int asora_raytrace_range(int src_begin, int src_count)
{
    clear_error();
    if (int rc = require_init("raytrace_range")) return rc;
    return rt_range(src_begin, src_count);
}

int asora_raytrace_fold(int i_begin, int i_count)
{
    clear_error();
    if (int rc = require_init("raytrace_fold")) return rc;
    return rt_fold(i_begin, i_count);
}

int asora_do_all_sources(double R, double *coldensh_out, double sig, double dr, const double *ndens,
                         const double *xh_av, double *phi_ion, int NumSrc, int m1, double minlogtau,
                         double dlogtau, int NumTau)
{
    (void)coldensh_out; (void)ndens;
    clear_error();
    if (int rc = require_init("do_all_sources")) return rc;
    if (int rc = check_N("do_all_sources", m1)) return rc;
    if (!xh_av || !phi_ion) return fail(3, "do_all_sources: null xh_av / phi_ion");
    State &st = state();
    if (NumSrc > st.num_src)
        return fail(3, "do_all_sources: NumSrc=" + std::to_string(NumSrc) + " exceeds the " +
                           std::to_string(st.num_src) + " sources on the device");
    const size_t bytes = st.ncell * sizeof(double);
    {
        bool done = false;
        if (int rc = do_all_sources_pipelined(R, sig, dr, xh_av, phi_ion, NumSrc, minlogtau, dlogtau, NumTau, done)) return rc;
        if (done) return 0;
    }
    ASORA_HIP_TRY(hipMemcpyAsync(st.grid[ASORA_GRID_XH_AV], xh_av, bytes, hipMemcpyHostToDevice, st.stream));
    st.grid_valid[ASORA_GRID_XH_AV] = true;
    if (int rc = do_raytrace(R, sig, dr, 0, NumSrc, minlogtau, dlogtau, NumTau, nullptr)) return rc;
    ASORA_HIP_TRY(hipMemcpyAsync(phi_ion, st.grid[ASORA_GRID_PHI_ION], bytes, hipMemcpyDeviceToHost, st.stream));
    ASORA_HIP_TRY(hipStreamSynchronize(st.stream));
    return 0;
}

int asora_last_raytrace_counts(long long *gamma_cells, long long *evaluated_cells)
{
    clear_error();
    if (int rc = require_init("last_raytrace_counts")) return rc;
    long long zero = 0;
    return asora_last_raytrace_counts_ex(gamma_cells, evaluated_cells, &zero);
}

int asora_last_raytrace_counts_ex(long long *gamma_cells, long long *evaluated_cells, long long *zero_rates_left_out)
{
    clear_error();
    if (int rc = require_init("last_raytrace_counts")) return rc;
    std::vector<unsigned long long> h((size_t)COUNTER_FIELDS * COUNTER_SLOTS, 0ULL);
    ASORA_HIP_TRY(hipStreamSynchronize(state().stream));
    ASORA_HIP_TRY(hipMemcpy(h.data(), state().counters, h.size() * sizeof(unsigned long long), hipMemcpyDeviceToHost));
    unsigned long long tot[COUNTER_FIELDS] = {0ULL, 0ULL, 0ULL};
    for (int q = 0; q < COUNTER_SLOTS; ++q) for (int f = 0; f < COUNTER_FIELDS; ++f) tot[f] += h[(size_t)COUNTER_FIELDS * q + f];
    if (gamma_cells) *gamma_cells = (long long)tot[0];
    if (evaluated_cells) *evaluated_cells = (long long)tot[1];
    if (zero_rates_left_out) *zero_rates_left_out = (long long)tot[2];
    return 0;
}

int asora_last_raytrace_variant(void) { return state().last_variant; }

int asora_debug_coldens(double R, double sig, double dr, int source_index, double *coldens_out, int N)
{
    clear_error();
    if (int rc = require_init("debug_coldens")) return rc;
    if (int rc = check_N("debug_coldens", N)) return rc;
    if (!coldens_out) return fail(3, "debug_coldens: null output");
    State &st = state();
    if (int rc = check_open_boundaries(st, "debug_coldens", st.opt[ASORA_OPT_OPEN_BOUNDARIES] != 0, true)) return rc;
    const size_t bytes = st.ncell * sizeof(double);
    ASORA_HIP_TRY(hipMemsetAsync(st.staging, 0, bytes, st.stream));
    const int numtau = st.table_len > 0 ? st.table_len : 1;
    const int grey_save = st.opt[ASORA_OPT_GREY_NOTABLES];
    if (!st.tables) { st.opt[ASORA_OPT_GREY_NOTABLES] = 1; st.coldens_only = true; }
    int rc = do_raytrace(R, sig, dr, source_index, 1, -20.0, 1.0, numtau, st.staging);
    st.opt[ASORA_OPT_GREY_NOTABLES] = grey_save; st.coldens_only = false;
    if (rc) return rc;
    ASORA_HIP_TRY(hipMemcpyAsync(coldens_out, st.staging, bytes, hipMemcpyDeviceToHost, st.stream));
    ASORA_HIP_TRY(hipStreamSynchronize(st.stream));
    return 0;
}

}
```

pyc2ray_amd/csrc/subbox_api.hip:

```cpp
#include "asora_internal.hpp"
#include "rates_device.hpp"


namespace asora {

struct SubboxCall {
    int max_subbox, subboxsize;
    float loss_fraction;
    double sig, dr, R, minlogtau, dlogtau;
    int NumTau, table_len;
    const double2 *tables;
    const int32_t *src_pos;
    const int32_t *host_pos;
    const double *src_flux;
    int src_begin, src_count;
    bool heat, keep_heat;
    double *dump;
};

static int refuse_source_spectra(const char *who)
{
    if (!state().src_spec) return 0;
    return fail(4, std::string(who) + ": the sub-box raytracer has one spectrum for all sources, and the sources on the device "
                                      "carry table sets of their own (source_spectra_to_device); use raytrace_device / evolve3D");
}

static int subbox_core(const SubboxCall &c, long long &total_nbox, double &total_loss)
{
    State &st = state();
    const int N = st.N;
    const size_t bytes = st.ncell * sizeof(double);
    const bool grey = st.opt[ASORA_OPT_GREY_NOTABLES] != 0;
    ASORA_HIP_TRY(hipMemsetAsync(st.grid[ASORA_GRID_PHI_ION], 0, 2 * bytes, st.stream));
    if (c.heat) {
        if (!c.keep_heat) ASORA_HIP_TRY(hipMemsetAsync(st.grid[ASORA_GRID_PHI_HEAT], 0, bytes, st.stream));
        ASORA_HIP_TRY(hipMemsetAsync(st.heat_t, 0, bytes, st.stream));
    }
    if (c.dump) ASORA_HIP_TRY(hipMemsetAsync(c.dump, 0, bytes, st.stream));
    if (int rc = launch_prepare_nhi(st, true)) return rc;
    if (int rc = ensure_logtab(st)) return rc;

    const int ext_r = std::min(c.max_subbox, N / 2 - 1 + N % 2);
    const int ext_l = std::min(c.max_subbox, N / 2);
    const int S_all = std::max(ext_r, ext_l);
    const bool range_open = ext_r > 0 && ext_l > 0;

    SubboxParams p;
    std::memset(&p, 0, sizeof p);
    p.N = N; p.W = std::max(S_all, 0) + 1;
    p.ext_r = ext_r; p.ext_l = ext_l;
    p.sig = c.sig; p.dr = c.dr; p.R = c.R;
    p.numtau_f = lut_index_limit(c.NumTau, c.table_len);
    p.lut_k1 = 0.30102999566398119521 / c.dlogtau;
    p.lut_k0 = 1.0 - c.minlogtau / c.dlogtau;
    p.table_len = c.table_len;
    p.grey = grey ? 1 : 0; p.heat = c.heat ? 1 : 0; p.add_zero = st.opt[ASORA_OPT_SKIP_ZERO_RATES] == 1 ? 0 : 1;
    const int last = c.src_begin + c.src_count - 1;
    p.flux_src = st.opt[ASORA_OPT_C2RAY_OWN_FLUX] ? -1 : last;
    p.dump_src = last;
    p.ncell = (unsigned)st.ncell;
    p.nhi = st.nhi; p.phi = st.grid[ASORA_GRID_PHI_ION]; p.heat_grid = st.grid[ASORA_GRID_PHI_HEAT];
    p.dump = c.dump;
    p.tables = c.tables; p.logtab = st.logtab_dev;
    p.src_pos = c.src_pos; p.src_flux = c.src_flux;
    p.unit_stride = (size_t)6 * p.W * p.W;

    total_nbox = 0;
    total_loss = 0.0;
    struct DropPairs { State &s; bool on; ~DropPairs() { if (on) release_pair_lists(s); } } drop_pairs{st, c.src_pos != st.src_pos};
    if (drop_pairs.on) release_pair_lists(st);
    RtParams tp;
    fill_rt_params(tp, c.R, c.sig, c.dr, c.minlogtau, c.dlogtau, c.NumTau, 1);
    tp.numtau_f = p.numtau_f; tp.lut_k1 = p.lut_k1; tp.lut_k0 = p.lut_k0; tp.tau_zero = INFINITY;
    tp.table_len = c.table_len; tp.tables = c.tables;
    tp.fortran_consts = 1; tp.grey = grey ? 1 : 0; tp.z_transposed = 1;
    tp.logtab = st.logtab_dev;
    tp.src_pos = c.src_pos; tp.src_flux = c.src_flux;
    tp.src_spec = nullptr;
    tp.flux_src = p.flux_src;
    const bool has_dump = c.dump != nullptr;
    SubboxTables tab;
    const int table_sources = c.src_count - (has_dump ? 1 : 0);
    {
        if (range_open && table_sources > 0)
            if (int rc = subbox_tables_prepare(st, tp, ext_r, ext_l, c.subboxsize, table_sources, c.heat, tab, c.host_pos)) return rc;
    }

    const size_t per_src = 8 * p.unit_stride * sizeof(double);
    const size_t budget = (size_t)4 << 30;
    const int max_batch = tab.ok ? (tab.max_batch >= table_sources ? std::max(c.src_count, 1) : tab.max_batch)
                                 : (int)std::max<size_t>(8, std::min<size_t>((budget / per_src) / 8 * 8, 1 << 20));
    const int cap = std::min(std::max(c.src_count, 1), max_batch);
    if ((size_t)cap > st.subbox_cap) {
        for (void *q : {(void *)st.sb_active, (void *)st.sb_nbox, (void *)st.sb_loss, (void *)st.sb_loss_final})
            if (q) (void)hipFree(q);
        st.sb_active = st.sb_nbox = nullptr; st.sb_loss = st.sb_loss_final = nullptr; st.subbox_cap = 0;
        ASORA_HIP_TRY(hipMalloc(&st.sb_active, sizeof(int) * cap));
        ASORA_HIP_TRY(hipMalloc(&st.sb_nbox, sizeof(int) * cap));
        ASORA_HIP_TRY(hipMalloc(&st.sb_loss, sizeof(double) * cap));
        ASORA_HIP_TRY(hipMalloc(&st.sb_loss_final, sizeof(double) * cap));
        st.subbox_cap = (size_t)cap;
    }
    if (!st.sb_nactive) ASORA_HIP_TRY(hipMalloc(&st.sb_nactive, sizeof(int)));
    std::vector<int> h_nbox((size_t)cap);
    std::vector<double> h_loss((size_t)cap);

    for (int done = 0; done < c.src_count;) {
        const int batch = std::min(c.src_count - done, max_batch);
        const bool dump_here = has_dump && done + batch == c.src_count;
        const int fly_count = tab.ok ? (dump_here ? 1 : 0) : batch;
        const int fly_first = tab.ok ? batch - fly_count : 0;
        const size_t need = (size_t)8 * ((std::max(fly_count, 1) + 7) / 8) * per_src;
        if (need > st.shell_scratch_bytes) {
            if (st.shell_scratch) ASORA_HIP_TRY(hipFree(st.shell_scratch));
            st.shell_scratch = nullptr; st.shell_scratch_bytes = 0;
            ASORA_HIP_TRY(hipMalloc(&st.shell_scratch, need));
            st.shell_scratch_bytes = need;
        }
        const int first = c.src_begin + done;
        p.scratch = st.shell_scratch;
        p.src_begin = first + fly_first; p.src_count = fly_count;
        p.active = st.sb_active + fly_first; p.loss = st.sb_loss + fly_first;
        tp.src_begin = first; tp.src_count = batch - fly_count;
        tp.sb_active = st.sb_active; tp.sb_loss = st.sb_loss;
        int n_active = 0;
        if (int rc = launch_subbox_decide(st, 0, batch, c.src_flux, first, (double)c.loss_fraction, range_open ? 1 : 0,
                                          st.sb_active, st.sb_loss, st.sb_loss_final, st.sb_nbox, st.sb_nactive)) return rc;
        ASORA_HIP_TRY(hipMemcpyAsync(&n_active, st.sb_nactive, sizeof(int), hipMemcpyDeviceToHost, st.stream));
        ASORA_HIP_TRY(hipStreamSynchronize(st.stream));
        long long box = 0;
        while (n_active > 0) {
            const long long prev_box = box;
            box += c.subboxsize;
            p.s_begin = (int)std::min<long long>(prev_box, S_all);
            p.s_end = (int)std::min<long long>(box, S_all);
            p.edge_r = (int)std::min<long long>(box, ext_r);
            p.edge_l = (int)std::min<long long>(box, ext_l);
            const bool beside = fly_count > 0 && tab.ok && tp.src_count > 0;
            if (beside) {
                ASORA_HIP_TRY(hipEventRecord(st.main_ready, st.stream));
                ASORA_HIP_TRY(hipStreamWaitEvent(st.side[0], st.main_ready, 0));
            }
            if (fly_count > 0) { if (int rc = launch_subbox_sweep(st, p, beside ? st.side[0] : nullptr)) return rc; }
            if (beside) ASORA_HIP_TRY(hipEventRecord(st.side_done[0], st.side[0]));
            if (tab.ok && tp.src_count > 0) {
                tp.sb_edge_r = p.edge_r; tp.sb_edge_l = p.edge_l;
                if (int rc = subbox_tables_sweep(st, tp, tab, p.s_begin, p.s_end, c.heat)) return rc;
            }
            if (beside) ASORA_HIP_TRY(hipStreamWaitEvent(st.stream, st.side_done[0], 0));
            const int more_range = (box < ext_r && box < ext_l) ? 1 : 0;
            if (int rc = launch_subbox_decide(st, 1, batch, c.src_flux, first, (double)c.loss_fraction, more_range,
                                              st.sb_active, st.sb_loss, st.sb_loss_final, st.sb_nbox, st.sb_nactive)) return rc;
            ASORA_HIP_TRY(hipMemcpyAsync(&n_active, st.sb_nactive, sizeof(int), hipMemcpyDeviceToHost, st.stream));
            ASORA_HIP_TRY(hipStreamSynchronize(st.stream));
        }
        ASORA_HIP_TRY(hipMemcpy(h_nbox.data(), st.sb_nbox, (size_t)batch * sizeof(int), hipMemcpyDeviceToHost));
        ASORA_HIP_TRY(hipMemcpy(h_loss.data(), st.sb_loss_final, (size_t)batch * sizeof(double), hipMemcpyDeviceToHost));
        for (int s = 0; s < batch; ++s) { total_nbox += h_nbox[s]; total_loss += h_loss[s]; }
        done += batch;
    }

    if (int rc = launch_finish_phi(st)) return rc;
    st.grid_valid[ASORA_GRID_PHI_ION] = true;
    if (c.heat) {
        if (int rc = launch_fold_transposed(st, st.heat_t, st.grid[ASORA_GRID_PHI_HEAT])) return rc;
        st.grid_valid[ASORA_GRID_PHI_HEAT] = true;
    }
    return 0;
}

}

namespace {
struct DeviceBuffers {
    std::vector<void *> ptrs;
    ~DeviceBuffers() { for (void *q : ptrs) (void)hipFree(q); }
    template <typename T> int alloc(T *&out, size_t count)
    {
        void *d = nullptr;
        ASORA_HIP_TRY(hipMalloc(&d, std::max<size_t>(count, 1) * sizeof(T)));
        ptrs.push_back(d);
        out = static_cast<T *>(d);
        return 0;
    }
};
}

using namespace asora;


extern "C" {

int c2ray_do_all_sources(const double *normflux, const int32_t *srcpos, int max_subbox, int subboxsize,
                         double *coldensh_out, double sig, double dr, const double *ndens, const double *xh_av,
                         double *phi_ion, double *phi_heat, float loss_fraction,
                         const double *photo_thin_table, const double *photo_thick_table,
                         const double *heat_thin_table, const double *heat_thick_table,
                         double minlogtau, double dlogtau, double R_max_LLS,
                         int NumTau, int NumSrc, int m1, int m2, int m3,
                         int *sum_nbox, double *photon_loss)
{
    clear_error();
    State &st = state();
    const char *who = "c2ray_do_all_sources";
    if (st.opt[ASORA_OPT_OPEN_BOUNDARIES])
        return fail(4, std::string(who) + ": open boundaries (ASORA_OPT_OPEN_BOUNDARIES) have no sub-box sweep (the reference's Fortran has no such mode)");
    if (m1 != m2 || m1 != m3) return fail(3, std::string(who) + ": the mesh must be cubic (raytracing.f90:174-175 use m1 for every axis)");
    if (NumSrc < 0 || (NumSrc > 0 && (!normflux || !srcpos))) return fail(3, std::string(who) + ": bad source arguments");
    if (!ndens || !xh_av || !phi_ion || !coldensh_out) return fail(3, std::string(who) + ": null grid");
    if (subboxsize < 1) return fail(3, std::string(who) + ": subboxsize must be >= 1");
    const bool grey = st.opt[ASORA_OPT_GREY_NOTABLES] != 0;
    if (!grey && (NumTau < 1 || !photo_thin_table || !photo_thick_table))
        return fail(3, std::string(who) + ": empty photo-ionisation tables");
    if (int rc = refuse_source_spectra(who)) return rc;
    bool heat = !grey && phi_heat && heat_thin_table && heat_thick_table;
    if (heat) {
        bool any = false;
        for (int i = 0; i < NumTau && !any; ++i) any = heat_thin_table[i] != 0.0 || heat_thick_table[i] != 0.0;
        heat = any;
    }
    if (int rc = asora_device_init_auto(m1)) return rc;
    const int N = st.N;
    for (int s = 0; s < NumSrc; ++s)
        for (int ax = 0; ax < 3; ++ax)
            if (srcpos[3 * s + ax] < 1 || srcpos[3 * s + ax] > N)
                return fail(3, std::string(who) + ": source " + std::to_string(s + 1) + " lies outside the mesh (1-based " +
                                   std::to_string(srcpos[3 * s + ax]) + " on axis " + std::to_string(ax + 1) + ")");

    DeviceBuffers tmp;
    const size_t bytes = st.ncell * sizeof(double);
    if (int rc = asora_grid_to_device(ASORA_GRID_NDENS, ndens, N, 'F')) return rc;
    if (int rc = asora_grid_to_device(ASORA_GRID_XH_AV, xh_av, N, 'F')) return rc;
    if (heat) { if (int rc = asora_grid_to_device(ASORA_GRID_PHI_HEAT, phi_heat, N, 'F')) return rc; }

    int32_t *d_pos = nullptr; double *d_flux = nullptr; double2 *d_tables = nullptr;
    std::vector<int32_t> host_pos0;
    if (NumSrc > 0) {
        host_pos0.resize(3 * (size_t)NumSrc);
        std::vector<int32_t> &pos0 = host_pos0;
        for (size_t q = 0; q < pos0.size(); ++q) pos0[q] = srcpos[q] - 1;
        if (int rc = tmp.alloc(d_pos, pos0.size())) return rc;
        if (int rc = tmp.alloc(d_flux, (size_t)NumSrc)) return rc;
        ASORA_HIP_TRY(hipMemcpy(d_pos, pos0.data(), pos0.size() * sizeof(int32_t), hipMemcpyHostToDevice));
        ASORA_HIP_TRY(hipMemcpy(d_flux, normflux, (size_t)NumSrc * sizeof(double), hipMemcpyHostToDevice));
    }
    const int len = grey ? 1 : NumTau;
    {
        std::vector<double2> pairs(std::max<size_t>(4 * (size_t)len, 16), double2{0.0, 0.0});
        const double *src[4] = {photo_thick_table, photo_thin_table, heat ? heat_thick_table : nullptr,
                                heat ? heat_thin_table : nullptr};
        for (int t = 0; t < 4 && !grey; ++t)
            if (src[t]) pack_rate_table(pairs.data(), t, src[t], len);
        if (int rc = tmp.alloc(d_tables, pairs.size())) return rc;
        ASORA_HIP_TRY(hipMemcpy(d_tables, pairs.data(), pairs.size() * sizeof(double2), hipMemcpyHostToDevice));
    }

    SubboxCall c;
    c.max_subbox = max_subbox; c.subboxsize = subboxsize; c.loss_fraction = loss_fraction;
    c.sig = sig; c.dr = dr; c.R = R_max_LLS; c.minlogtau = minlogtau; c.dlogtau = dlogtau; c.NumTau = NumTau;
    c.table_len = len; c.tables = d_tables; c.src_pos = d_pos; c.src_flux = d_flux;
    c.host_pos = host_pos0.empty() ? nullptr : host_pos0.data();
    c.src_begin = 0; c.src_count = NumSrc;
    c.heat = heat; c.keep_heat = true;
    c.dump = st.staging;
    long long total_nbox = 0;
    double total_loss = 0.0;
    if (int rc = subbox_core(c, total_nbox, total_loss)) return rc;

    if (int rc = launch_transpose(st, st.staging, st.nhi_t, N)) return rc;
    ASORA_HIP_TRY(hipMemcpyAsync(coldensh_out, st.nhi_t, bytes, hipMemcpyDeviceToHost, st.stream));
    if (int rc = asora_grid_to_host(ASORA_GRID_PHI_ION, phi_ion, N, 'F')) return rc;
    if (heat) { if (int rc = asora_grid_to_host(ASORA_GRID_PHI_HEAT, phi_heat, N, 'F')) return rc; }
    ASORA_HIP_TRY(hipStreamSynchronize(st.stream));
    if (sum_nbox) *sum_nbox = (int)total_nbox;
    if (photon_loss) *photon_loss = total_loss;
    return 0;
}

int asora_device_init_auto(int N)
{
    clear_error();
    State &st = state();
    if (!st.init || (st.auto_init && st.N != N)) {
        if (int rc = asora_device_init(N, 1)) return rc;
        st.auto_init = true;
        return 0;
    }
    return check_N("device_init_auto", N);
}

int asora_subbox_raytrace_device(int max_subbox, int subboxsize, float loss_fraction, double R_max_LLS, double sig, double dr,
                                 double minlogtau, double dlogtau, int NumTau, int src_begin, int src_count,
                                 int *sum_nbox, double *photon_loss)
{
    clear_error();
    if (int rc = require_init("subbox_raytrace_device")) return rc;
    State &st = state();
    const char *who = "subbox_raytrace_device";
    if (st.opt[ASORA_OPT_OPEN_BOUNDARIES])
        return fail(4, std::string(who) + ": open boundaries (ASORA_OPT_OPEN_BOUNDARIES) have no sub-box sweep (the reference's Fortran has no such mode)");
    if (!st.grid_valid[ASORA_GRID_NDENS]) return fail(4, std::string(who) + ": density not on device");
    if (!st.grid_valid[ASORA_GRID_XH_AV]) return fail(4, std::string(who) + ": xh_av not on device");
    if (subboxsize < 1) return fail(3, std::string(who) + ": subboxsize must be >= 1");
    const bool grey = st.opt[ASORA_OPT_GREY_NOTABLES] != 0;
    if (!grey && (!st.tables || NumTau < 1)) return fail(4, std::string(who) + ": radiation tables not on device");
    if (int rc = check_sources(who, 4, "source range outside the uploaded sources", src_begin, src_count)) return rc;
    if (int rc = refuse_source_spectra(who)) return rc;
    const bool heat = !grey && st.opt[ASORA_OPT_HEATING] != 0;
    if (heat && !st.have_heat_tables) return fail(4, std::string(who) + ": heating requested but no heating tables on device");
    SubboxCall c;
    c.max_subbox = max_subbox; c.subboxsize = subboxsize; c.loss_fraction = loss_fraction;
    c.sig = sig; c.dr = dr; c.R = R_max_LLS; c.minlogtau = minlogtau; c.dlogtau = dlogtau; c.NumTau = NumTau;
    c.table_len = st.table_len > 0 ? st.table_len : 1; c.tables = st.tables;
    c.src_pos = st.src_pos; c.src_flux = st.src_flux; c.src_begin = src_begin; c.src_count = src_count;
    c.host_pos = st.src_pos_host.empty() ? nullptr : st.src_pos_host.data();
    c.heat = heat; c.keep_heat = false; c.dump = nullptr;
    long long total_nbox = 0;
    double total_loss = 0.0;
    if (int rc = subbox_core(c, total_nbox, total_loss)) return rc;
    if (sum_nbox) *sum_nbox = (int)total_nbox;
    if (photon_loss) *photon_loss = total_loss;
    return 0;
}

}
```

Baseline: 115.9 billion.

## Defer xh_intermed and phi_ion materialisation in evolve loop until requested

In the isothermal, non-slab evolve loop, the chemistry pass no longer stores xh_intermed each iteration, and the phi_ion fold after convergence is deferred. Both outputs are marked pending and rebuilt on demand by a new recompute kernel or the existing fold whenever a grid accessor, option change or other API call needs them. xh_av is double-buffered in a new arena slot so the final input xh_av stays available for the recompute. This cuts per-iteration memory writes and end-of-step work, at the cost of extra bookkeeping, an added arena slot, and a recompute pass when the outputs are actually read.

After: 119.9 billion, median of 5. +3.4%, better.

```diff
diff --git a/include/asora_hip.h b/include/asora_hip.h
--- a/include/asora_hip.h
+++ b/include/asora_hip.h
@@ -162,6 +162,7 @@
     ASORA_OPT_OPEN_BOUNDARIES = 18,
     ASORA_OPT_COUNT = 19
 };
+enum { ASORA_OPT_EAGER_OUTPUTS = 32 };
 int asora_set_option(int option, int value);
 int asora_get_option(int option);
 
diff --git a/pyc2ray_amd/_capi.py b/pyc2ray_amd/_capi.py
--- a/pyc2ray_amd/_capi.py
+++ b/pyc2ray_amd/_capi.py
@@ -11,6 +11,7 @@
  OPT_HEATING, OPT_C2RAY_OWN_FLUX, OPT_NO_UNIFORM_T, OPT_SUBBOX_GLOBAL_SHELLS, OPT_PIPELINED_COPIES,
  OPT_SKIP_ZERO_RATES, OPT_GLOBAL_ATOMICS, OPT_PAIR_SOURCES, OPT_SUBBOX_TABLES, OPT_ALIGNED_ROWS, OPT_GEOMETRY_ON_HOST,
  OPT_PLACEMENT_CANDIDATES, OPT_OPEN_BOUNDARIES) = range(19)
+OPT_EAGER_OUTPUTS = 32
 MAX_SPECTRA = 16
 KERNEL_RAYTRACE, KERNEL_CHEMISTRY, KERNEL_PREP, KERNEL_FINISH = range(4)
 VARIANT_PAIRED, VARIANT_ALIGNED, VARIANT_BUFFER_ATOMICS, VARIANT_SPLIT_DESCRIPTORS, VARIANT_SKIP_ZERO, VARIANT_GLOBAL_SHELLS = 1, 2, 4, 8, 16, 32
diff --git a/pyc2ray_amd/csrc/api.hip b/pyc2ray_amd/csrc/api.hip
--- a/pyc2ray_amd/csrc/api.hip
+++ b/pyc2ray_amd/csrc/api.hip
@@ -92,6 +92,8 @@
     st.lls_a = st.lls_b = 0.0;
     for (int g = 0; g < ASORA_GRID_COUNT; ++g) { st.grid[g] = nullptr; st.grid_valid[g] = false; }
     st.nhi = st.staging = st.acc = nullptr;
+    st.xav_buf[0] = st.xav_buf[1] = nullptr;
+    st.ev_lazy = st.lazy_unsettled = st.pend_xint = st.pend_phi = false;
     drop(st.arena); st.arena_bytes = 0;
     st.ev_clean[0] = st.ev_clean[1] = false; st.ev_sets_known = false;
     drop(st.reach.mask); drop(st.reach.count_dev); st.reach = State::ReachMask();
@@ -159,7 +161,7 @@
 extern "C" {
 
 constexpr int ARENA_CANDIDATES = 8;
-constexpr int ARENA_SLOTS = 14;
+constexpr int ARENA_SLOTS = 15;
 __global__ void __launch_bounds__(256) placement_probe_kernel(char *arena, size_t slot, size_t n)
 {
     const double *in[5]; double *out[7];
@@ -269,7 +271,9 @@
         st.nhi = take(2);
         st.grid[ASORA_GRID_PHI_ION] = take(2);
         st.staging = take(1);
-    }
+        st.xav_buf[0] = st.grid[ASORA_GRID_XH_AV]; st.xav_buf[1] = take(1);
+    }
+    st.ev_lazy = st.lazy_unsettled = st.pend_xint = st.pend_phi = false;
     for (int g = 0; g < ASORA_GRID_COUNT; ++g)
         if (g != ASORA_GRID_PHI_HEAT && g != ASORA_GRID_TEMP_END && g != ASORA_GRID_CLUMP && !st.grid[g]) return fail(11, "device_init: a grid without a place in the arena (internal error)");
     st.nhi_t = st.nhi + st.ncell;
@@ -308,13 +312,17 @@
 int asora_set_option(int option, int value)
 {
     clear_error();
+    if (option == ASORA_OPT_EAGER_OUTPUTS) { g_state.eager_outputs = value; return 0; }
     if (option < 0 || option >= ASORA_OPT_COUNT) return fail(3, "set_option: unknown option");
+    if (g_state.init && option != ASORA_OPT_TIMING && g_state.opt[option] != value)
+        if (int rc = materialise_evolve_outputs(g_state)) return rc;
     g_state.opt[option] = value;
     return 0;
 }
 
 int asora_get_option(int option)
 {
+    if (option == ASORA_OPT_EAGER_OUTPUTS) return g_state.eager_outputs;
     if (option < 0 || option >= ASORA_OPT_COUNT) return -1;
     return g_state.opt[option];
 }
diff --git a/pyc2ray_amd/csrc/asora_internal.hpp b/pyc2ray_amd/csrc/asora_internal.hpp
--- a/pyc2ray_amd/csrc/asora_internal.hpp
+++ b/pyc2ray_amd/csrc/asora_internal.hpp
@@ -213,6 +213,11 @@
     double ev_chem[6] = {0, 0, 0, 0, 0, 0};
     int ev_src_begin = 0, ev_src_count = 0;
     RtParams ev_rt;
+    double *xav_buf[2] = {nullptr, nullptr};
+    bool ev_lazy = false;
+    bool lazy_unsettled = false;
+    bool pend_xint = false, pend_phi = false;
+    int lazy_niter = 0;
     bool ev_slab = false;
     int ev_own_begin = 0, ev_own_count = 0;
     bool ev_slab_passed = false;
@@ -254,6 +259,7 @@
     std::vector<PendingTimer> pending_timers;
     std::vector<hipEvent_t> free_events;
     int opt[ASORA_OPT_COUNT] = {0, 0, 0, 1, 0, 0, 0, 0, 0, 0, 1, 0, 0, 0, 0, 0, 0, 0, 0};
+    int eager_outputs = 0;
     double k_ms[ASORA_KERNEL_COUNT] = {0, 0, 0, 0};
     long k_n[ASORA_KERNEL_COUNT] = {0, 0, 0, 0};
 };
@@ -397,6 +403,7 @@
 int launch_temp_probe(State &st, const double *temp, size_t n, double bh00, double albpow, double colh0, double temph0,
                       double *out_dev);
 int launch_chemistry_tiles(State &st, ChemTileParams &p, hipStream_t stream);
+int launch_xh_intermed_tiles(State &st, const ChemTileParams &p, hipStream_t stream);
 size_t chemistry_tile_blocks(const State &st, int N, int planes);
 int launch_prepare_nhi_from(State &st, const double *xh_av, bool need_transposed);
 int launch_prepare_range(State &st, int i_begin, int i_count, bool zero_acc, double *acc, const int *done = nullptr);
@@ -430,5 +437,8 @@
 int ensure_red_capacity(size_t entries);
 int ensure_temp_probe(double bh00, double albpow, double colh0, double temph0);
 ChemTileParams chem_tile_common(int i_begin, int i_count, const double chem[6]);
+constexpr unsigned PENDING_XINT = 1u, PENDING_PHI = 2u, PENDING_ALL = 3u;
+int materialise_evolve_outputs(State &st, unsigned which = PENDING_ALL);
+int evolve_outputs_before(State &st, int which, bool writes, bool whole = true);
 
 }
diff --git a/pyc2ray_amd/csrc/chemistry.hip b/pyc2ray_amd/csrc/chemistry.hip
--- a/pyc2ray_amd/csrc/chemistry.hip
+++ b/pyc2ray_amd/csrc/chemistry.hip
@@ -315,10 +315,11 @@
 
 __device__ __forceinline__ double stream_load(const double *q) { return __builtin_nontemporal_load(q); }
 
-template <bool FOLD, bool EMIT, bool UNIFORM_T, bool THERMAL = false, bool CLUMP = false>
+template <bool FOLD, bool EMIT, bool UNIFORM_T, bool THERMAL = false, bool CLUMP = false, bool STORE_XINT = true>
 __global__ void __launch_bounds__(CH_THREADS, 1) chemistry_tile_kernel(const ChemTileParams p)
 {
     static_assert(!THERMAL || (EMIT && !UNIFORM_T), "thermal pass: the device loop's emit forms only (with or without fold), never UNIFORM_T");
+    static_assert(STORE_XINT || (FOLD && EMIT && !THERMAL), "xh_intermed on demand: the isothermal fold + emit form only");
     if (p.status && p.status->done) return;
     __shared__ double tile_g[32][33], tile_n[32][33];
     __shared__ double tile_h[(THERMAL && FOLD) ? 32 : 1][33];
@@ -382,7 +383,7 @@
                     if (!UNIFORM_T) temperature_factors(cp, stream_load(p.temp + idx), tf);
                     chemistry_cell<CLUMP>(cp, n, stream_load(p.xh + idx), g, xav, xint, nconv, tf, c);
                 }
-                p.xh_intermed[idx] = xint;
+                if (STORE_XINT) p.xh_intermed[idx] = xint;
                 p.xh_av[idx] = xav;
                 sum1 += xint; sum0 += 1.0 - xint;
                 if (EMIT) {
@@ -417,6 +418,48 @@
         p.red_partial[b] = r1[0];
         p.red_partial[(size_t)p.red_stride + b] = r0[0];
         p.red_partial[2 * (size_t)p.red_stride + b] = (double)rc[0];
+    }
+}
+
+template <bool UNIFORM_T, bool CLUMP>
+__global__ void __launch_bounds__(CH_THREADS) xh_intermed_tile_kernel(const ChemTileParams p)
+{
+    __shared__ double tile_g[32][33];
+    const int N = p.N;
+    const int NL = (N + 7) >> 3;
+    const int tx = threadIdx.x & 31, ty = threadIdx.x >> 5;
+    const int kb = blockIdx.x * 32, ib = p.i_begin + blockIdx.z * 32;
+    ChemParams cp;
+    cp.dt = p.dt; cp.bh00 = p.bh00; cp.albpow = p.albpow; cp.colh0 = p.colh0; cp.temph0 = p.temph0; cp.abu_c = p.abu_c;
+    unsigned int nconv = 0;
+    TempFactors tf;
+    if (UNIFORM_T) { tf.T = p.uniform_T; tf.brech0 = p.uniform_brech0; tf.acolh0 = p.uniform_acolh0; tf.t_ok = p.uniform_t_ok != 0; }
+    for (int j = blockIdx.y; j < N; j += gridDim.y) {
+        if (j != (int)blockIdx.y) __syncthreads();
+        for (int r = ty; r < 32; r += 8) {
+            const int k = kb + r, i = ib + tx;
+            if (k < N && i < p.i_end) {
+                const bool reached = !p.reach_t || p.reach_t[((size_t)k * N + j) * NL + (i >> 3)] != 0;
+                tile_g[r][tx] = reached ? stream_load(p.gamma_t + ((size_t)k * N + j) * N + i) : 0.0;
+            }
+        }
+        __syncthreads();
+        for (int r = ty; r < 32; r += 8) {
+            const int i = ib + r, k = kb + tx;
+            if (i < p.i_end && k < N) {
+                const size_t idx = ((size_t)i * N + j) * N + k;
+                const bool reached = !p.reach_a || p.reach_a[((size_t)i * N + j) * NL + (k >> 3)] != 0;
+                double g = reached ? stream_load(p.gamma + idx) : 0.0;
+                g += tile_g[tx][r];
+                const double n = stream_load(p.ndens + idx);
+                double xav = stream_load(p.xh_av_in + idx), xint;
+                double c = 1.0;
+                if (CLUMP) c = stream_load(p.clump + idx);
+                if (!UNIFORM_T) temperature_factors(cp, stream_load(p.temp + idx), tf);
+                chemistry_cell<CLUMP>(cp, n, stream_load(p.xh + idx), g, xav, xint, nconv, tf, c);
+                p.xh_intermed[idx] = xint;
+            }
+        }
     }
 }
 
@@ -589,6 +632,12 @@
 static int launch_tile_form(const ChemTileParams &q, dim3 grid, hipStream_t stream)
 {
     const bool u = q.uniform != 0;
+    if (!q.xh_intermed) {
+        if (q.thermal || !q.fold || !q.emit) return fail(11, "chemistry: only the isothermal fold + emit pass runs without xh_intermed (internal error)");
+        if (u) hipLaunchKernelGGL((chemistry_tile_kernel<true, true, true, false, CLUMP, false>), grid, dim3(CH_THREADS), 0, stream, q);
+        else   hipLaunchKernelGGL((chemistry_tile_kernel<true, true, false, false, CLUMP, false>), grid, dim3(CH_THREADS), 0, stream, q);
+        return 0;
+    }
     if (q.thermal) {
         if (!q.emit) return fail(11, "chemistry: the thermal pass exists in the emit forms only (internal error)");
         if (!q.fold && !q.heat_out) return fail(11, "chemistry: the thermal pass without fold keeps the summed heating (internal error)");
@@ -634,6 +683,31 @@
     return 0;
 }
 
+int launch_xh_intermed_tiles(State &st, const ChemTileParams &p, hipStream_t stream)
+{
+    const int planes = p.i_end - p.i_begin;
+    if (planes <= 0) return 0;
+    if (p.thermal || !p.fold || !p.gamma_t || !p.xh_intermed) return fail(11, "chemistry: xh_intermed is formed again for the isothermal fold + emit pass only (internal error)");
+    const dim3 grid = tile_pass_grid(st, p.N, planes);
+    ChemTileParams q = p;
+    double f;
+    const int ck = clumping_of(st, false, st.ncell, q.clump, q.clump_c, f);
+    if (ck > 1) return ck;
+    q.bh00 = f * p.bh00;
+    if (p.uniform && st.temp_probe_clump != f)
+        return fail(4, "chemistry: the temperature probe was made for another clumping mode (set asora_clumping before asora_evolve_begin)");
+    KernelTimer kt(ASORA_KERNEL_FINISH, stream);
+    if (ck) {
+        if (p.uniform) hipLaunchKernelGGL((xh_intermed_tile_kernel<true, true>), grid, dim3(CH_THREADS), 0, stream, q);
+        else           hipLaunchKernelGGL((xh_intermed_tile_kernel<false, true>), grid, dim3(CH_THREADS), 0, stream, q);
+    } else {
+        if (p.uniform) hipLaunchKernelGGL((xh_intermed_tile_kernel<true, false>), grid, dim3(CH_THREADS), 0, stream, q);
+        else           hipLaunchKernelGGL((xh_intermed_tile_kernel<false, false>), grid, dim3(CH_THREADS), 0, stream, q);
+    }
+    ASORA_HIP_TRY(hipGetLastError());
+    return 0;
+}
+
 __global__ void convergence_test_kernel(const double *sums, EvolveStatus *status)
 {
     if (status->done) return;
diff --git a/pyc2ray_amd/csrc/chemistry_api.hip b/pyc2ray_amd/csrc/chemistry_api.hip
--- a/pyc2ray_amd/csrc/chemistry_api.hip
+++ b/pyc2ray_amd/csrc/chemistry_api.hip
@@ -69,6 +69,7 @@
     clear_error();
     if (int rc = require_init("chemistry_device")) return rc;
     State &st = state();
+    if (int rc = materialise_evolve_outputs(st)) return rc;
     if (int rc = require_grids("chemistry_device", {ASORA_GRID_NDENS, ASORA_GRID_TEMP, ASORA_GRID_XH, ASORA_GRID_XH_AV, ASORA_GRID_PHI_ION})) return rc;
     if (st.th_on) {
         if (!st.grid[ASORA_GRID_PHI_HEAT] || !st.grid_valid[ASORA_GRID_PHI_HEAT])
@@ -99,6 +100,7 @@
     clear_error();
     if (int rc = require_init("chemistry_range")) return rc;
     State &st = state();
+    if (int rc = materialise_evolve_outputs(st)) return rc;
     if (st.th_on) return fail(4, "chemistry_range: not available in thermal mode (single GPU: asora_chemistry_device or asora_evolve_*)");
     if (int rc = require_grids("chemistry_range", {ASORA_GRID_NDENS, ASORA_GRID_TEMP, ASORA_GRID_XH, ASORA_GRID_XH_AV, ASORA_GRID_PHI_ION})) return rc;
     st.grid_valid[ASORA_GRID_XH_INTERMED] = true;
@@ -171,6 +173,7 @@
     clear_error();
     if (int rc = require_init("thermal_params")) return rc;
     State &st = state();
+    if (int rc = materialise_evolve_outputs(st)) return rc;
     if (!enable) { st.th_on = false; return 0; }
     if (!st.have_heat_tables || st.opt[ASORA_OPT_GREY_NOTABLES])
         return fail(4, "thermal_params: thermal mode needs heating tables on the device (heat_table_to_device) and table rates");
@@ -190,6 +193,7 @@
 {
     clear_error();
     State &st = state();
+    if (st.init) { if (int rc = materialise_evolve_outputs(st)) return rc; }
     if (mode == 0) { st.clump_mode = 0; st.clump_c = 1.0; return 0; }
     if (int rc = require_init("clumping")) return rc;
     if (mode == 1) {
@@ -212,6 +216,7 @@
     State &st = state();
     if (!(std::isfinite(n_const) && n_const >= 0.0 && std::isfinite(per_density) && per_density >= 0.0))
         return fail(3, "lls_opacity: n_const and per_density must be finite and >= 0");
+    if (st.init) { if (int rc = materialise_evolve_outputs(st)) return rc; }
     if (n_const == 0.0 && per_density == 0.0) { st.lls_a = st.lls_b = 0.0; return 0; }
     if (int rc = require_init("lls_opacity")) return rc;
     if (st.opt[ASORA_OPT_GREY_NOTABLES])
diff --git a/pyc2ray_amd/csrc/evolve_api.hip b/pyc2ray_amd/csrc/evolve_api.hip
--- a/pyc2ray_amd/csrc/evolve_api.hip
+++ b/pyc2ray_amd/csrc/evolve_api.hip
@@ -86,6 +86,67 @@
     return c;
 }
 
+static const double *lazy_xav_in(const State &st, int k) { return k == 1 ? st.grid[ASORA_GRID_XH] : st.xav_buf[(k - 1) & 1]; }
+
+static int read_status(State &st)
+{
+    ASORA_HIP_TRY(hipMemcpyAsync(st.ev_host, st.ev_status, sizeof(EvolveStatus), hipMemcpyDeviceToHost, st.stream));
+    ASORA_HIP_TRY(hipStreamSynchronize(st.stream));
+    const int niter = st.ev_host->niter;
+    if (niter > 0) {
+        const int set = (st.ev_base + niter - 1) & 1;
+        st.ev_clean[set] = false; st.ev_clean[set ^ 1] = true;
+    }
+    st.ev_sets_known = true;
+    st.ev_enqueued = niter;
+    if (st.lazy_unsettled) {
+        st.lazy_unsettled = false;
+        st.lazy_niter = niter;
+        if (niter > 0) st.grid[ASORA_GRID_XH_AV] = st.xav_buf[niter & 1];
+        else st.pend_xint = st.pend_phi = false;
+    }
+    return 0;
+}
+
+int materialise_evolve_outputs(State &st, unsigned which)
+{
+    if (st.lazy_unsettled) { if (int rc = read_status(st)) return rc; }
+    const int k = st.lazy_niter, set = (st.ev_base + k - 1) & 1;
+    if ((which & PENDING_PHI) && st.pend_phi) {
+        const double *a = acc_pair(set);
+        if (int rc = launch_fold_sum(st, a, a + st.ncell, st.grid[ASORA_GRID_PHI_ION])) return rc;
+        st.ev_folded_iter = k;
+        st.pend_phi = false;
+    }
+    if ((which & PENDING_XINT) && st.pend_xint) {
+        ChemTileParams c = evolve_pass_params(0, st.N, set);
+        c.xh_av_in = lazy_xav_in(st, k);
+        if (st.reach.in_use) { c.reach_a = st.reach.mask; c.reach_t = st.reach.mask + st.reach.bytes; }
+        if (int rc = launch_xh_intermed_tiles(st, c, st.stream)) return rc;
+        st.pend_xint = false;
+    }
+    return 0;
+}
+
+int evolve_outputs_before(State &st, int which, bool writes, bool whole)
+{
+    if (!st.lazy_unsettled && !st.pend_xint && !st.pend_phi) return 0;
+    switch (which) {
+    case ASORA_GRID_XH_AV:
+        return st.lazy_unsettled ? read_status(st) : 0;
+    case ASORA_GRID_XH_INTERMED:
+    case ASORA_GRID_PHI_ION: {
+        const unsigned bit = which == ASORA_GRID_PHI_ION ? PENDING_PHI : PENDING_XINT;
+        if (writes && whole) { (bit == PENDING_PHI ? st.pend_phi : st.pend_xint) = false; return 0; }
+        return materialise_evolve_outputs(st, bit);
+    }
+    case ASORA_GRID_NDENS: case ASORA_GRID_XH: case ASORA_GRID_TEMP: case ASORA_GRID_CLUMP:
+        return writes ? materialise_evolve_outputs(st) : 0;
+    default:
+        return 0;
+    }
+}
+
 static void evolve_pass_thermal(ChemTileParams &c, int set)
 {
     State &st = state();
@@ -109,6 +170,7 @@
     clear_error();
     if (int rc = require_init("evolve_begin")) return rc;
     State &st = state();
+    if (int rc = materialise_evolve_outputs(st)) return rc;
     st.ev_open = false;
     if (slab && st.th_on && !slab_thermal)
         return fail(4, "evolve_begin_slab: thermal mode is on, and this entry begins an isothermal step (single-GPU thermal loop: "
@@ -176,6 +238,7 @@
     st.ev_slab = slab; st.ev_own_begin = own_begin; st.ev_own_count = own_count; st.ev_slab_passed = false;
     st.ev_slab_thermal = slab && st.th_on;
     st.ev_rates_in_outbox = false; st.ev_folded_all = false;
+    st.ev_lazy = !slab && !st.th_on && !st.eager_outputs;
     st.ev_open = true;
     return 0;
 }
@@ -442,8 +505,13 @@
     if (st.ev_enqueued - st.ev_reported + iterations > EVOLVE_HIST)
         return fail(4, "evolve_enqueue: " + std::to_string(st.ev_enqueued - st.ev_reported) + " iterations enqueued since the last "
                            "asora_evolve_poll; the history ring holds " + std::to_string(EVOLVE_HIST) + " (poll first)");
+    if (st.ev_lazy && st.th_on) {
+        if (st.ev_enqueued > 0) return fail(4, "evolve_enqueue: thermal mode was switched on inside a step (call asora_evolve_begin again)");
+        st.ev_lazy = false;
+    }
     st.ev_sets_known = false;
     for (int it = 0; it < iterations; ++it) {
+        const int k = st.ev_enqueued + it + 1;
         const int set = (st.ev_base + st.ev_enqueued + it) & 1;
         if (st.ev_src_count > 0) {
             RtParams p = st.ev_rt;
@@ -454,6 +522,7 @@
         ChemTileParams c = evolve_pass_params(0, st.N, set);
         if (st.reach.in_use) { c.reach_a = st.reach.mask; c.reach_t = st.reach.mask + st.reach.bytes; }
         if (st.th_on) evolve_pass_thermal(c, set);
+        if (st.ev_lazy) { c.xh_av_in = lazy_xav_in(st, k); c.xh_av = st.xav_buf[k & 1]; c.xh_intermed = nullptr; }
         if (int rc = launch_chemistry_tiles(st, c, st.stream)) return rc;
         st.ev_first = false;
     }
@@ -464,7 +533,12 @@
     }
     st.ev_enqueued += iterations;
     st.grid_valid[ASORA_GRID_XH_AV] = st.grid_valid[ASORA_GRID_XH_INTERMED] = true;
-    st.grid_valid[ASORA_GRID_PHI_ION] = false;
+    if (st.ev_lazy) {
+        st.pend_xint = st.pend_phi = true;
+        st.lazy_unsettled = true;
+        st.grid_valid[ASORA_GRID_PHI_ION] = true;
+    } else
+        st.grid_valid[ASORA_GRID_PHI_ION] = false;
     return 0;
 }
 
@@ -474,11 +548,12 @@
     if (int rc = require_init("evolve_poll")) return rc;
     State &st = state();
     if (!st.ev_open) return fail(4, "evolve_poll: no evolve step in progress (call asora_evolve_begin)");
-    ASORA_HIP_TRY(hipMemcpyAsync(st.ev_host, st.ev_status, sizeof(EvolveStatus), hipMemcpyDeviceToHost, st.stream));
-    ASORA_HIP_TRY(hipStreamSynchronize(st.stream));
+    if (int rc = read_status(st)) return rc;
     const EvolveStatus &h = *st.ev_host;
     const bool thermal = st.ev_slab ? st.ev_slab_thermal : st.th_on;
-    if (h.niter > 0) {
+    if (h.niter > 0 && st.ev_lazy) {
+        if (h.done) { if (int rc = materialise_evolve_outputs(st)) return rc; }
+    } else if (h.niter > 0) {
         const int set = (st.ev_base + h.niter - 1) & 1;
         if (st.ev_slab && st.ev_rates_in_outbox) st.ev_folded_iter = h.niter;
         if (st.ev_folded_iter != h.niter) {
@@ -491,17 +566,14 @@
             st.ev_folded_iter = h.niter;
         }
         st.grid_valid[ASORA_GRID_PHI_ION] = true;
-        st.ev_clean[set] = false; st.ev_clean[set ^ 1] = true;
         if (thermal) {
             st.grid_valid[ASORA_GRID_PHI_HEAT] = true;
             st.heat_clean[set] = false; st.heat_clean[set ^ 1] = true;
         }
     }
-    st.ev_sets_known = true;
     int rows = 0;
     for (int it = st.ev_reported; it < h.niter && history && rows < history_rows; ++it, ++rows)
         for (int q = 0; q < 5; ++q) history[5 * rows + q] = h.hist[it % EVOLVE_HIST][q];
-    st.ev_enqueued = h.niter;
     if (history) st.ev_reported += rows;
     else st.ev_reported = h.niter;
     if (rows_written) *rows_written = rows;
diff --git a/pyc2ray_amd/csrc/grids_api.hip b/pyc2ray_amd/csrc/grids_api.hip
--- a/pyc2ray_amd/csrc/grids_api.hip
+++ b/pyc2ray_amd/csrc/grids_api.hip
@@ -29,6 +29,7 @@
     if (which < 0 || which >= ASORA_GRID_COUNT) return fail(3, "grid_to_device: bad grid selector");
     if (!host) return fail(3, "grid_to_device: null host pointer");
     State &st = state();
+    if (int rc = evolve_outputs_before(st, which, true)) return rc;
     if (int rc = ensure_optional_grid(which)) return rc;
     st.zero_since_probe = std::max(st.zero_since_probe, 48);
     const size_t bytes = st.ncell * sizeof(double);
@@ -54,6 +55,7 @@
     if (!host) return fail(3, "grid_to_host: null host pointer");
     State &st = state();
     if (!st.grid[which] || !st.grid_valid[which]) return fail(3, "grid_to_host: grid " + std::to_string(which) + " holds no data");
+    if (int rc = evolve_outputs_before(st, which, false)) return rc;
     const size_t bytes = st.ncell * sizeof(double);
     if (order == 'C' || order == 'c') {
         ASORA_HIP_TRY(hipMemcpyAsync(host, st.grid[which], bytes, hipMemcpyDeviceToHost, st.stream));
@@ -74,6 +76,8 @@
         return fail(3, "grid_copy: bad grid selectors");
     State &st = state();
     if (!st.grid_valid[src]) return fail(3, "grid_copy: source grid holds no data");
+    if (int rc = evolve_outputs_before(st, src, false)) return rc;
+    if (int rc = evolve_outputs_before(st, dst, true)) return rc;
     if (int rc = ensure_optional_grid(dst)) return rc;
     ASORA_HIP_TRY(hipMemcpyAsync(st.grid[dst], st.grid[src], st.ncell * sizeof(double), hipMemcpyDeviceToDevice,
                                  st.stream));
@@ -89,6 +93,7 @@
     if (which < 0 || which >= ASORA_GRID_COUNT) return fail(3, "grid_scale: bad grid selector");
     State &st = state();
     if (!st.grid_valid[which]) return fail(3, "grid_scale: grid " + std::to_string(which) + " holds no data");
+    if (int rc = evolve_outputs_before(st, which, true, false)) return rc;
     if (int rc = launch_scale(st, st.grid[which], st.ncell, factor)) return rc;
     if (which == ASORA_GRID_TEMP) st.temp_probe_valid = false;
     return 0;
@@ -102,6 +107,7 @@
     if (!sum) return fail(3, "grid_sum: null output pointer");
     State &st = state();
     if (!st.grid_valid[which]) return fail(3, "grid_sum: grid " + std::to_string(which) + " holds no data");
+    if (int rc = evolve_outputs_before(st, which, false)) return rc;
     if (!st.temp_probe_dev) ASORA_HIP_TRY(hipMalloc(&st.temp_probe_dev, sizeof(double) * 8));
     if (int rc = launch_grid_sum(st, st.grid[which], st.ncell, st.temp_probe_dev + 5)) return rc;
     ASORA_HIP_TRY(hipMemcpyAsync(sum, st.temp_probe_dev + 5, sizeof(double), hipMemcpyDeviceToHost, st.stream));
@@ -129,6 +135,7 @@
 void *asora_device_ptr(int which)
 {
     if (!state().init || which < 0 || which >= ASORA_GRID_COUNT) return nullptr;
+    if (evolve_outputs_before(state(), which, true, false) != 0) return nullptr;
     return state().grid[which];
 }
 
@@ -360,6 +367,7 @@
     if (i_count == 0) return 0;
     if (!host) return fail(3, "planes_to_host: null host pointer");
     if (!st.grid_valid[which]) return fail(3, "planes_to_host: grid " + std::to_string(which) + " holds no data");
+    if (int rc = evolve_outputs_before(st, which, false)) return rc;
     const size_t plane = (size_t)st.N * st.N;
     ASORA_HIP_TRY(hipMemcpyAsync(host, st.grid[which] + (size_t)i_begin * plane, (size_t)i_count * plane * sizeof(double),
                                  hipMemcpyDeviceToHost, st.stream));
@@ -376,6 +384,7 @@
     if (int rc = check_planes("planes_to_device", 3, "bad plane range", i_begin, i_count)) return rc;
     if (i_count == 0) return 0;
     if (!host) return fail(3, "planes_to_device: null host pointer");
+    if (int rc = evolve_outputs_before(st, which, true, false)) return rc;
     if (int rc = ensure_optional_grid(which)) return rc;
     const size_t plane = (size_t)st.N * st.N;
     ASORA_HIP_TRY(hipMemcpyAsync(st.grid[which] + (size_t)i_begin * plane, host, (size_t)i_count * plane * sizeof(double),
diff --git a/pyc2ray_amd/csrc/raytrace_api.hip b/pyc2ray_amd/csrc/raytrace_api.hip
--- a/pyc2ray_amd/csrc/raytrace_api.hip
+++ b/pyc2ray_amd/csrc/raytrace_api.hip
@@ -293,6 +293,7 @@
 {
     clear_error();
     if (int rc = require_init("raytrace_device")) return rc;
+    if (int rc = materialise_evolve_outputs(state())) return rc;
     return do_raytrace(R, sig, dr, src_begin, src_count, minlogtau, dlogtau, NumTau, nullptr);
 }
 
@@ -300,6 +301,7 @@
 {
     clear_error();
     if (int rc = require_init("raytrace_begin")) return rc;
+    if (int rc = materialise_evolve_outputs(state())) return rc;
     return rt_begin(R, sig, dr, minlogtau, dlogtau, NumTau, nullptr, true);
 }
 
@@ -308,6 +310,7 @@
 {
     clear_error();
     if (int rc = require_init("raytrace_begin_planes")) return rc;
+    if (int rc = materialise_evolve_outputs(state())) return rc;
     State &st = state();
     st.rt_open = false;
     if (int rc = require_raytrace_inputs("raytrace_begin_planes", R, NumTau, true, true)) return rc;
@@ -348,6 +351,7 @@
     (void)coldensh_out; (void)ndens;
     clear_error();
     if (int rc = require_init("do_all_sources")) return rc;
+    if (int rc = materialise_evolve_outputs(state())) return rc;
     if (int rc = check_N("do_all_sources", m1)) return rc;
     if (!xh_av || !phi_ion) return fail(3, "do_all_sources: null xh_av / phi_ion");
     State &st = state();
@@ -397,6 +401,7 @@
 {
     clear_error();
     if (int rc = require_init("debug_coldens")) return rc;
+    if (int rc = materialise_evolve_outputs(state())) return rc;
     if (int rc = check_N("debug_coldens", N)) return rc;
     if (!coldens_out) return fail(3, "debug_coldens: null output");
     State &st = state();
diff --git a/pyc2ray_amd/csrc/subbox_api.hip b/pyc2ray_amd/csrc/subbox_api.hip
--- a/pyc2ray_amd/csrc/subbox_api.hip
+++ b/pyc2ray_amd/csrc/subbox_api.hip
@@ -220,6 +220,7 @@
         heat = any;
     }
     if (int rc = asora_device_init_auto(m1)) return rc;
+    if (int rc = materialise_evolve_outputs(st)) return rc;
     const int N = st.N;
     for (int s = 0; s < NumSrc; ++s)
         for (int ax = 0; ax < 3; ++ax)
@@ -296,6 +297,7 @@
     clear_error();
     if (int rc = require_init("subbox_raytrace_device")) return rc;
     State &st = state();
+    if (int rc = materialise_evolve_outputs(st)) return rc;
     const char *who = "subbox_raytrace_device";
     if (st.opt[ASORA_OPT_OPEN_BOUNDARIES])
         return fail(4, std::string(who) + ": open boundaries (ASORA_OPT_OPEN_BOUNDARIES) have no sub-box sweep (the reference's Fortran has no such mode)");
```
